# charles-cooper/Smoothed-Particle-Hydrodynamics

Hardware: AMD Instinct MI355X
Metric: particle-steps/sec (whole node) (higher is better)
Workload: dtype f32; 1 GPU; config4_16M_box; particles=16507704, particles_per_gpu=16507704, cell_ids=wide, parallelism=1 GPU

## Files before the change

include/sphmi.h:

```cpp
#ifndef SPHMI_H
#define SPHMI_H

#include <stddef.h>
#include <stdint.h>

#ifdef __cplusplus
extern "C" {
#endif

#define SPHMI_ABI_VERSION 2
#define SPH_MAX_PARTICLES ((1 << 27) - 1)
#define SPH_MAX_NEIGHBOR_COUNT 32
#define SPH_MAX_MEMBRANES_INCLUDING_SAME_PARTICLE 7
#define SPH_LIQUID_PARTICLE 1
#define SPH_ELASTIC_PARTICLE 2
#define SPH_BOUNDARY_PARTICLE 3

typedef enum sph_status {
  SPH_OK = 0,
  SPH_ERR_INVALID = -1,
  SPH_ERR_HIP = -2,
  SPH_ERR_ORDER = -3,
  SPH_ERR_UNKNOWN_BUFFER = -4,
  SPH_ERR_SIZE = -5
// ... 69 lines not shown

#define SPH_SURFACE_FIELDS 6
int sph_extract_surface(sph_solver* s, const float origin[3], const float spacing[3], const int32_t dims[3], uint32_t typeMask,
                        int32_t field, float iso, int64_t counts[2] );
int sph_read_surface(sph_solver* s, float* vertices , int32_t* triangles );

#define SPH_GRADIENT_WORDS 32
int sph_sample_gradient_points(sph_solver* s, const float* points4 , int32_t count,
                               uint32_t typeMask, float* out );
int sph_sample_gradient_grid(sph_solver* s, const float origin[3], const float spacing[3], const int32_t dims[3],
                             uint32_t typeMask, float* out );
int sph_surface_normals(sph_solver* s, float* normals );

#define SPH_DIAG_WORDS 32
#define SPH_DIAG_MAX_REGIONS 16
int sph_diagnostics(sph_solver* s, const float* regions6 , int32_t count,
                    uint32_t typeMask, double* out );
#define SPH_HIST_MAX_BINS 4096
int sph_histogram(sph_solver* s, int32_t field, float lo, float hi, int32_t bins, const float* region6 ,
                  uint32_t typeMask, uint32_t* out );

int sph_label_components(sph_solver* s, float linkRadius, uint32_t typeMask, int64_t counts[2] );
int sph_read_components(sph_solver* s, int32_t* labels , int32_t* rootCount ,
                        float* bbox );
int sph_component_diagnostics(sph_solver* s, const int32_t* components , int32_t count,
                              double* out );

#define SPH_SELECT_WORDS 12
#define SPH_SELECT_MAX_TERMS 4
#define SPH_SELECT_FIELD_SURFACE 7
typedef struct sph_select_term { int32_t field; float lo, hi; } sph_select_term;
int sph_particle_measure(sph_solver* s, float* out );
int sph_select_particles(sph_solver* s, const float* region6 , uint32_t typeMask,
                         const sph_select_term* terms , int32_t termCount, int32_t component ,
                         int64_t* count);
int sph_read_selection(sph_solver* s, int32_t* sortedIndex , uint32_t* origId ,
                       float* records );

#define SPH_ELASTIC_WORDS 12
#define SPH_MUSCLE_WORDS 16
#define SPH_MEMBRANE_WORDS 8
int sph_elastic_measure(sph_solver* s, int32_t* sortedIndex , uint32_t* origId ,
                        float* records , float* connections );
int sph_muscle_diagnostics(sph_solver* s, double* out );
int sph_membrane_measure(sph_solver* s, float* out , double totals[4]);

#define SPH_FORCE_WORDS 40
#define SPH_FORCE_DIAG_WORDS 64
int sph_force_measure(sph_solver* s, int32_t fromSelection, float* out );
int sph_force_diagnostics(sph_solver* s, const float* regions6 , int32_t count,
                          uint32_t typeMask, double* out );

typedef struct sph_render_view {
  int32_t width, height;
  int32_t projection;
  float eye[3], right[3], up[3], forward[3];
  float scale;
  float centre[2];
  float nearPlane;
  float radius;
  float maxRadiusPx;
  int32_t colourMode;
  int32_t field; float lo, hi;
  float typeColour[3][3];
  float ambient;
  uint8_t background[4];
} sph_render_view;
#define SPH_RENDER_FIELD_RAMP { {0.f, 0.f, 1.f}, {0.f, 1.f, 1.f}, {0.f, 1.f, 0.f}, {1.f, 1.f, 0.f}, {1.f, 0.f, 0.f} }
#define SPH_RENDER_LABEL_COLOURS 12
#define SPH_RENDER_LABEL_PALETTE { {0.90f, 0.10f, 0.10f}, {0.10f, 0.50f, 0.90f}, {0.20f, 0.70f, 0.20f}, {0.95f, 0.60f, 0.10f}, \
                                   {0.60f, 0.30f, 0.80f}, {0.10f, 0.75f, 0.75f}, {0.95f, 0.90f, 0.20f}, {0.85f, 0.35f, 0.65f}, \
                                   {0.55f, 0.35f, 0.15f}, {0.40f, 0.85f, 0.55f}, {0.30f, 0.30f, 0.65f}, {0.75f, 0.75f, 0.75f} }
int sph_render_particles(sph_solver* s, const sph_render_view* view, const float* region6 , uint32_t typeMask,
                         int32_t wantThickness, int64_t counts[2] );
int sph_read_render(sph_solver* s, float* depth, int32_t* sortedIndex, uint32_t* origId, uint8_t* rgba ,
                    uint32_t* thickness);

typedef struct sph_render_mesh_style {
  int32_t source;
  int32_t shading;
  int32_t colourMode;
  int32_t field;
  float lo, hi;
  float colour[3];
  int32_t compose;
} sph_render_mesh_style;
int sph_render_mesh(sph_solver* s, const sph_render_view* view, const sph_render_mesh_style* style,
                    int64_t counts[4] );
int sph_read_render_triangles(sph_solver* s, int32_t* triangle );

int sph_remove_region(sph_solver* s, const float* region6 , uint32_t typeMask, int32_t countOnly,
                      int64_t* removed);
int sph_remove_selection(sph_solver* s, int64_t* removed);
int sph_remove_ids(sph_solver* s, const uint32_t* origIds , int64_t count, int64_t* removed);
int sph_add_particles(sph_solver* s, const float* position4, const float* velocity4 , int32_t count);
int sph_emit_lattice(sph_solver* s, const float origin[3], const float spacing[3], const int32_t dims[3], const float velocity[3],
                     float typeValue , int64_t* added);
int sph_read_edit_map(sph_solver* s, int32_t* newIdOfOld );

#define SPH_FIELD_SLOTS 4
#define SPH_FIELD_DIAG_WORDS 8
int sph_field_create(sph_solver* s, int32_t slot, const float* valuesN , float inflow);
int sph_field_release(sph_solver* s, int32_t slot);
int sph_field_write(sph_solver* s, int32_t slot, const float* valuesN );
int sph_field_read(sph_solver* s, int32_t slot, float* outN );
int sph_field_set_region(sph_solver* s, int32_t slot, const float* region6 , uint32_t typeMask, float value,
                         int64_t* painted);
int sph_field_set_selection(sph_solver* s, int32_t slot, float value, int64_t* painted);
int sph_field_diffuse(sph_solver* s, int32_t slot, float coefficient, int32_t substeps, uint32_t typeMask, float* stability);
int sph_field_diagnostics(sph_solver* s, int32_t slot, const float* regions6 , int32_t count,
                          uint32_t typeMask, double* out );

#define SPH_TRACE_TIME 0
#define SPH_TRACE_ARC 1
#define SPH_TRACE_EULER 0
#define SPH_TRACE_MIDPOINT 1
#define SPH_TRACE_MOVING 0
#define SPH_TRACE_MAX_STEPS 1
#define SPH_TRACE_LEFT_MATTER 2
#define SPH_TRACE_LEFT_REGION 3
#define SPH_TRACE_STAGNANT 4
#define SPH_TRACE_NONFINITE 5
#define SPH_TRACE_MAX_STEPS_LIMIT 65535
typedef struct sph_trace_params {
  float step;
  float minSpeed;
  int32_t maxSteps;
  int32_t mode;
  int32_t integrator;
} sph_trace_params;
int sph_trace_streamlines(sph_solver* s, const float* seeds4 , int32_t count, uint32_t typeMask,
                          const sph_trace_params* params, const float* region6 ,
                          float* vertices , int32_t* lengths ,
                          int32_t* status );
int sph_tracers_set(sph_solver* s, const float* points4 , int32_t count);
int sph_tracers_advect(sph_solver* s, uint32_t typeMask, const sph_trace_params* params, const float* region6 ,
                       int64_t counts[2] );
int sph_tracers_read(sph_solver* s, float* pos4 , int32_t* status, int32_t* steps);

int sph_synchronize(sph_solver* s);

typedef enum sph_stage {
  SPH_ST_HASH = 0, SPH_ST_SORT, SPH_ST_SORT_POST, SPH_ST_INDEX, SPH_ST_FIND_NEIGHBORS, SPH_ST_DENSITY,
  SPH_ST_FORCES, SPH_ST_ELASTIC, SPH_ST_PREDICT_DENSITY, SPH_ST_PRESSURE_FORCE, SPH_ST_INTEGRATE, SPH_ST_MEMBRANES,
  SPH_ST_COUNT
} sph_stage;
int sph_set_stage_timing(sph_solver* s, int enable);
int sph_get_stage_times(sph_solver* s, double* ms_total, int64_t* launches, int n);
int sph_reset_stage_times(sph_solver* s);
int sph_step_sort_passes(sph_solver* s);
int sph_set_step_chunks(sph_solver* s, int32_t chunks);
int sph_set_step_pipeline(sph_solver* s, int32_t depth);

typedef struct sph_slab {
  int32_t layerLo, layerHi;
  int32_t ghostLayers;
  int32_t hasLower, hasUpper;
  int32_t globalIdBits;
} sph_slab;
#define SPH_SLAB_RECORD_WORDS 9
#define SPH_SLAB_COMPACT_WORDS 7
int sph_slab_init(sph_solver* s, const sph_slab* slab, const uint32_t* globalIds );
int sph_slab_pack(sph_solver* s, void* msgDown, void* msgUp, int32_t capRecords, int32_t counts[3]);
int sph_slab_pack_framed(sph_solver* s, void* frameDown, void* frameUp, int32_t capRecords, int32_t counts[3]);
int sph_slab_rebuild(sph_solver* s, const void* recvDown, int32_t nDown, const void* recvUp, int32_t nUp);
int sph_slab_step_begin(sph_solver* s, int iterationCount, void* frameDown, void* frameUp, int32_t capRecords);
int sph_slab_step_messages(sph_solver* s, int32_t counts[2]);
int sph_slab_rebuild_framed(sph_solver* s, const void* frameDown, int32_t capDownRecords, const void* frameUp, int32_t capUpRecords);
int sph_slab_rebuild_finish(sph_solver* s, int32_t counts[4]);
int sph_slab_liquid_signature(sph_solver* s, uint32_t* typeBits);
int sph_slab_set_record_format(sph_solver* s, int32_t recordWords, uint32_t typeBits);
int sph_stream_wait_event(sph_solver* s, void* hipEvent);
int sph_particle_count(sph_solver* s);
int sph_slab_read(sph_solver* s, float* position4, float* velocity4, uint32_t* globalIds, uint32_t* owned);

const char* sph_last_error(void);
int sph_abi_version(void);
const char* sph_build_info(void);

#ifdef __cplusplus
}
#endif
#endif
```

smoothed-particle-hydrodynamics_amd/csrc/sph_api.hip:

```cpp
#include <stdarg.h>
#include <string.h>

#include <cmath>
#include <memory>

#include "sph_api_internal.h"
#include "sph_fastmath.h"

#define SPH_STR_(x) #x
#define SPH_STR(x) SPH_STR_(x)
static thread_local char g_err[512] = "";
void sph_set_error(const char* fmt, ...) {
  va_list ap;
  va_start(ap, fmt);
  vsnprintf(g_err, sizeof(g_err), fmt, ap);
  va_end(ap);
}

extern "C" const char* sph_last_error(void) { return g_err; }
extern "C" int sph_abi_version(void) { return SPHMI_ABI_VERSION; }

extern "C" const char* sph_build_info(void) {
  return "libsphmi gfx950 abi " SPH_STR(SPHMI_ABI_VERSION)
#ifdef FN_STAMPS
// ... 196 lines not shown
      if (ended) continue;
      if (x <= -2.f || (double)x >= (double)N) {
        sph_set_error("elastic connection %d of particle %d: partner %g is neither -1 nor in [0, %d)", k, i, x, N);
        return SPH_ERR_INVALID;
      }
      if ((int)x == -1) { ended = true; continue; }
      if (!std::isfinite(w[1])) { sph_set_error("elastic connection %d of particle %d: rest length %g is not finite", k, i, w[1]); return SPH_ERR_INVALID; }
      if (!(w[2] >= -2147483648.f && w[2] < 2147483648.f)) {
        sph_set_error("elastic connection %d of particle %d: muscle word %g does not convert to int", k, i, w[2]);
        return SPH_ERR_INVALID;
      }
    }
  }
  if (!(membraneData && pml && M > 0)) return SPH_OK;
  for (size_t k = 0; k < (size_t)3 * M; k++)
    if (membraneData[k] < 0 || membraneData[k] >= N) {
      sph_set_error("membraneData[%zu] (corner %zu of membrane %zu) = %d is not in [0, %d)", k, k % 3, k / 3, membraneData[k], N);
      return SPH_ERR_INVALID;
    }
  for (int i = 0; i < E; i++)
    for (int k = 0; k < SPH_MAX_MEMBRANES_INCLUDING_SAME_PARTICLE; k++) {
      const int32_t m = pml[(size_t)i * SPH_MAX_MEMBRANES_INCLUDING_SAME_PARTICLE + k];
      if (m < 0) break;
      if (m >= M) {
        sph_set_error("particleMembranesList[%d][%d] = %d is not below numOfMembranes %d", i, k, m, M);
        return SPH_ERR_INVALID;
      }
    }
  if (c.elasticOffset != 0) { sph_set_error("membrane lists need elasticOffset 0 (got %d): they are indexed by original particle id", c.elasticOffset); return SPH_ERR_INVALID; }
  for (int i = E; i < N; i++)
    if (position[4 * (size_t)i + 3] >= 2.f && position[4 * (size_t)i + 3] < 3.f) {
      sph_set_error("particle %d has elastic type %g but lies outside the elastic block [0, %d) that the membrane lists cover", i,
                    position[4 * (size_t)i + 3], E);
      return SPH_ERR_INVALID;
    }
  return SPH_OK;
}

extern "C" int sph_create(const sph_config* cfg, const float* position, const float* velocity, const float* elastic,
                          const int32_t* membraneData, const int32_t* pml, sph_solver** out) {
  if (!cfg || !position || !velocity || !out) { sph_set_error("sph_create: null argument"); return SPH_ERR_INVALID; }
  *out = nullptr;
  if (cfg->abi_version != SPHMI_ABI_VERSION) { sph_set_error("sph_config.abi_version %d != %d", cfg->abi_version, SPHMI_ABI_VERSION); return SPH_ERR_INVALID; }
  const int N = cfg->particleCount;
  const int cap = cfg->capacity > 0 ? cfg->capacity : N;
  static_assert((long long)SPH_MAX_PARTICLES * SPH_MAXN < 0x100000000LL, "uint32 mapBase in k_find_neighbors");
  if (N <= 0 || cap < N || cap > SPH_MAX_PARTICLES) {
    sph_set_error("particleCount %d / capacity %d out of range: one solver holds at most %d particles (2^27 - 1; 32-bit neighbour-map "
                  "indices)", N, cap, SPH_MAX_PARTICLES);
    return SPH_ERR_INVALID;
  }
  if (cfg->gridCellsX <= 0 || cfg->gridCellsY <= 0 || cfg->gridCellsZ <= 0 ||
      (long long)cfg->gridCellsX * cfg->gridCellsY * cfg->gridCellsZ != (long long)cfg->gridCellCount) {
    sph_set_error("gridCellCount does not equal gridCellsX*gridCellsY*gridCellsZ");
    return SPH_ERR_INVALID;
  }
  if (cfg->cellIdMask != 0xffffu && cfg->cellIdMask != 0xffffffffu) { sph_set_error("cellIdMask must be 0xffff (reference) or 0xffffffff (wide)"); return SPH_ERR_INVALID; }
  if (cfg->numOfElasticP < 0 || (cfg->numOfElasticP > 0 && cfg->elasticOffset < 0) || (long long)cfg->numOfElasticP + cfg->elasticOffset > N ||
      (cfg->numOfElasticP > 0 && !elastic)) {
    sph_set_error("elastic configuration inconsistent");
    return SPH_ERR_INVALID;
  }
  if (cfg->numOfElasticP > 0 && (cfg->muscleCount <= 0 || cfg->muscleCount > 4096)) { sph_set_error("muscleCount out of range"); return SPH_ERR_INVALID; }
  if (cfg->maxIteration < 1) { sph_set_error("maxIteration must be >= 1"); return SPH_ERR_INVALID; }
  if (!(cfg->h > 0.f) || !(cfg->hashGridCellSize > 0.f)) { sph_set_error("h / hashGridCellSize must be positive"); return SPH_ERR_INVALID; }

  uint32_t liquidSig = 0u;
  for (int i = 0; i < N; i++) {
    const float* p4 = position + 4 * (size_t)i;
    sph_fold_liquid_signature(liquidSig, p4, velocity + 4 * (size_t)i);
    if (const char* fault = sph_position_fault(*cfg, p4)) {
      sph_set_error("particle %d at (%g, %g, %g) is %s", i, p4[0], p4[1], p4[2], fault);
      return SPH_ERR_INVALID;
    }
  }
  { const int rc = check_elastic_input(*cfg, position, elastic, membraneData, pml); if (rc != SPH_OK) return rc; }
  int ndev = 0;
  const hipError_t devErr = hipGetDeviceCount(&ndev);
  if (devErr != hipSuccess || ndev <= 0 || cfg->device < 0 || cfg->device >= ndev) {
    char two[300];
    if (two_hip_runtimes(two, sizeof(two)))
      sph_set_error("no HIP device %d (found %d): two HIP runtimes are mapped into this process (%s); load the one the rest of the "
                    "process uses BEFORE libsphmi.so so that both bind to it", cfg->device, ndev, two);
    else
      sph_set_error("no HIP device %d (found %d%s%s): libsphmi has no CPU fallback", cfg->device, ndev,
                    devErr != hipSuccess ? ", " : "", devErr != hipSuccess ? hipGetErrorString(devErr) : "");
    return SPH_ERR_HIP;
  }
  SPH_HIP(hipSetDevice(cfg->device));

  std::unique_ptr<sph_solver> owner(new sph_solver());
  sph_solver* const s = owner.get();
  s->cfg = *cfg;
  s->liquidSig = liquidSig;
  if (cfg->stream) { s->stream = (hipStream_t)cfg->stream; s->ownStream = false; }
  else {
    hipError_t e = hipStreamCreateWithFlags(&s->stream, hipStreamNonBlocking);
    if (e != hipSuccess) { sph_set_error("hipStreamCreate failed: %s", hipGetErrorString(e)); return SPH_ERR_HIP; }
    s->ownStream = true;
  }
  SPH_HIP(hipStreamCreateWithFlags(&s->chunkStream, hipStreamNonBlocking));
  SPH_HIP(hipStreamCreateWithFlags(&s->searchStream, hipStreamNonBlocking));
  SPH_HIP(hipEventCreateWithFlags(&s->evSearchFork, hipEventDisableTiming));
  for (hipEvent_t& e : s->evChunk) SPH_HIP(hipEventCreateWithFlags(&e, hipEventDisableTiming));
  SPH_HIP(hipEventCreateWithFlags(&s->evChunkJoin, hipEventDisableTiming));
  SphDev& d = s->d;
  d.N = N; d.G = cfg->gridCellCount; d.gx = cfg->gridCellsX; d.gy = cfg->gridCellsY; d.gz = cfg->gridCellsZ;
  d.cellMask = cfg->cellIdMask;
  d.h = cfg->h; d.cellSize = cfg->hashGridCellSize; d.cellSizeInv = cfg->hashGridCellSizeInv;
  d.simScale = cfg->simulationScale; d.simScaleInv = cfg->simulationScaleInv;
  d.xmin = cfg->xmin; d.xmax = cfg->xmax; d.ymin = cfg->ymin; d.ymax = cfg->ymax; d.zmin = cfg->zmin; d.zmax = cfg->zmax;
  d.r0 = cfg->r0; d.mass = cfg->mass; d.rho0 = cfg->rho0; d.dt = cfg->timeStep; d.delta = cfg->delta;
  d.gravx = cfg->gravity_x; d.gravy = cfg->gravity_y; d.gravz = cfg->gravity_z;
  d.surfTens = cfg->surfTensCoeff;
  {
    volatile float massMu = cfg->mass * cfg->viscosity;
    volatile float hs = cfg->h * cfg->simulationScale;
    volatile float hs2 = hs * hs;
    volatile float hs4 = hs2 * hs2;
    volatile float hs6 = hs4 * hs2;
    volatile float pts = cfg->timeStep * cfg->simulationScaleInv;
    volatile float r0d = cfg->rho0 * cfg->delta;
    volatile float halfHs = hs / 2;
    d.massMu = massMu; d.hs = hs; d.hs2 = hs2; d.hs6 = hs6; d.posTimeStep = pts; d.rho0delta = r0d;
    d.closeR = 0.5 * (double)halfHs;
    float f = (float)d.closeR;
    while ((double)f < d.closeR) f = nextafterf(f, INFINITY);
    while ((double)nextafterf(f, -INFINITY) >= d.closeR) f = nextafterf(f, -INFINITY);
    d.closeRf = f;
  }
  d.massWpoly6 = ((double)cfg->mass) * cfg->Wpoly6Coefficient;
  sph_fast_bounds(cfg->simulationScale, d.hs, (float)((double)d.hs6 * d.massWpoly6), &d.fastD2Min, &d.fastD2Max, &d.fastValueMin);
  d.massGradW = ((double)cfg->mass) * cfg->gradWspikyCoefficient;
  d.del2W = cfg->del2WviscosityCoefficient;
  d.numElastic = cfg->numOfElasticP; d.elasticOffset = cfg->elasticOffset; d.muscleCount = cfg->muscleCount;
  d.numMembranes = cfg->numOfMembranes; d.hasElastic = cfg->numOfElasticP > 0;
  d.rangeLo = 0; d.rangeHi = d.G;

  s->capacity = cap;
  s->capTiles = (cap + SPH_TILE - 1) / SPH_TILE;
  s->sortBits = (cfg->cellIdMask == 0xffffu) ? 16 : bit_length((uint32_t)(d.G > 0 ? d.G - 1 : 0));
  if (s->sortBits < 1) s->sortBits = 1;
  s->maxSortBlocks = (cap + (SPH_BLOCK * 16) - 1) / (SPH_BLOCK * 16);

  int rc = SPH_OK;
  const size_t n = (size_t)cap, nUp = (size_t)N, G1 = (size_t)d.G + 1, mapN = (size_t)s->capTiles * 64 * 32;
#define A(ptr, count) if (rc == SPH_OK) rc = dev_alloc(s, &(ptr), (count))
  A(d.posOrig, n); A(d.velOrig, n); A(d.sortedPos, n); A(d.sortedVel, n); A(d.predPos, 3 * n); A(d.acc, n); A(d.accP, n); A(d.rp, n); A(d.bndMask, n); A(d.gatherRec, 2 * ((n + 3) / 4 * 4));
  A(d.keys, n); A(d.vals, n); A(d.keysAlt, n); A(d.valsAlt, n); A(d.backIndex, n);
  A(d.cellStart, G1); A(d.cellStartRaw, G1);
  A(d.nbrId, mapN); A(d.nbrDist, mapN); A(d.nbr16, mapN); A(d.nbrBase, (size_t)s->capTiles * 64);
  A(d.rho, n);
  const size_t waves = (size_t)s->capTiles;
  A(d.pBlk, waves); A(d.cBlk, waves); A(d.xBlk, waves); A(d.k12Skip, waves); A(d.k10Skip, waves); A(d.skipGate, SPH_GATE_SLOTS);
  A(s->blockHist, (size_t)SPH_SORT_MAX_DIGITS * s->maxSortBlocks + SPH_SORT_MAX_DIGITS);
  A(d.gid, n); A(d.owned, n); A(s->slabCounts, SPH_SLAB_COUNT_WORDS);
  A(d.dbg, SPH_DBG_WORDS); A(s->chunkEdges, SPH_STEP_CHUNKS_MAX + 1); A(s->pipeTable, SPH_STEP_CHUNKS_MAX + 3);
  float* binU = nullptr;
  A(binU, 64);
  d.binU = binU;
  if (d.hasElastic) {
    A(d.elasticMask, n); A(d.membDelta, n); A(d.elastic, (size_t)32 * d.numElastic); A(d.muscle, (size_t)d.muscleCount);
    if (membraneData && pml && cfg->numOfMembranes > 0) { A(d.membraneData, (size_t)3 * cfg->numOfMembranes); A(d.pml, (size_t)7 * d.numElastic); }
  }
#undef A
  if (rc != SPH_OK) return rc;

#define UP(dst, src, bytes) do { hipError_t e_ = hipMemcpyAsync((dst), (src), (bytes), hipMemcpyHostToDevice, s->stream); \
    if (e_ != hipSuccess) { sph_set_error("upload failed: %s", hipGetErrorString(e_)); return SPH_ERR_HIP; } } while (0)
  UP(d.posOrig, position, sizeof(float4) * nUp);
  UP(d.velOrig, velocity, sizeof(float4) * nUp);
  if (d.hasElastic) {
    UP(d.elastic, elastic, sizeof(float4) * 32 * (size_t)d.numElastic);
    hipMemsetAsync(d.muscle, 0, sizeof(float) * (size_t)d.muscleCount, s->stream);
    hipMemsetAsync(d.membDelta, 0, sizeof(float4) * n, s->stream);
    if (d.membraneData) {
      UP(d.membraneData, membraneData, sizeof(int32_t) * 3 * (size_t)cfg->numOfMembranes);
      UP(d.pml, pml, sizeof(int32_t) * 7 * (size_t)d.numElastic);
    }
  }
  {
    float U[64];
    compute_bin_thresholds(cfg->h, U);
    UP(binU, U, sizeof(U));
  }
#undef UP
  hipMemsetAsync(d.predPos, 0, sizeof(float) * 3 * n, s->stream);
  hipMemsetAsync(d.acc, 0, sizeof(float4) * n, s->stream);
  hipMemsetAsync(d.accP, 0, sizeof(float4) * n, s->stream);
  hipMemsetAsync(d.rho, 0, sizeof(float) * n, s->stream);
  hipMemsetAsync(d.rp, 0, sizeof(float2) * n, s->stream);
  for (uint8_t* f : {d.pBlk, d.cBlk, d.xBlk, d.k12Skip, d.k10Skip}) hipMemsetAsync(f, 0, waves, s->stream);
  hipMemsetAsync(d.nbrId, 0xff, sizeof(int32_t) * mapN, s->stream);
  hipMemsetAsync(d.nbrDist, 0, sizeof(float) * mapN, s->stream);
  hipMemsetAsync(d.nbr16, 0xff, sizeof(uint16_t) * mapN, s->stream);
  hipMemsetAsync(d.nbrBase, 0, sizeof(int32_t) * (size_t)s->capTiles * 64, s->stream);
  hipMemsetAsync(d.dbg, 0, sizeof(uint32_t) * SPH_DBG_WORDS, s->stream);
  hipMemsetAsync(d.skipGate, 0, sizeof(uint32_t) * SPH_GATE_SLOTS, s->stream);
  hipMemsetAsync(d.cellStartRaw, 0, sizeof(uint32_t) * G1, s->stream);
  hipMemsetAsync(d.cellStart, 0, sizeof(uint32_t) * G1, s->stream);
  hipMemsetAsync(d.sortedPos, 0, sizeof(float4) * n, s->stream);
  hipMemsetAsync(d.sortedVel, 0, sizeof(float4) * n, s->stream);
  hipMemsetAsync(d.keys, 0, sizeof(uint32_t) * n, s->stream);
  hipMemsetAsync(d.vals, 0, sizeof(uint32_t) * n, s->stream);
  hipMemsetAsync(d.backIndex, 0, sizeof(uint32_t) * n, s->stream);
  hipError_t e = hipStreamSynchronize(s->stream);
  if (e != hipSuccess) { sph_set_error("sph_create: %s", hipGetErrorString(e)); return SPH_ERR_HIP; }
  *out = owner.release();
  return SPH_OK;
}

struct Stage {
  const char* name;
  int need, timer;
  int (*launch)(sph_solver*);
  int gain;
};
#define LAUNCH(call) [](sph_solver* s) { return call; }
static const Stage kClearBuffers = {"sph_run_clear_buffers", 0, SPH_ST_FIND_NEIGHBORS, LAUNCH(sphk_clear_neighbors(s)), 0};
static const Stage kHashParticles = {"sph_run_hash_particles", 0, SPH_ST_HASH, LAUNCH(sphk_hash(s)), P_HASH};
static const Stage kSort = {"sph_run_sort", P_HASH, SPH_ST_SORT, LAUNCH(sphk_sort(s)), P_SORT};
static const Stage kSortPostPass = {"sph_run_sort_post_pass", P_SORT, SPH_ST_SORT_POST, LAUNCH(sphk_sort_post(s)), P_SORTPOST};
static const Stage kIndexx = {"sph_run_indexx", P_SORT, SPH_ST_INDEX, LAUNCH(sphk_index_raw(s)), P_INDEXX};
static const Stage kIndexPostPass = {"sph_run_index_post_pass", P_INDEXX, SPH_ST_INDEX, LAUNCH(sphk_index_fixed(s)), P_INDEXPOST};
static const Stage kFindNeighbors = {"sph_run_find_neighbors", P_SORTPOST | P_INDEXPOST, SPH_ST_FIND_NEIGHBORS, LAUNCH(sphk_find_neighbors(s)), P_FIND};
static const Stage kComputeDensity = {"sph_run_pcisph_compute_density", P_FIND, SPH_ST_DENSITY, LAUNCH(sphk_density(s)), P_DENSITY};
static const Stage kComputeForces = {"sph_run_pcisph_compute_forces_and_init_pressure", P_DENSITY, SPH_ST_FORCES, LAUNCH(sphk_forces(s, false)), P_FORCES};
static const Stage kElasticForces = {"sph_run_pcisph_compute_elastic_forces", P_FORCES, SPH_ST_ELASTIC, LAUNCH(sphk_elastic(s)), 0};
static const Stage kPredictPositions = {"sph_run_pcisph_predict_positions", P_FORCES, SPH_ST_PRESSURE_FORCE, LAUNCH(sphk_predict_positions(s)), P_PREDICTPOS};
static const Stage kPredictDensity = {"sph_run_pcisph_predict_density", P_PREDICTPOS, SPH_ST_PREDICT_DENSITY, LAUNCH(sphk_predict_density(s, false)), P_PREDICTDENS};
static const Stage kCorrectPressure = {"sph_run_pcisph_correct_pressure", P_PREDICTDENS, SPH_ST_PREDICT_DENSITY, LAUNCH(sphk_correct_pressure(s)), 0};
static const Stage kPressureForce = {"sph_run_pcisph_compute_pressure_force_acceleration", P_PREDICTDENS, SPH_ST_PRESSURE_FORCE, LAUNCH(sphk_pressure_force(s, 0)), P_PRESSUREFORCE};
static const Stage kIntegrate = {"sph_run_pcisph_integrate", P_FORCES, SPH_ST_INTEGRATE, LAUNCH(sphk_integrate(s)), 0};
static const Stage kClearMembraneBuffers = {"sph_run_clear_membrane_buffers", 0, SPH_ST_MEMBRANES, LAUNCH(sphk_clear_membranes(s)), 0};
static const Stage kMembranes = {"sph_run_compute_interaction_with_membranes", P_FIND, SPH_ST_MEMBRANES, LAUNCH(sphk_membranes(s)), 0};
static const Stage kMembranesFinalize = {"sph_run_compute_interaction_with_membranes_finalize", 0, SPH_ST_MEMBRANES, LAUNCH(sphk_membranes_finalize(s)), 0};
#undef LAUNCH

static int run_stage(sph_solver* s, const Stage& st) {
  ENTER(s); NEED(s, st.need, st.name);
  sph_state_changes(s);
  StageTimer t(s, st.timer);
  const int rc = st.launch(s);
  if (rc == SPH_OK) s->progress = st.gain == P_HASH ? P_HASH : s->progress | st.gain;
  return rc;
}

extern "C" int sph_run_clear_buffers(sph_solver* s) { return run_stage(s, kClearBuffers); }
extern "C" int sph_run_hash_particles(sph_solver* s) { return run_stage(s, kHashParticles); }
extern "C" int sph_run_sort(sph_solver* s) { return run_stage(s, kSort); }
extern "C" int sph_run_sort_post_pass(sph_solver* s) { return run_stage(s, kSortPostPass); }
extern "C" int sph_run_indexx(sph_solver* s) { return run_stage(s, kIndexx); }
extern "C" int sph_run_index_post_pass(sph_solver* s) { return run_stage(s, kIndexPostPass); }
extern "C" int sph_run_find_neighbors(sph_solver* s) { return run_stage(s, kFindNeighbors); }
extern "C" int sph_run_pcisph_compute_density(sph_solver* s) { return run_stage(s, kComputeDensity); }
extern "C" int sph_run_pcisph_compute_forces_and_init_pressure(sph_solver* s) { return run_stage(s, kComputeForces); }
extern "C" int sph_run_pcisph_compute_elastic_forces(sph_solver* s) { return run_stage(s, kElasticForces); }
extern "C" int sph_run_pcisph_predict_positions(sph_solver* s) { return run_stage(s, kPredictPositions); }
extern "C" int sph_run_pcisph_predict_density(sph_solver* s) { return run_stage(s, kPredictDensity); }
extern "C" int sph_run_pcisph_correct_pressure(sph_solver* s) { return run_stage(s, kCorrectPressure); }
extern "C" int sph_run_pcisph_compute_pressure_force_acceleration(sph_solver* s) { return run_stage(s, kPressureForce); }
extern "C" int sph_run_pcisph_integrate(sph_solver* s, int ) { return run_stage(s, kIntegrate); }
extern "C" int sph_run_clear_membrane_buffers(sph_solver* s) { return run_stage(s, kClearMembraneBuffers); }
extern "C" int sph_run_compute_interaction_with_membranes(sph_solver* s) {
  ENTER(s); NEED(s, kMembranes.need, kMembranes.name);
  if (!s->d.pml) return SPH_OK;
  return run_stage(s, kMembranes);
}
extern "C" int sph_run_compute_interaction_with_membranes_finalize(sph_solver* s) { return run_stage(s, kMembranesFinalize); }

#ifndef SPH_OVERLAP_CHUNKS
#define SPH_OVERLAP_CHUNKS 16
#endif
#ifndef SPH_OVERLAP_MIN_PARTICLES
#define SPH_OVERLAP_MIN_PARTICLES (4 << 20)
#endif
static_assert(SPH_OVERLAP_CHUNKS >= 1 && SPH_OVERLAP_CHUNKS <= SPH_STEP_CHUNKS_MAX, "chunk count");
#ifndef SPH_PIPELINE_DEPTH
#define SPH_PIPELINE_DEPTH 1
#endif
static_assert(SPH_PIPELINE_DEPTH >= 0 && SPH_PIPELINE_DEPTH <= SPH_PIPELINE_STAGES_MAX, "pipeline depth");

extern "C" int sph_set_step_chunks(sph_solver* s, int32_t chunks) {
  ENTER(s);
  if (chunks < 0 || chunks > SPH_STEP_CHUNKS_MAX) { sph_set_error("sph_set_step_chunks: %d is not in [0, %d]", chunks, SPH_STEP_CHUNKS_MAX); return SPH_ERR_INVALID; }
  s->stepChunks = chunks;
  return SPH_OK;
}

extern "C" int sph_set_step_pipeline(sph_solver* s, int32_t depth) {
  ENTER(s);
  if (depth < -1 || depth > SPH_PIPELINE_STAGES_MAX) { sph_set_error("sph_set_step_pipeline: %d is not in [-1, %d]", depth, SPH_PIPELINE_STAGES_MAX); return SPH_ERR_INVALID; }
  s->stepPipeline = depth;
  return SPH_OK;
}

static int step_chunks(const sph_solver* s) {
  if (s->hasSlab || s->timing) return 1;
  if (s->stepChunks > 0) return s->stepChunks;
  return s->d.N >= SPH_OVERLAP_MIN_PARTICLES ? SPH_OVERLAP_CHUNKS : 1;
}

struct ChunkEdges { uint32_t e[SPH_STEP_CHUNKS_MAX + 1]; };
__global__ void k_chunk_edges(uint32_t* edges, ChunkEdges v) {
  if (threadIdx.x <= SPH_STEP_CHUNKS_MAX) edges[threadIdx.x] = v.e[threadIdx.x];
}

static int step_pipeline(const sph_solver* s) {
  return sphPipelineDepth(s->stepPipeline >= 0 ? s->stepPipeline : SPH_PIPELINE_DEPTH, s->cfg.maxIteration, s->d.hasElastic ? 1 : 0);
}

__global__ void k_halo_check(const uint32_t* keys, const uint32_t* cellStart, int G, int gx, int gy, int N, int chunks, ChunkEdges v,
                             uint32_t* table, uint32_t* dbg) {
  const int c = threadIdx.x;
  int ok = 1;
  if (c < chunks) {
    const int64_t reach = (int64_t)gx * gy + gx + 1;
    ok = sphChunkHaloOk(keys, cellStart, G, reach, N, v.e[c], v.e[c + 1], v.e[max(c - 1, 0)], v.e[min(c + 2, chunks)]);
  }
  const bool passed = __all(ok);
  if (c <= SPH_STEP_CHUNKS_MAX) table[c] = passed ? v.e[c] : 0u;
  if (c == 0) {
    table[SPH_STEP_CHUNKS_MAX + 1] = 0u;
    table[SPH_STEP_CHUNKS_MAX + 2] = passed ? 0u : (uint32_t)N;
    atomicAdd(&dbg[passed ? 10 : 9], 1u);
  }
}

static int enqueue_search_overlapped(sph_solver* s, int chunks, int depth) {
  const int N = s->d.N;
  ChunkEdges v;
  for (int i = 0; i <= SPH_STEP_CHUNKS_MAX; i++) v.e[i] = (uint32_t)sphChunkEdge(N, chunks, i);
  if (s->chunkEdgesN != N || s->chunkEdgesC != chunks) {
    hipLaunchKernelGGL(k_chunk_edges, dim3(1), dim3(64), 0, s->stream, s->chunkEdges, v);
    SPH_HIP(hipGetLastError());
    s->chunkEdgesN = N; s->chunkEdgesC = chunks;
  }
  if (depth > 0) {
    hipLaunchKernelGGL(k_halo_check, dim3(1), dim3(64), 0, s->stream, s->d.keys, s->d.cellStart, s->d.G, s->d.gx, s->d.gy, N, chunks, v,
                       s->pipeTable, s->d.dbg);
    SPH_HIP(hipGetLastError());
  }
  SPH_HIP(hipEventRecord(s->evSearchFork, s->stream));
  SPH_HIP(hipStreamWaitEvent(s->searchStream, s->evSearchFork, 0));
  auto launch = [s, N, chunks](int stage, int c) -> int {
    const int lo = (int)sphChunkEdge(N, chunks, c), hi = (int)sphChunkEdge(N, chunks, c + 1);
    if (hi <= lo) return SPH_OK;
    if (stage > 0) return sphk_pipeline_stage(s, stage, c, lo, hi, s->chunkStream);
    hipStream_t fnStream = (c & 1) ? s->searchStream : s->stream;
    int rc = sphk_find_neighbors(s, -1, lo, hi, fnStream);
    if (rc != SPH_OK) return rc;
    SPH_HIP(hipEventRecord(s->evChunk[c], fnStream));
    SPH_HIP(hipStreamWaitEvent(s->chunkStream, s->evChunk[c], 0));
    rc = sphk_density_chunk(s, c, lo, hi, s->chunkStream);
    return rc != SPH_OK ? rc : sphk_pack_gather_records(s, lo, hi, s->chunkStream);
  };
  int32_t stage[SPH_PIPELINE_ITEMS_MAX(SPH_STEP_CHUNKS_MAX)], chunk[SPH_PIPELINE_ITEMS_MAX(SPH_STEP_CHUNKS_MAX)];
  const int items = sphPipelineSchedule(chunks, depth, s->cfg.maxIteration, s->d.hasElastic ? 1 : 0, stage, chunk);
  int rc = SPH_OK;
  for (int i = 0; i < items && rc == SPH_OK; i++) rc = launch(stage[i], chunk[i]);
  SPH_HIP(hipEventRecord(s->evChunkJoin, s->chunkStream));
  SPH_HIP(hipStreamWaitEvent(s->stream, s->evChunkJoin, 0));
  for (int k = 1; k <= depth && rc == SPH_OK; k++) rc = sphk_pipeline_stage(s, k, -1, 0, N, s->stream);
  return rc;
}

int enqueue_step(sph_solver* s, const StepTail* tail) {
  int rc;
  sph_state_changes(s);
#define RUN(stage, call) do { StageTimer t_(s, stage); rc = (call); if (rc != SPH_OK) return rc; } while (0)
  if (s->hasSlab) {
    RUN(SPH_ST_SORT, sphk_hash_sort_post_slab(s));
    RUN(SPH_ST_SORT_POST, sphk_index_fixed(s));
  } else {
    int bits = s->sortBits;
    bool compact = false;
    RUN(SPH_ST_HASH, sphk_hash_for_step(s, &bits, &compact));
    RUN(SPH_ST_SORT, sphk_sort_pairs(s, s->d.N, bits));
    if (compact) {
      StageTimer t_(s, SPH_ST_SORT_POST);
      rc = sphk_sort_post_rekey(s);
      if (rc == SPH_OK) rc = sphk_index_fixed(s);
      if (rc != SPH_OK) return rc;
    } else {
      RUN(SPH_ST_SORT_POST, sphk_sort_post_and_index(s));
    }
  }
  const bool slab = s->hasSlab;
  const int M = s->cfg.maxIteration;
  auto layersFor = [&](int hops) { return slab ? min((hops * 31 + 59) / 60, s->slab.ghostLayers) : -1; };
  const int chunks = step_chunks(s);
  const int piped = chunks > 1 ? step_pipeline(s) : 0;
  s->waveSkip = !slab && piped <= 1;
  if (chunks > 1) {
    rc = enqueue_search_overlapped(s, chunks, piped);
    if (rc != SPH_OK) return rc;
  } else {
    RUN(SPH_ST_FIND_NEIGHBORS, sphk_find_neighbors(s, layersFor(2 * (M - 1) + 1)));
    RUN(SPH_ST_DENSITY, sphk_density(s, layersFor(1)));
  }
  if (slab) RUN(SPH_ST_FORCES, sphk_ghost_init(s));
  const bool densityInForces = !slab && M >= 1;
  if (piped < 1) RUN(SPH_ST_FORCES, sphk_forces(s, true, layersFor(0), densityInForces, chunks <= 1));
  if (s->d.hasElastic) RUN(SPH_ST_ELASTIC, sphk_elastic(s));
  for (int iter = 0; iter < M; iter++) {
    const int left = M - 1 - iter;
    if (piped >= 2 * iter + 2) continue;
    if (piped < 2 * iter + 1) {
      if (iter > 0 || !densityInForces) RUN(SPH_ST_PREDICT_DENSITY, sphk_predict_density(s, true, layersFor(2 * left + 1), iter == 0, iter));
      else RUN(SPH_ST_PREDICT_DENSITY, SPH_OK);
    }
    if (left > 0 || !tail) { RUN(SPH_ST_PRESSURE_FORCE, sphk_pressure_force(s, left == 0 ? 2 : 1, layersFor(2 * left), iter)); continue; }
    const long long lo = max((long long)s->slab.layerLo, 0LL), hi = min((long long)s->slab.layerHi, (long long)s->d.gz);
    const long long W1 = (long long)s->slab.ghostLayers + 1;
    const long long dEnd = s->slab.hasLower ? min(lo + W1, hi) : lo;
    const long long uBeg = s->slab.hasUpper ? max(hi - W1, dEnd) : hi;
    if (dEnd > lo) RUN(SPH_ST_PRESSURE_FORCE, sphk_pressure_force_layers(s, 2, lo, dEnd));
    if (hi > uBeg) RUN(SPH_ST_PRESSURE_FORCE, sphk_pressure_force_layers(s, 2, uBeg, hi));
    const SphDev dA = sph_ranged_layers(s, lo, dEnd), dB = sph_ranged_layers(s, uBeg, hi);
    SlabPart part{SLAB_PART_MESSAGES, dA.rangeLo, dA.rangeHi, dB.rangeLo, dB.rangeHi};
    rc = sphk_slab_pack(s, tail->frameDown ? tail->frameDown + 1 : nullptr, tail->frameUp ? tail->frameUp + 1 : nullptr, tail->capRecords,
                        tail->frameDown, tail->frameUp, part, s->slabCounts + 4);
    if (rc != SPH_OK) return rc;
    SPH_HIP(hipMemcpyAsync(s->slabHost + 4, s->slabCounts + 4, sizeof(uint32_t) * 3, hipMemcpyDeviceToHost, s->stream));
    SPH_HIP(hipEventRecord(s->slabMsgEvent, s->stream));
    if (uBeg > dEnd) RUN(SPH_ST_PRESSURE_FORCE, sphk_pressure_force_layers(s, 2, dEnd, uBeg));
    rc = sphk_slab_pack(s, nullptr, nullptr, 0, nullptr, nullptr, SlabPart{SLAB_PART_KEPT, 0, 0, 0, 0}, s->slabCounts + 8);
    if (rc != SPH_OK) return rc;
    SPH_HIP(hipMemcpyAsync(s->slabHost + 8, s->slabCounts + 8, sizeof(uint32_t) * 3, hipMemcpyDeviceToHost, s->stream));
    SPH_HIP(hipMemcpyAsync(s->slabHost + 3, s->slabCounts + 3, sizeof(uint32_t), hipMemcpyDeviceToHost, s->stream));
    SPH_HIP(hipMemcpyAsync(s->slabHost + 7, s->slabCounts + 7, sizeof(uint32_t), hipMemcpyDeviceToHost, s->stream));
  }
  if (s->d.hasElastic) {
    RUN(SPH_ST_MEMBRANES, sphk_clear_membranes(s));
    if (s->d.pml) RUN(SPH_ST_MEMBRANES, sphk_membranes(s));
    RUN(SPH_ST_MEMBRANES, sphk_membranes_finalize(s));
  }
#undef RUN
  s->progress = P_HASH | P_SORT | P_SORTPOST | P_INDEXPOST | P_FIND | P_DENSITY | P_FORCES | P_PREDICTPOS | P_PREDICTDENS |
                P_PRESSUREFORCE;
  return SPH_OK;
}

extern "C" int sph_step(sph_solver* s, int iterationCount) {
  (void)iterationCount;
  ENTER(s);
  return enqueue_step(s, nullptr);
}

extern "C" int sph_update_muscles(sph_solver* s, const float* signal, int n) {
  ENTER(s);
  if (!signal || n != s->cfg.muscleCount) { sph_set_error("sph_update_muscles: n must equal muscleCount"); return SPH_ERR_SIZE; }
  if (!s->d.muscle) return SPH_OK;
  SPH_HIP(hipMemcpyAsync(s->d.muscle, signal, sizeof(float) * (size_t)n, hipMemcpyHostToDevice, s->stream));
  SPH_HIP(hipStreamSynchronize(s->stream));
  return SPH_OK;
}

extern "C" int sph_step_sort_passes(sph_solver* s) {
  ENTER(s);
  bool compact;
  return sph_sort_passes(sphk_step_sort_bits(s, &compact));
}

extern "C" int sph_synchronize(sph_solver* s) {
  ENTER(s);
  return sph_check_finite_state(s);
}
```

smoothed-particle-hydrodynamics_amd/csrc/sph_api_read.hip:

```cpp
#include <string.h>

#include <vector>

#include "sph_api_internal.h"

int sph_d2h(sph_solver* s, void* dst, const void* src, size_t bytes) {
  SPH_HIP(hipMemcpyAsync(dst, src, bytes, hipMemcpyDeviceToHost, s->stream));
  SPH_HIP(hipStreamSynchronize(s->stream));
  return SPH_OK;
}

static int report_blown_up(sph_solver* s) {
  sph_set_error("%llu particle coordinate(s) were not finite: the simulation state has blown up", (unsigned long long)s->blownUp);
  return SPH_ERR_INVALID;
}
int sph_check_finite_state(sph_solver* s) {
  uint32_t bad = 0;
  SPH_HIP(hipMemcpyAsync(&bad, s->d.dbg + 6, sizeof(bad), hipMemcpyDeviceToHost, s->stream));
  SPH_HIP(hipStreamSynchronize(s->stream));
  if (bad) {
    s->blownUp += bad;
    SPH_HIP(hipMemsetAsync(s->d.dbg + 6, 0, sizeof(uint32_t), s->stream));
  }
  return s->blownUp ? report_blown_up(s) : SPH_OK;
}

extern "C" int sph_read_position(sph_solver* s, float* out) {
  ENTER(s); if (!out) return SPH_ERR_INVALID;
  const int rc = sph_d2h(s, out, s->d.posOrig, sizeof(float4) * (size_t)s->d.N);
  return rc != SPH_OK ? rc : sph_check_finite_state(s);
}
static int copy_setup(sph_solver* s) {
  if (s->copyStream) return SPH_OK;
  SPH_HIP(hipStreamCreateWithFlags(&s->copyStream, hipStreamNonBlocking));
  SPH_HIP(hipEventCreateWithFlags(&s->evReadReady, hipEventDisableTiming));
  SPH_HIP(hipEventCreateWithFlags(&s->evCopyDone, hipEventDisableTiming));
  SPH_HIP(hipHostMalloc((void**)&s->pinnedFlags, sizeof(uint32_t) * 4, hipHostMallocDefault));
  s->pinnedFlags[0] = 0u;
  return SPH_OK;
}

static bool host_pinned(sph_solver* s, void* p, size_t bytes) {
  for (int i = 0; i < s->numHostRegs; i++)
    if ((char*)p >= (char*)s->hostRegs[i].p && (char*)p + bytes <= (char*)s->hostRegs[i].p + s->hostRegs[i].bytes) return true;
  unsigned int flags = 0;
  if (hipHostGetFlags(&flags, p) == hipSuccess) return true;
  (void)hipGetLastError();
  if (s->numHostRegs >= 8) return false;
  const hipError_t e = hipHostRegister(p, bytes, hipHostRegisterDefault);
  if (e != hipSuccess) { (void)hipGetLastError(); return false; }
  s->hostRegs[s->numHostRegs].p = p; s->hostRegs[s->numHostRegs].bytes = bytes; s->numHostRegs++;
  return true;
}

extern "C" int sph_read_position_wait(sph_solver* s) {
  ENTER(s);
  if (!s->copyPending) return s->blownUp ? report_blown_up(s) : SPH_OK;
  SPH_HIP(hipEventSynchronize(s->evCopyDone));
  s->copyPending = false;
  if (s->copyViaStage) memcpy(s->copyUserDst, s->copyStage, s->copyBytes);
  if (s->pinnedFlags[0]) {
    if (!s->blownUp) s->blownUp = s->pinnedFlags[0];
    return report_blown_up(s);
  }
  return s->blownUp ? report_blown_up(s) : SPH_OK;
}

extern "C" int sph_read_position_async(sph_solver* s, float* out) {
  ENTER(s); if (!out) return SPH_ERR_INVALID;
  int rc = copy_setup(s);
  if (rc != SPH_OK) return rc;
  if (s->copyPending) {
    rc = sph_read_position_wait(s);
    if (rc != SPH_OK) return rc;
  }
  const size_t bytes = sizeof(float4) * (size_t)s->d.N;
  void* dst = out;
  s->copyViaStage = false;
  if (!host_pinned(s, out, bytes)) {
    if (s->copyStageBytes < bytes) {
      if (s->copyStage) hipHostFree(s->copyStage);
      s->copyStage = nullptr; s->copyStageBytes = 0;
      SPH_HIP(hipHostMalloc(&s->copyStage, bytes, hipHostMallocDefault));
      s->copyStageBytes = bytes;
    }
    dst = s->copyStage;
    s->copyViaStage = true;
  }
  s->copyUserDst = out;
  s->copyBytes = bytes;
  SPH_HIP(hipEventRecord(s->evReadReady, s->stream));
  SPH_HIP(hipStreamWaitEvent(s->copyStream, s->evReadReady, 0));
  SPH_HIP(hipMemcpyAsync(dst, s->d.posOrig, bytes, hipMemcpyDeviceToHost, s->copyStream));
  SPH_HIP(hipMemcpyAsync(s->pinnedFlags, s->d.dbg + 6, sizeof(uint32_t), hipMemcpyDeviceToHost, s->copyStream));
  SPH_HIP(hipEventRecord(s->evCopyDone, s->copyStream));
  s->copyPending = true;
  return SPH_OK;
}

extern "C" int sph_host_unregister(sph_solver* s, void* p) {
  ENTER(s);
  if (s->copyPending) { const int rc = sph_read_position_wait(s); if (rc != SPH_OK && rc != SPH_ERR_INVALID) return rc; }
  for (int i = 0; i < s->numHostRegs; i++)
    if (s->hostRegs[i].p == p) {
      hipHostUnregister(p);
      s->hostRegs[i] = s->hostRegs[--s->numHostRegs];
      return SPH_OK;
    }
  return SPH_OK;
}

int sph_guard_position_write(sph_solver* s, hipStream_t stream) {
  if (s->copyPending) SPH_HIP(hipStreamWaitEvent(stream ? stream : s->stream, s->evCopyDone, 0));
  return SPH_OK;
}

extern "C" int sph_read_velocity(sph_solver* s, float* out) {
  ENTER(s); if (!out) return SPH_ERR_INVALID;
  return sph_d2h(s, out, s->d.velOrig, sizeof(float4) * (size_t)s->d.N);
}
extern "C" int sph_read_density(sph_solver* s, float* out) {
  ENTER(s); if (!out) return SPH_ERR_INVALID;
  return sph_d2h(s, out, s->d.rho, sizeof(float) * (size_t)s->d.N);
}
extern "C" int sph_read_particle_index(sph_solver* s, uint32_t* out) {
  ENTER(s); if (!out) return SPH_ERR_INVALID;
  const size_t n = (size_t)s->d.N;
  std::vector<uint32_t> k(n), v(n);
  int rc = sph_d2h(s, k.data(), s->d.keys, sizeof(uint32_t) * n);
  if (rc == SPH_OK) rc = sph_d2h(s, v.data(), s->d.vals, sizeof(uint32_t) * n);
  if (rc != SPH_OK) return rc;
  for (size_t i = 0; i < n; i++) { out[2 * i] = k[i]; out[2 * i + 1] = v[i]; }
  return SPH_OK;
}

extern "C" int sph_read_buffer(sph_solver* s, const char* name, void* out, size_t bytes, size_t* needed) {
  ENTER(s);
  if (!name) return SPH_ERR_INVALID;
  const SphDev& d = s->d;
  const size_t n = (size_t)d.N, G1 = (size_t)d.G + 1;
  size_t need = 0;
  enum { B_POS, B_VEL, B_SPOS, B_SVEL, B_ACC, B_NMAP, B_NIDS, B_PI, B_PIB, B_GCI, B_GCIF, B_P, B_RHO, B_DBG, B_TRACE, B_K12SKIP, B_K10SKIP } which;
  if (!strcmp(name, "position")) { which = B_POS; need = sizeof(float4) * 2 * n; }
  else if (!strcmp(name, "velocity")) { which = B_VEL; need = sizeof(float4) * 2 * n; }
  else if (!strcmp(name, "sortedPosition")) { which = B_SPOS; need = sizeof(float4) * 2 * n; }
  else if (!strcmp(name, "sortedVelocity")) { which = B_SVEL; need = sizeof(float4) * n; }
  else if (!strcmp(name, "acceleration")) { which = B_ACC; need = sizeof(float4) * 2 * n; }
  else if (!strcmp(name, "neighborMap")) { which = B_NMAP; need = sizeof(float) * 2 * 32 * n; }
  else if (!strcmp(name, "neighborIds")) { which = B_NIDS; need = sizeof(int32_t) * 32 * n; }
  else if (!strcmp(name, "particleIndex")) { which = B_PI; need = sizeof(uint32_t) * 2 * n; }
  else if (!strcmp(name, "particleIndexBack")) { which = B_PIB; need = sizeof(uint32_t) * n; }
  else if (!strcmp(name, "gridCellIndex")) { which = B_GCI; need = sizeof(uint32_t) * G1; }
  else if (!strcmp(name, "gridCellIndexFixedUp")) { which = B_GCIF; need = sizeof(uint32_t) * G1; }
  else if (!strcmp(name, "pressure")) { which = B_P; need = sizeof(float) * n; }
  else if (!strcmp(name, "rho")) { which = B_RHO; need = sizeof(float) * 2 * n; }
  else if (!strcmp(name, "diagnosticTrace")) { which = B_TRACE; need = sizeof(uint32_t) * n; }
  else if (!strcmp(name, "debugCounters")) { which = B_DBG; need = sizeof(uint32_t) * SPH_DBG_WORDS; }
  else if (!strcmp(name, "pressureForceSkipped")) { which = B_K12SKIP; need = (n + SPH_TILE - 1) / SPH_TILE; }
  else if (!strcmp(name, "predictDensitySkipped")) { which = B_K10SKIP; need = (n + SPH_TILE - 1) / SPH_TILE; }
  else { sph_set_error("unknown buffer '%s'", name); return SPH_ERR_UNKNOWN_BUFFER; }
  if (needed) *needed = need;
  if (!out) return SPH_OK;
  if (bytes != need) { sph_set_error("buffer '%s' is %zu bytes, caller gave %zu", name, need, bytes); return SPH_ERR_SIZE; }
  int rc = SPH_OK;
  char* o = (char*)out;
  switch (which) {
    case B_POS:
      rc = sph_d2h(s, o, d.posOrig, sizeof(float4) * n);
      if (rc == SPH_OK) { if (d.membDelta) rc = sph_d2h(s, o + sizeof(float4) * n, d.membDelta, sizeof(float4) * n); else memset(o + sizeof(float4) * n, 0, sizeof(float4) * n); }
      break;
    case B_VEL:
      rc = sph_d2h(s, o, d.velOrig, sizeof(float4) * n);
      memset(o + sizeof(float4) * n, 0, sizeof(float4) * n);
      break;
    case B_SPOS: {
      std::vector<uint32_t> k(n);
      std::vector<float4> sv(n);
      rc = sph_d2h(s, o, d.sortedPos, sizeof(float4) * n);
      if (rc == SPH_OK) {
        std::vector<float> p3(3 * n);
        rc = sph_d2h(s, p3.data(), d.predPos, sizeof(float) * 3 * n);
        float4* half = (float4*)(o + sizeof(float4) * n);
        if (rc == SPH_OK) for (size_t i = 0; i < n; i++) half[i] = make_float4(p3[3 * i], p3[3 * i + 1], p3[3 * i + 2], 0.f);
      }
      if (rc == SPH_OK) rc = sph_d2h(s, k.data(), d.keys, sizeof(uint32_t) * n);
      if (rc == SPH_OK) rc = sph_d2h(s, sv.data(), d.sortedVel, sizeof(float4) * n);
      if (rc != SPH_OK) break;
      float4* a = (float4*)o;
      for (size_t i = 0; i < n; i++) {
        const int type = (int)a[i].w;
        const float cellf = (float)(int)k[i];
        a[i].w = cellf;
        a[n + i].w = (type == SPH_BOUNDARY_PARTICLE) ? cellf : cellf + d.posTimeStep * (sv[i].w + d.dt * 0.f);
      }
    } break;
    case B_SVEL: rc = sph_d2h(s, o, d.sortedVel, sizeof(float4) * n); break;
    case B_ACC:
      rc = sph_d2h(s, o, d.acc, sizeof(float4) * n);
      if (rc == SPH_OK) rc = sph_d2h(s, o + sizeof(float4) * n, d.accP, sizeof(float4) * n);
      break;
    case B_NIDS: rc = sph_read_neighbor_rows(s, 0, d.N, (int32_t*)o, nullptr); break;
    case B_NMAP: {
      std::vector<int32_t> ids(32 * n);
      std::vector<float> dist(32 * n);
      rc = sph_read_neighbor_rows(s, 0, d.N, ids.data(), dist.data());
      if (rc == SPH_OK) for (size_t e = 0; e < 32 * n; e++) { ((float*)o)[2 * e] = (float)ids[e]; ((float*)o)[2 * e + 1] = dist[e]; }
    } break;
    case B_PI: rc = sph_read_particle_index(s, (uint32_t*)o); break;
    case B_PIB: rc = sph_d2h(s, o, d.backIndex, sizeof(uint32_t) * n); break;
    case B_GCI: rc = sph_d2h(s, o, d.cellStartRaw, sizeof(uint32_t) * G1); break;
    case B_GCIF: rc = sph_d2h(s, o, d.cellStart, sizeof(uint32_t) * G1); break;
    case B_P: {
      std::vector<float2> rp(n);
      rc = sph_d2h(s, rp.data(), d.rp, sizeof(float2) * n);
      if (rc == SPH_OK) for (size_t i = 0; i < n; i++) ((float*)o)[i] = rp[i].y;
    } break;
    case B_TRACE: rc = sph_d2h(s, o, d.valsAlt, sizeof(uint32_t) * n); break;
    case B_DBG: rc = sph_d2h(s, o, d.dbg, sizeof(uint32_t) * SPH_DBG_WORDS); break;
    case B_K12SKIP: rc = sph_d2h(s, o, d.k12Skip, need); break;
    case B_K10SKIP: rc = sph_d2h(s, o, d.k10Skip, need); break;
    case B_RHO:
      rc = sph_d2h(s, o, d.rho, sizeof(float) * n);
      if (rc == SPH_OK) {
        std::vector<float2> rp(n);
        rc = sph_d2h(s, rp.data(), d.rp, sizeof(float2) * n);
        if (rc == SPH_OK) for (size_t i = 0; i < n; i++) ((float*)o)[n + i] = rp[i].x;
      }
      break;
  }
  return rc;
}

extern "C" int sph_read_neighbor_rows(sph_solver* s, int32_t first, int32_t count, int32_t* ids, float* dist) {
  ENTER(s);
  if (first < 0 || count < 0 || (long long)first + count > s->d.N) { sph_set_error("sph_read_neighbor_rows: range outside [0, N)"); return SPH_ERR_INVALID; }
  if (count == 0) return SPH_OK;
  const size_t t0 = (size_t)first / SPH_TILE, t1 = ((size_t)first + count + SPH_TILE - 1) / SPH_TILE;
  const size_t words = (t1 - t0) * 64 * 32, base = t0 * 64 * 32;
  std::vector<int32_t> ti;
  std::vector<float> td;
  int rc = SPH_OK;
  std::vector<uint16_t> t16;
  std::vector<int32_t> tb;
  if (ids) {
    ti.resize(words); t16.resize(words); tb.resize((t1 - t0) * 64);
    rc = sph_d2h(s, ti.data(), s->d.nbrId + base, sizeof(int32_t) * words);
    if (rc == SPH_OK) rc = sph_d2h(s, t16.data(), s->d.nbr16 + base, sizeof(uint16_t) * words);
    if (rc == SPH_OK) rc = sph_d2h(s, tb.data(), s->d.nbrBase + t0 * 64, sizeof(int32_t) * tb.size());
  }
  if (rc == SPH_OK && dist) { td.resize(words); rc = sph_d2h(s, td.data(), s->d.nbrDist + base, sizeof(float) * words); }
  if (rc != SPH_OK) return rc;
  const int shift = (int)(t0 * 64);
  for (int32_t i = 0; i < count; i++)
    for (int k = 0; k < 32; k++) {
      const size_t src = nbr_index(first + i, k) - base;
      if (ids) {
        int j = nbr_decode(t16.data(), tb.data(), ti.data(), first + i - shift, k);
        const uint32_t e = t16[src];
        if (t16[nbr_index(first + i - shift, 0)] != SPH_N16_WIDE && e != SPH_N16_EMPTY && !(e & 0x8000u)) j += shift;
        ids[(size_t)i * 32 + k] = j;
      }
      if (dist) dist[(size_t)i * 32 + k] = td[src];
    }
  return SPH_OK;
}
```

smoothed-particle-hydrodynamics_amd/csrc/sph_common.h:

```cpp
#pragma once
#include <hip/hip_runtime.h>
#include <stdint.h>
#include <stdio.h>

#include <vector>

#include "sphmi.h"
#include "sphmi_chunks.h"

#define SPH_BLOCK 256
#define SPH_TILE 64
#define SPH_MAXN 32
#define SPH_RSEG 30
#define SPH_DBG_WORDS 32
#define SPH_SLAB_COUNT_WORDS 24
#define SPH_SORT_MAX_DIGITS 512
#define SPH_GATE_SLOTS 16
#define SPH_STEP_CHUNKS_MAX 16
static_assert(SPH_CHUNK_ALIGN == SPH_BLOCK, "chunk edges are launch-block edges of the density and pack passes");

struct SphDev {
  int N, G;
  int gx, gy, gz;
  uint32_t cellMask;
  float h, cellSize, cellSizeInv, simScale, simScaleInv;
  float xmin, xmax, ymin, ymax, zmin, zmax;
  float r0, mass, rho0, dt, delta;
  float gravx, gravy, gravz;
  float surfTens;
  float massMu;
  float hs, hs2, hs6;
  float posTimeStep;
  float rho0delta;
  double massWpoly6;
  double massGradW;
  double del2W;
  double closeR;
  float fastValueMin, fastD2Min, fastD2Max;
  float closeRf;
  int rangeLo, rangeHi;
  int numElastic, elasticOffset, muscleCount, numMembranes;
  int hasElastic;
  float4 *posOrig, *velOrig, *membDelta;
  float4 *sortedPos, *sortedVel, *acc, *accP;
  float* predPos;
  uint32_t* elasticMask;
  uint32_t* bndMask;
  float4* gatherRec;
  float2* rp;
  uint8_t* pBlk;
  uint8_t* cBlk;
  uint8_t* xBlk;
  uint32_t* skipGate;
  int gateIn, gateOut;
  uint8_t *k12Skip, *k10Skip;
  uint32_t *keys, *vals, *keysAlt, *valsAlt, *backIndex;
  uint32_t *cellStart, *cellStartRaw;
  uint32_t *gid, *owned;
  int32_t* nbrId;
  float* nbrDist;
  uint16_t* nbr16;
  int32_t* nbrBase;
  float* rho;
  float4* elastic;
  int32_t *membraneData, *pml;
  float* muscle;
  const float* binU;
  uint32_t* dbg;
};

struct SphScratch {
  void* p = nullptr;
  size_t bytes = 0;
  SphScratch() = default;
  SphScratch(const SphScratch&) = delete;
  SphScratch& operator=(const SphScratch&) = delete;
  ~SphScratch() { if (p) hipFree(p); }
};

struct SphDerived {
  bool valid = false;
  int N = 0;
  uint64_t epoch = 0;
};

struct sph_solver {
  sph_config cfg = {};
  SphDev d = {};
  std::vector<void*> allocs;
  hipStream_t stream = nullptr;
  bool ownStream = false;
  int sortBits = 0;
  int capacity = 0;
  int capTiles = 0;
  sph_slab slab = {}; bool hasSlab = false;
  uint32_t* slabCounts = nullptr;
  uint32_t* slabHost = nullptr;
  hipEvent_t slabMsgEvent = nullptr;
  bool slabStepPending = false;
  int slabCapRecords = 0;
  int slabKept = 0;
  int slabRecWords = 0;
  uint32_t slabTypeBits = 0;
  uint32_t liquidSig = 0;
  bool slabRebuildPending = false;
  hipEvent_t slabRebuildEvent = nullptr;
  int slabCapDown = 0, slabCapUp = 0;
  uint32_t* blockHist = nullptr;
  int maxSortBlocks = 0;
  int progress = 0;
  bool timing = false;
  struct Pending { int stage; hipEvent_t a, b; };
  std::vector<Pending> pending;
  double stageMs[SPH_ST_COUNT] = {};
  int64_t stageLaunches[SPH_ST_COUNT] = {};
  hipStream_t copyStream = nullptr;
  hipEvent_t evReadReady = nullptr, evCopyDone = nullptr;
  hipStream_t chunkStream = nullptr, searchStream = nullptr;
  hipEvent_t evChunk[SPH_STEP_CHUNKS_MAX] = {}, evChunkJoin = nullptr, evSearchFork = nullptr;
  int stepChunks = 0;
  uint32_t* chunkEdges = nullptr;
  int chunkEdgesN = -1, chunkEdgesC = -1;
  int stepPipeline = -1;
  bool waveSkip = false;
  uint32_t* pipeTable = nullptr;
  bool copyPending = false;
  float* copyUserDst = nullptr;
  void* copyStage = nullptr; size_t copyStageBytes = 0;
  bool copyViaStage = false;
  size_t copyBytes = 0;
  struct HostReg { void* p; size_t bytes; };
  HostReg hostRegs[8] = {}; int numHostRegs = 0;
  uint32_t* pinnedFlags = nullptr;
  uint64_t blownUp = 0;
  uint64_t stateEpoch = 0;
  SphScratch sampleBuf, diagBuf, surfBuf, meshBuf;
  SphDerived mesh;
  int64_t meshCounts[2] = {};
  uint32_t meshTypeMask = 0; int meshField = 0;
  SphScratch ccBuf, ccTable;
  SphDerived cc;
  int64_t ccCounts[2] = {};
  SphScratch selBuf, selList;
  SphDerived sel;
  int64_t selCount = 0;
  SphScratch elasticBuf;
  SphScratch renderBuf;
  SphDerived render;
  bool renderThickness = false;
  int renderW = 0, renderH = 0;
  SphScratch renderMeshBuf, renderTriBuf;
  bool renderHasMesh = false;
  sph_render_view renderView = {};
  SphScratch editBuf;
  SphDerived map;
  bool mapIdentity = false;
  int mapLength = 0;
  SphScratch fieldSlot[SPH_FIELD_SLOTS], fieldBuf, fieldStage;
  bool fieldLive[SPH_FIELD_SLOTS] = {};
  float fieldInflow[SPH_FIELD_SLOTS] = {};
  SphScratch tracerBuf;
  int tracerCount = 0;

  sph_solver() = default;
  ~sph_solver();
};

int sph_guard_position_write(sph_solver* s, hipStream_t stream = nullptr);

void sph_set_error(const char* fmt, ...);

#define SPH_HIP(call)                                                                   \
  do {                                                                                  \
    hipError_t _e = (call);                                                             \
    if (_e != hipSuccess) {                                                             \
      sph_set_error("%s failed: %s (%s:%d)", #call, hipGetErrorString(_e), __FILE__, __LINE__); \
      return SPH_ERR_HIP;                                                               \
    }                                                                                   \
  } while (0)

static inline int sph_blocks(int n, int per = SPH_BLOCK) { return (n + per - 1) / per; }

SphDev sph_ranged(const sph_solver* s, int ghostDepth);

#ifdef __HIPCC__
__device__ __forceinline__ bool sph_range_id(const SphDev& d, int linear, int& id) {
  const int begin = (int)d.cellStart[d.rangeLo], end = (int)d.cellStart[d.rangeHi];
  id = begin + linear;
  return id < end;
}

__device__ __forceinline__ int xcd_block(int nblocks) {
  const int b = blockIdx.x;
  const int per = nblocks >> 3;
  const int even = per << 3;
  if (b >= even) return b;
  return (b & 7) * per + (b >> 3);
}
#endif


__host__ __device__ static inline size_t nbr_index(int id, int slot) {
  return ((((size_t)(id >> 6) * 8 + (size_t)(slot >> 2)) * 64 + (size_t)(id & 63)) << 2) + (size_t)(slot & 3);
}

#define SPH_N16_BIAS 16384
#define SPH_N16_MAX 0x7FFD
#define SPH_N16_EMPTY 0xFFFFu
#define SPH_N16_WIDE 0xFFFEu
__host__ __device__ static inline int nbr_decode(const uint16_t* n16, const int32_t* nbase, const int32_t* n32, int id, int slot) {
  const size_t row0 = nbr_index(id, 0), at = nbr_index(id, slot);
  if (n16[row0] == SPH_N16_WIDE) return n32[at];
  const uint32_t e = n16[at];
  if (e == SPH_N16_EMPTY) return -1;
  return ((e & 0x8000u) ? nbase[id] : id) + (int)(e & 0x7fffu) - SPH_N16_BIAS;
}

int sphk_hash(sph_solver* s);
int sphk_sort(sph_solver* s);
int sphk_sort_pairs(sph_solver* s, int n, int bits);
int sph_sort_passes(int bits);
int sphk_step_sort_bits(const sph_solver* s, bool* compact);
int sphk_hash_for_step(sph_solver* s, int* sortBits, bool* compact);
int sphk_sort_post_rekey(sph_solver* s);
int sphk_sort_post(sph_solver* s);
int sphk_index_raw(sph_solver* s);
int sphk_index_fixed(sph_solver* s);
int sphk_sort_post_and_index(sph_solver* s);
int sphk_hash_sort_post_slab(sph_solver* s);
int sphk_clear_neighbors(sph_solver* s);
int sphk_find_neighbors(sph_solver* s, int ghostDepth = -1, int idxLo = 0, int idxHi = INT32_MAX, hipStream_t stream = nullptr);
int sphk_density(sph_solver* s, int ghostDepth = -1);
int sphk_density_chunk(sph_solver* s, int c, int idxLo, int idxHi, hipStream_t stream);
int sphk_pack_gather_records(sph_solver* s, int idxLo, int idxHi, hipStream_t stream);
int sphk_forces(sph_solver* s, bool fusePredict, int ghostDepth = -1, bool fuseDensity = false, bool packRecords = true);
int sphk_ghost_init(sph_solver* s);
int sphk_predict_positions(sph_solver* s);
int sphk_predict_density(sph_solver* s, bool fuseCorrect, int ghostDepth = -1, bool first = false, int iteration = 0);
int sphk_correct_pressure(sph_solver* s);
int sphk_pressure_force(sph_solver* s, int fuse, int ghostDepth = -1, int iteration = 0);
int sphk_integrate(sph_solver* s);
int sphk_pipeline_stage(sph_solver* s, int stage, int c, int idxLo, int idxHi, hipStream_t stream);
enum { SLAB_PART_ALL = 0, SLAB_PART_MESSAGES = 1, SLAB_PART_KEPT = 2 };
struct SlabPart { int mode, a0, a1, b0, b1; };
int sphk_slab_pack(sph_solver* s, uint32_t* msgDown, uint32_t* msgUp, int capRecords, uint32_t* headDown = nullptr,
                   uint32_t* headUp = nullptr,
                   SlabPart part = SlabPart{SLAB_PART_ALL, 0, 0, 0, 0}, uint32_t* counts = nullptr);
SphDev sph_ranged_layers(const sph_solver* s, long long loLayer, long long hiLayer);
int sphk_pressure_force_layers(sph_solver* s, int fuse, long long loLayer, long long hiLayer);
int sphk_slab_rebuild(sph_solver* s, const uint32_t* recvDown, int nDown, const uint32_t* recvUp, int nUp, int kept);
int sphk_slab_rebuild_framed(sph_solver* s, const uint32_t* frameDown, int capDown, const uint32_t* frameUp, int capUp,
                             const uint32_t* keptPtr, uint32_t* totals);
int sphk_slab_sort_rebuild(sph_solver* s, int total);
struct SampleArgs {
  uint32_t typeMask;
  float hh;
  float ss2;
  float mwp;
  float ox, oy, oz, sx, sy, sz;
  int nx, ny, nz, kBase;
};
int sphk_sample_points(sph_solver* s, const SampleArgs& a, const float* pts4, int count, float* out);
int sphk_sample_grid(sph_solver* s, const SampleArgs& a, const float origin[3], const float spacing[3], int nx, int ny,
                     int kBase, int nz, float* out);
int sphk_gradient_points(sph_solver* s, const SampleArgs& a, float K, const float* pts4, int count, float* out);
int sphk_gradient_grid(sph_solver* s, const SampleArgs& a, float K, const float origin[3], const float spacing[3], int nx, int ny,
                       int kBase, int nz, float* out);
int sphk_surface_normals(sph_solver* s, const SampleArgs& a, float K, int field, const float* verts, int count, float* normals);
struct TraceArgs {
  float step, minSpeed;
  int maxSteps, mode, integrator;
  int hasRegion;
  float box[6];
};
int sphk_trace_streamlines(sph_solver* s, const SampleArgs& a, const TraceArgs& t, const float* seeds4, int count, float* verts,
                           int32_t* lengths, int32_t* status);
int sphk_tracers_advect(sph_solver* s, const SampleArgs& a, const TraceArgs& t, float* pos4, int32_t* status, int32_t* steps,
// ... 108 lines not shown
```

smoothed-particle-hydrodynamics_amd/csrc/sph_pcisph.hip:

```cpp
#include "sph_common.h"
#include "sph_fastmath.h"

#define TYPE_OF(p4) ((int)(p4).w)
typedef float f32x3 __attribute__((ext_vector_type(3)));
typedef f32x3 f32x3a __attribute__((aligned(4)));
__device__ __forceinline__ float4 load_pred(const SphDev& d, int id) {
  const f32x3a v = *reinterpret_cast<const f32x3a*>(d.predPos + 3 * (size_t)id);
  return make_float4(v.x, v.y, v.z, 0.f);
}
__device__ __forceinline__ void store_pred(const SphDev& d, int id, const float4 p) {
  const f32x3a v = {p.x, p.y, p.z};
  *reinterpret_cast<f32x3a*>(d.predPos + 3 * (size_t)id) = v;
}
#define NBR_INDEX(j) (max((j), 0))

#define FC_BATCH 8
#define PF_BATCH 8
#define PD_BATCH 16
#define SPH_SERIAL_GRID 2048

__device__ __forceinline__ size_t rec_index(int j, int part) { return ((size_t)(j >> 2) << 3) + (size_t)(part << 2) + (size_t)(j & 3); }

struct NbrTile {
  const int4* ids;
  const float4* dist;
  const uint2* v16;
  int self, zOff;
  __device__ __forceinline__ NbrTile(const SphDev& d, int id) {
    const size_t base = ((size_t)(id >> 6) * 8) * 64 + (size_t)(id & 63);
    ids = reinterpret_cast<const int4*>(d.nbrId) + base;
    dist = reinterpret_cast<const float4*>(d.nbrDist) + base;
    v16 = reinterpret_cast<const uint2*>(d.nbr16) + base;
    self = id;
    zOff = d.nbrBase[id] - id;
  }
  __device__ __forceinline__ int4 id4(int g) const { return ids[(size_t)g * 64]; }
  __device__ __forceinline__ float4 dist4(int g) const {
    typedef float nt4 __attribute__((ext_vector_type(4)));
    const nt4 q = __builtin_nontemporal_load(reinterpret_cast<const nt4*>(&dist[(size_t)g * 64]));
    return make_float4(q.x, q.y, q.z, q.w);
  }
  __device__ __forceinline__ uint2 vec16(int g) const {
    typedef unsigned int nt2 __attribute__((ext_vector_type(2)));
    const nt2 q = __builtin_nontemporal_load(reinterpret_cast<const nt2*>(&v16[(size_t)g * 64]));
    return make_uint2(q.x, q.y);
  }
  __device__ __forceinline__ static bool wide(const uint2& group0) { return (group0.x & 0xffffu) == SPH_N16_WIDE; }
  __device__ __forceinline__ int id_wide(int slot) const {
    return reinterpret_cast<const int32_t*>(ids)[((size_t)(slot >> 2) * 64) * 4 + (size_t)(slot & 3)];
  }
  __device__ __forceinline__ int decode(const uint2& v, int k) const {
    const uint32_t w = (k >> 1) == 0 ? v.x : v.y;
    const uint32_t e = (k & 1) ? (w >> 16) : (w & 0xffffu);
    const int j = self - SPH_N16_BIAS + (int)(e & 0x7fffu) + ((e & 0x8000u) ? zOff : 0);
    return e == SPH_N16_EMPTY ? -1 : j;
  }
};

__device__ __forceinline__ bool xcd_range_id(const SphDev& d, int b, int& id) {
  const int begin = (int)d.cellStart[d.rangeLo], end = (int)d.cellStart[d.rangeHi];
  const int active = (end - begin + SPH_BLOCK - 1) / SPH_BLOCK;
  if (b >= active) return false;
  const int per = active >> 3, even = per << 3;
  if (b < even) {
    const int x = b & 7;
    int k = b >> 3;
    b = x * per + k;
  }
  id = begin + b * SPH_BLOCK + threadIdx.x;
  return id < end;
}
__device__ __forceinline__ bool xcd_range_id(const SphDev& d, int& id) { return xcd_range_id(d, (int)blockIdx.x, id); }
__device__ __forceinline__ int range_blocks(const SphDev& d) {
  return ((int)d.cellStart[d.rangeHi] - (int)d.cellStart[d.rangeLo] + SPH_BLOCK - 1) / SPH_BLOCK;
}

__device__ __forceinline__ bool wave_leader() { return (int)__lane_id() == __ffsll((unsigned long long)__ballot(1)) - 1; }
__device__ __forceinline__ bool wave_flag_store(uint8_t* flags, int id, bool set) {
  const bool any = __any(set);
  if (wave_leader()) flags[id >> 6] = any ? 1 : 0;
  return any;
}
__device__ __forceinline__ bool gate_open(const SphDev& d) { return d.skipGate[d.gateIn] == 0u; }
__device__ __forceinline__ void gate_count(const SphDev& d, int id, bool waveFlagged) {
  if (waveFlagged && ((id >> 8) & 63) == 0 && wave_leader() && *(volatile uint32_t*)&d.skipGate[d.gateOut] == 0u)
    atomicAdd(&d.skipGate[d.gateOut], 1u);
}
__device__ __forceinline__ bool nbr_wave_flags(const NbrTile& t, const uint2 (&v16)[8], const bool wideRow, const uint8_t* flags) {
  uint32_t seen = 0u;
#pragma unroll
  for (int g = 0; g < 8; g++) {
    int jj[4];
#pragma unroll
    for (int k = 0; k < 4; k++) jj[k] = t.decode(v16[g], k);
    if (wideRow) {
#pragma unroll
      for (int k = 0; k < 4; k++) jj[k] = t.id_wide(g * 4 + k);
    }
#pragma unroll
    for (int k = 0; k < 4; k++) {
      const uint32_t f = flags[NBR_INDEX(jj[k]) >> 6];
      seen |= jj[k] != -1 ? f : 0u;
    }
  }
  return seen != 0u;
}

constexpr int DENSITY_ITEMS = 1;
__global__ __launch_bounds__(SPH_BLOCK) void k_density(SphDev d, int nblocks) {
  typedef float nt4 __attribute__((ext_vector_type(4)));
  const int begin = (int)d.cellStart[d.rangeLo], end = (int)d.cellStart[d.rangeHi];
  const int first = begin + blockIdx.x * (SPH_BLOCK * DENSITY_ITEMS) + threadIdx.x;
  float4 r[DENSITY_ITEMS][8];
#pragma unroll
  for (int it = 0; it < DENSITY_ITEMS; it++) {
    const int id = first + it * SPH_BLOCK;
    if (id < end) {
      const NbrTile t(d, id);
#pragma unroll
      for (int g = 0; g < 8; g++) {
        const nt4 q = __builtin_nontemporal_load(reinterpret_cast<const nt4*>(&t.dist[(size_t)g * 64]));
        r[it][g] = make_float4(q.x, q.y, q.z, q.w);
      }
    }
  }
#pragma unroll
  for (int it = 0; it < DENSITY_ITEMS; it++) {
    const int id = first + it * SPH_BLOCK;
    if (id >= end) continue;
    double density = 0.0;
#pragma unroll
    for (int g = 0; g < 8; g++) {
      const float rr[4] = {r[it][g].x, r[it][g].y, r[it][g].z, r[it][g].w};
#pragma unroll
      for (int k = 0; k < 4; k++) {
        if (rr[k] != -1.f) {
          const float r2 = rr[k] * rr[k];
          const float a = d.hs2 - r2;
          density += (double)(a * a * a);
        }
      }
    }
    if (density < (double)d.hs6) density = (double)d.hs6;
    density *= d.massWpoly6;
    d.rho[id] = (float)density;
  }
}

int sphk_density(sph_solver* s, int ghostDepth) {
  const int nb = sph_blocks(s->d.N, SPH_BLOCK * DENSITY_ITEMS);
  hipLaunchKernelGGL(k_density, dim3(nb), dim3(SPH_BLOCK), 0, s->stream, sph_ranged(s, ghostDepth), nb);
  SPH_HIP(hipGetLastError());
  return SPH_OK;
}

__device__ __forceinline__ float4 predict_position(const SphDev& d, const float4 x, const float4 v, const float4 ap) {
  if (TYPE_OF(x) == SPH_BOUNDARY_PARTICLE) return x;
  float4 o;
  o.x = x.x + d.posTimeStep * (v.x + d.dt * ap.x);
  o.y = x.y + d.posTimeStep * (v.y + d.dt * ap.y);
  o.z = x.z + d.posTimeStep * (v.z + d.dt * ap.z);
  o.w = x.w;
  return o;
}

__global__ __launch_bounds__(SPH_BLOCK) void k_predict_positions(SphDev d) {
  const int id = blockIdx.x * SPH_BLOCK + threadIdx.x;
  if (id >= d.N) return;
  store_pred(d, id, predict_position(d, d.sortedPos[id], d.sortedVel[id], d.accP[id]));
}

int sphk_predict_positions(sph_solver* s) {
  hipLaunchKernelGGL(k_predict_positions, dim3(sph_blocks(s->d.N)), dim3(SPH_BLOCK), 0, s->stream, s->d);
  SPH_HIP(hipGetLastError());
  return SPH_OK;
}

__device__ __forceinline__ float corrected_pressure(const SphDev& d, float p, float rhoPred);

template <bool FUSE_PREDICT, bool FUSE_DENSITY>
__device__ __forceinline__ void forces_particle(const SphDev& d, const int id) {
  static_assert(FUSE_PREDICT || !FUSE_DENSITY, "the density half reads what the predict half forms");
  const float4 xi = d.sortedPos[id];
  const float4 zero = make_float4(0.f, 0.f, 0.f, 0.f);
  const bool boundary = TYPE_OF(xi) == SPH_BOUNDARY_PARTICLE;
  if (!FUSE_DENSITY && boundary) {
    d.acc[id] = zero;
    if (FUSE_PREDICT) store_pred(d, id, xi);
    else { d.accP[id] = zero; d.rp[id].y = 0.f; }
    return;
  }
  const float4 vi = d.sortedVel[id];
  const NbrTile t(d, id);
  float4 xpi = xi;
  if (FUSE_DENSITY) xpi = predict_position(d, xi, vi, zero);
  double density = 0.0;
  float sx = 0.f, sy = 0.f, sz = 0.f, tx = 0.f, ty = 0.f, tz = 0.f;
  uint32_t bnd = 0u, ela = 0u;
  bool wideRow = false;
  bool closePair = false;
#pragma unroll 1
  for (int b = 0; b < 32 / FC_BATCH; b++) {
    int jj[FC_BATCH];
    float rr[FC_BATCH];
#pragma unroll
    for (int q = 0; q < FC_BATCH / 4; q++) {
      const float4 rq = t.dist4(b * (FC_BATCH / 4) + q);
      rr[4 * q] = rq.x; rr[4 * q + 1] = rq.y; rr[4 * q + 2] = rq.z; rr[4 * q + 3] = rq.w;
    }
#pragma unroll
    for (int q = 0; q < FC_BATCH / 4; q++) {
      const uint2 v = t.vec16(b * (FC_BATCH / 4) + q);
      if (b == 0 && q == 0) wideRow = NbrTile::wide(v);
#pragma unroll
      for (int k = 0; k < 4; k++) jj[4 * q + k] = t.decode(v, k);
    }
    if (wideRow) {
#pragma unroll
      for (int k = 0; k < FC_BATCH; k++) jj[k] = t.id_wide(b * FC_BATCH + k);
    }
    float4 xj[FC_BATCH], vr[FC_BATCH];
#pragma unroll
    for (int k = 0; k < FC_BATCH; k++) {
      const int jc = NBR_INDEX(jj[k]);
      xj[k] = d.gatherRec[rec_index(jc, 0)];
      vr[k] = d.gatherRec[rec_index(jc, 1)];
    }
#pragma unroll
    for (int k = 0; k < FC_BATCH; k++) {
      const int slot = b * FC_BATCH + k;
      const bool valid = jj[k] != -1;
      if (valid && TYPE_OF(xj[k]) == SPH_BOUNDARY_PARTICLE) bnd |= 1u << slot;
      if (valid && TYPE_OF(xj[k]) == SPH_ELASTIC_PARTICLE) ela |= 1u << slot;
      const bool use = valid && rr[k] < d.hs;
      if (FUSE_DENSITY) closePair |= valid && rr[k] < d.closeRf;
      const float rj = vr[k].w;
      const float w = d.hs - rr[k];
      sx = use ? sx + (vr[k].x - vi.x) * w / rj : sx;
      sy = use ? sy + (vr[k].y - vi.y) * w / rj : sy;
      sz = use ? sz + (vr[k].z - vi.z) * w / rj : sz;
      tx = use ? tx + d.surfTens * (xi.x - xj[k].x) : tx;
      ty = use ? ty + d.surfTens * (xi.y - xj[k].y) : ty;
      tz = use ? tz + d.surfTens * (xi.z - xj[k].z) : tz;
      if (FUSE_DENSITY) {
        const float4 xpj = predict_position(d, xj[k], vr[k], zero);
        const float rx = xpi.x - xpj.x, ry = xpi.y - xpj.y, rz = xpi.z - xpj.z;
        const float r2 = (rx * rx + ry * ry + rz * rz) * d.simScale * d.simScale;
        const float a = d.hs2 - r2;
        const float term = (valid && r2 < d.hs2) ? a * a * a : 0.f;
        density += (double)term;
      }
    }
  }
  if (FUSE_DENSITY) {
    if (density < (double)d.hs6) density = (double)d.hs6;
    density *= d.massWpoly6;
    const float rhoP = (float)density;
    const float p = corrected_pressure(d, 0.f, rhoP);
    d.rp[id] = make_float2(rhoP, p);
    store_pred(d, id, xpi);
    if (d.pBlk) {
      const bool anyP = wave_flag_store(d.pBlk, id, p != 0.f);
      const bool anyC = wave_flag_store(d.cBlk, id, closePair && !boundary);
      gate_count(d, id, anyP || anyC);
    }
    if (boundary) { d.acc[id] = zero; return; }
  }
  d.bndMask[id] = bnd;
  if (d.hasElastic) d.elasticMask[id] = ela;
  const float scale = d.massMu * (float)(d.del2W / (double)d.rho[id]);
  float4 a;
  a.x = sx * scale + d.gravx + tx;
  a.y = sy * scale + d.gravy + ty;
  a.z = sz * scale + d.gravz + tz;
  a.w = 0.f;
  d.acc[id] = a;
  if (FUSE_DENSITY) return;
  if (FUSE_PREDICT) store_pred(d, id, predict_position(d, xi, vi, zero));
  else { d.accP[id] = zero; d.rp[id].y = 0.f; }
}

template <bool FUSE_PREDICT, bool FUSE_DENSITY>
__global__ __launch_bounds__(SPH_BLOCK, 4) void k_forces(SphDev d, int nblocks) {
  int id;
  if (!xcd_range_id(d, id)) return;
  forces_particle<FUSE_PREDICT, FUSE_DENSITY>(d, id);
}
template <bool FUSE_PREDICT, bool FUSE_DENSITY>
__global__ __launch_bounds__(SPH_BLOCK, 4) void k_forces_strided(SphDev d) {
  const int active = range_blocks(d);
  for (int b = blockIdx.x; b < active; b += gridDim.x) {
    int id;
    if (xcd_range_id(d, b, id)) forces_particle<FUSE_PREDICT, FUSE_DENSITY>(d, id);
  }
}


__global__ __launch_bounds__(SPH_BLOCK) void k_pack_gather_records(SphDev d, int lo, int hi) {
  const int id = lo + blockIdx.x * SPH_BLOCK + threadIdx.x;
  if (id >= hi) return;
  const float4 v = d.sortedVel[id];
  d.gatherRec[rec_index(id, 0)] = d.sortedPos[id];
  d.gatherRec[rec_index(id, 1)] = make_float4(v.x, v.y, v.z, d.rho[id]);
}

__global__ __launch_bounds__(SPH_BLOCK) void k_ghost_init(SphDev d) {
  const int id = blockIdx.x * SPH_BLOCK + threadIdx.x;
  if (id >= d.N) return;
  const float4 zero = make_float4(0.f, 0.f, 0.f, 0.f);
  store_pred(d, id, predict_position(d, d.sortedPos[id], d.sortedVel[id], zero));
}

int sphk_ghost_init(sph_solver* s) {
  hipLaunchKernelGGL(k_ghost_init, dim3(sph_blocks(s->d.N)), dim3(SPH_BLOCK), 0, s->stream, s->d);
  SPH_HIP(hipGetLastError());
  return SPH_OK;
}

int sphk_pack_gather_records(sph_solver* s, int idxLo, int idxHi, hipStream_t stream) {
  if (idxLo < 0 || idxLo % 4 != 0) { sph_set_error("sphk_pack_gather_records: idxLo %d is not a multiple of 4", idxLo); return SPH_ERR_INVALID; }
  idxHi = min(idxHi, s->d.N);
  if (idxHi <= idxLo) return SPH_OK;
  hipLaunchKernelGGL(k_pack_gather_records, dim3(sph_blocks(idxHi - idxLo)), dim3(SPH_BLOCK), 0, stream, s->d, idxLo, idxHi);
  SPH_HIP(hipGetLastError());
  return SPH_OK;
}

int sphk_density_chunk(sph_solver* s, int c, int idxLo, int idxHi, hipStream_t stream) {
  if (c < 0 || c >= SPH_STEP_CHUNKS_MAX || idxLo < 0 || idxHi > s->d.N) { sph_set_error("sphk_density_chunk: chunk %d [%d, %d) of %d particles", c, idxLo, idxHi, s->d.N); return SPH_ERR_INVALID; }
  if (idxHi <= idxLo) return SPH_OK;
  SphDev d = s->d;
  d.cellStart = s->chunkEdges; d.rangeLo = c; d.rangeHi = c + 1;
  const int nb = sph_blocks(idxHi - idxLo, SPH_BLOCK * DENSITY_ITEMS);
  hipLaunchKernelGGL(k_density, dim3(nb), dim3(SPH_BLOCK), 0, stream, d, nb);
  SPH_HIP(hipGetLastError());
  return SPH_OK;
}

static SphDev wave_skip_view(const sph_solver* s, SphDev d, bool fused, int stage) {
  if (!(fused && s->waveSkip)) d.pBlk = d.cBlk = d.xBlk = d.k12Skip = d.k10Skip = nullptr;
  d.gateIn = (stage - 1) & (SPH_GATE_SLOTS - 1); d.gateOut = stage & (SPH_GATE_SLOTS - 1);
  return d;
}

int sphk_forces(sph_solver* s, bool fusePredict, int ghostDepth, bool fuseDensity, bool packRecords) {
  if (fuseDensity && (!fusePredict || s->hasSlab)) { sph_set_error("sphk_forces: the density half needs the fused step outside slab mode"); return SPH_ERR_INVALID; }
  const int nb = sph_blocks(s->d.N);
  const SphDev d = wave_skip_view(s, sph_ranged(s, ghostDepth), fuseDensity, 1);
  if (packRecords) { const int rc = sphk_pack_gather_records(s, 0, s->d.N, s->stream); if (rc != SPH_OK) return rc; }
  if (fuseDensity) hipLaunchKernelGGL((k_forces<true, true>), dim3(nb), dim3(SPH_BLOCK), 0, s->stream, d, nb);
  else if (fusePredict) hipLaunchKernelGGL((k_forces<true, false>), dim3(nb), dim3(SPH_BLOCK), 0, s->stream, d, nb);
  else hipLaunchKernelGGL((k_forces<false, false>), dim3(nb), dim3(SPH_BLOCK), 0, s->stream, d, nb);
  SPH_HIP(hipGetLastError());
  return SPH_OK;
}

__device__ __forceinline__ float corrected_pressure(const SphDev& d, float p, float rhoPred) {
  const float rho_err = rhoPred - d.rho0;
  float p_corr = rho_err * d.delta;
  if (p_corr < 0.f) p_corr = 0.f;
  return p + p_corr;
}

template <bool FUSE_CORRECT, bool FIRST>
__device__ __forceinline__ void predict_density_particle(const SphDev& d, const int id) {
  const float4 xi = load_pred(d, id);
  const NbrTile t(d, id);
  uint2 v16[8];
#pragma unroll
  for (int g = 0; g < 8; g++) v16[g] = t.vec16(g);
  const bool wideRow = NbrTile::wide(v16[0]);
  if (FUSE_CORRECT && !FIRST && d.xBlk) {
    bool skip = false;
    const float2 old = d.rp[id];
    if (gate_open(d)) {
      const bool moved = d.xBlk[id >> 6] != 0 || nbr_wave_flags(t, v16, wideRow, d.xBlk);
      skip = !__any(moved);
    }
    if (wave_leader()) d.k10Skip[id >> 6] = skip ? 1 : 0;
    if (skip) {
      const float p = corrected_pressure(d, old.y, old.x);
      d.rp[id] = make_float2(old.x, p);
      gate_count(d, id, wave_flag_store(d.pBlk, id, p != 0.f) || d.cBlk[id >> 6] != 0);
      return;
    }
  }
  double density = 0.0;
#pragma unroll
  for (int b = 0; b < 32 / PD_BATCH; b++) {
    int jj[PD_BATCH];
#pragma unroll
    for (int k = 0; k < PD_BATCH; k++) {
      const int slot = b * PD_BATCH + k;
      jj[k] = t.decode(v16[slot >> 2], slot & 3);
    }
    if (wideRow) {
#pragma unroll
      for (int k = 0; k < PD_BATCH; k++) jj[k] = t.id_wide(b * PD_BATCH + k);
    }
    float4 xj[PD_BATCH];
#pragma unroll
    for (int k = 0; k < PD_BATCH; k++) xj[k] = load_pred(d, NBR_INDEX(jj[k]));
#pragma unroll
    for (int k = 0; k < PD_BATCH; k++) {
      const float rx = xi.x - xj[k].x, ry = xi.y - xj[k].y, rz = xi.z - xj[k].z;
      const float r2 = (rx * rx + ry * ry + rz * rz) * d.simScale * d.simScale;
      const float a = d.hs2 - r2;
      const float term = (jj[k] != -1 && r2 < d.hs2) ? a * a * a : 0.f;
      density += (double)term;
    }
  }
  if (density < (double)d.hs6) density = (double)d.hs6;
  density *= d.massWpoly6;
  const float rhoP = (float)density;
  if (FUSE_CORRECT) {
    const float pOld = FIRST ? 0.f : d.rp[id].y;
    const float p = corrected_pressure(d, pOld, rhoP);
    d.rp[id] = make_float2(rhoP, p);
    if (d.pBlk) gate_count(d, id, wave_flag_store(d.pBlk, id, p != 0.f) || d.cBlk[id >> 6] != 0);
  } else {
    d.rp[id].x = rhoP;
  }
}

template <bool FUSE_CORRECT, bool FIRST>
__global__ __launch_bounds__(SPH_BLOCK) void k_predict_density(SphDev d, int nblocks) {
  int id;
  if (!xcd_range_id(d, id)) return;
  predict_density_particle<FUSE_CORRECT, FIRST>(d, id);
}
template <bool FUSE_CORRECT, bool FIRST>
__global__ __launch_bounds__(SPH_BLOCK) void k_predict_density_strided(SphDev d) {
  const int active = range_blocks(d);
  for (int b = blockIdx.x; b < active; b += gridDim.x) {
    int id;
    if (xcd_range_id(d, b, id)) predict_density_particle<FUSE_CORRECT, FIRST>(d, id);
  }
}

int sphk_predict_density(sph_solver* s, bool fuseCorrect, int ghostDepth, bool first, int iteration) {
  const int nb = sph_blocks(s->d.N);
  const SphDev d = wave_skip_view(s, sph_ranged(s, ghostDepth), fuseCorrect, 2 * iteration + 1);
  if (fuseCorrect && first) hipLaunchKernelGGL((k_predict_density<true, true>), dim3(nb), dim3(SPH_BLOCK), 0, s->stream, d, nb);
  else if (fuseCorrect) hipLaunchKernelGGL((k_predict_density<true, false>), dim3(nb), dim3(SPH_BLOCK), 0, s->stream, d, nb);
  else hipLaunchKernelGGL((k_predict_density<false, false>), dim3(nb), dim3(SPH_BLOCK), 0, s->stream, d, nb);
  SPH_HIP(hipGetLastError());
  return SPH_OK;
}

__global__ __launch_bounds__(SPH_BLOCK) void k_correct_pressure(SphDev d) {
  const int id = blockIdx.x * SPH_BLOCK + threadIdx.x;
  if (id >= d.N) return;
  const float2 v = d.rp[id];
  d.rp[id].y = corrected_pressure(d, v.y, v.x);
}

int sphk_correct_pressure(sph_solver* s) {
  hipLaunchKernelGGL(k_correct_pressure, dim3(sph_blocks(s->d.N)), dim3(SPH_BLOCK), 0, s->stream, s->d);
  SPH_HIP(hipGetLastError());
  return SPH_OK;
}

__device__ __forceinline__ void integrate_particle(const SphDev& d, int id, const float4 x, const float4 v, const float4 a0,
                                                   const float4 a1) {
  const float ax = a0.x + a1.x, ay = a0.y + a1.y, az = a0.z + a1.z;
  float nvx = v.x + d.dt * ax, nvy = v.y + d.dt * ay, nvz = v.z + d.dt * az, nvw = v.w + d.dt * 0.f;
  float nx = x.x + d.posTimeStep * nvx, ny = x.y + d.posTimeStep * nvy, nz = x.z + d.posTimeStep * nvz;
  if (nx < d.xmin) nx = d.xmin;
  if (ny < d.ymin) ny = d.ymin;
  if (nz < d.zmin) nz = d.zmin;
  if (nx > d.xmax - 0.000001f) nx = d.xmax - 0.000001f;
  if (ny > d.ymax - 0.000001f) ny = d.ymax - 0.000001f;
  if (nz > d.zmax - 0.000001f) nz = d.zmax - 0.000001f;
  nvx = (v.x + nvx) * 0.5f; nvy = (v.y + nvy) * 0.5f; nvz = (v.z + nvz) * 0.5f; nvw = (v.w + nvw) * 0.5f;

  const NbrTile t(d, id);
  float ncx = 0.f, ncy = 0.f, ncz = 0.f, ncw = 0.f, wsum = 0.f, wsum2 = 0.f;
  const uint32_t bnd = d.bndMask[id];
  if (__any(bnd != 0u)) {
    const bool wideRow = NbrTile::wide(t.vec16(0));
#pragma unroll 2
    for (int g = 0; g < 8; g++) {
      const uint2 v = t.vec16(g);
#pragma unroll
      for (int k = 0; k < 4; k++) {
        if (!((bnd >> (g * 4 + k)) & 1u)) continue;
        const int jb = wideRow ? t.id_wide(g * 4 + k) : t.decode(v, k);
        const float4 pb = d.sortedPos[jb];
        float dist = (nx - pb.x) * (nx - pb.x);
        dist += (ny - pb.y) * (ny - pb.y);
        dist += (nz - pb.z) * (nz - pb.z);
        dist = sqrtf(dist);
        const float w = fmaxf(0.f, (d.r0 - dist) / d.r0);
        const float4 nb = d.sortedVel[jb];
        ncx += nb.x * w; ncy += nb.y * w; ncz += nb.z * w; ncw += nb.w * w;
        wsum += w;
        wsum2 += w * (d.r0 - dist);
      }
    }
  }
  float len = ((ncx * ncx + ncy * ncy) + ncz * ncz) + ncw * ncw;
  if (len != 0.f) {
    len = sqrtf(len);
    nx += ((ncx / len) * wsum2) / wsum;
    ny += ((ncy / len) * wsum2) / wsum;
    nz += ((ncz / len) * wsum2) / wsum;
    const float vn = ncx * nvx + ncy * nvy + ncz * nvz;
    if (vn < 0.f) {
      nvx -= ncx * vn; nvy -= ncy * vn; nvz -= ncz * vn;
      nvx *= 0.99f; nvy *= 0.99f; nvz *= 0.99f; nvw *= 0.99f;
    }
  }
  if (!d.hasElastic) {
    nx += 0.f; ny += 0.f; nz += 0.f;
  }
  const uint32_t src = d.vals[id];
  d.velOrig[src] = make_float4(nvx, nvy, nvz, nvw);
  d.posOrig[src] = make_float4(nx, ny, nz, x.w);
}

__global__ __launch_bounds__(SPH_BLOCK) void k_integrate(SphDev d, int nblocks) {
  const int id = xcd_block(nblocks) * SPH_BLOCK + threadIdx.x;
  if (id >= d.N) return;
  const float4 x = d.sortedPos[id];
  if (TYPE_OF(x) == SPH_BOUNDARY_PARTICLE) return;
  integrate_particle(d, id, x, d.sortedVel[id], d.acc[id], d.accP[id]);
}

int sphk_integrate(sph_solver* s) {
  const int nb = sph_blocks(s->d.N);
  { const int g = sph_guard_position_write(s); if (g != SPH_OK) return g; }
  hipLaunchKernelGGL(k_integrate, dim3(nb), dim3(SPH_BLOCK), 0, s->stream, s->d, nb);
  SPH_HIP(hipGetLastError());
  return SPH_OK;
}

template <bool FAST>
__device__ __forceinline__ bool pf_batch(const SphDev& d, const float4 xi, const float pi_, const float hq, const float4 (&xj)[PF_BATCH],
                                         const float2 (&rpj)[PF_BATCH], const int (&jj)[PF_BATCH], float& rx, float& ry, float& rz,
                                         const bool ownOk) {
  bool ok = ownOk;
  const float half = FAST ? SPH_FAST_HALF_SCALED : 0.5f;
#pragma unroll
  for (int k = 0; k < PF_BATCH; k++) {
    const float ex_ = xi.x - xj[k].x, ey_ = xi.y - xj[k].y, ez_ = xi.z - xj[k].z;
    const float d2_ = ex_ * ex_ + ey_ * ey_ + ez_ * ez_;
    float sq_;
    if (FAST) ok = sph_sqrt_fast(d2_, d.fastD2Min, d.fastD2Max, &sq_) && ok;
    else sq_ = sqrtf(d2_);
    const float r = sq_ * d.simScale;
    float num = -(d.hs - r) * (d.hs - r) * half * (pi_ + rpj[k].y);
    if (__any(r < d.closeRf)) num = (r < d.closeRf) ? -(hq - r) * (hq - r) * half * d.rho0delta : num;
    const float value = FAST ? sph_div1_by(num, rpj[k].x) : num / rpj[k].x;
    const float vx = (xi.x - xj[k].x) * d.simScale, vy = (xi.y - xj[k].y) * d.simScale, vz = (xi.z - xj[k].z) * d.simScale;
    const bool use = jj[k] != -1 && r < d.hs;
    const float ax_ = value * vx, ay_ = value * vy, az_ = value * vz;
    float q_[3];
    if (FAST) ok = (sph_div3_by<false>(ax_, ay_, az_, value, d.fastValueMin, r, q_) || !use) && ok;
    else { q_[0] = ax_ / r; q_[1] = ay_ / r; q_[2] = az_ / r; }
    if (FAST) {
      rx = use ? __builtin_fmaf(q_[0], SPH_FAST_UNSCALE, rx) : rx;
      ry = use ? __builtin_fmaf(q_[1], SPH_FAST_UNSCALE, ry) : ry;
      rz = use ? __builtin_fmaf(q_[2], SPH_FAST_UNSCALE, rz) : rz;
    } else {
      rx = use ? rx + q_[0] : rx;
      ry = use ? ry + q_[1] : ry;
      rz = use ? rz + q_[2] : rz;
    }
  }
  return !FAST || !__any(!ok);
}

template <int FUSE>
__device__ __forceinline__ void pressure_force_particle(const SphDev& d, const int id) {
  const float4 xi = d.sortedPos[id];
  const float4 zero = make_float4(0.f, 0.f, 0.f, 0.f);
  const bool boundary = TYPE_OF(xi) == SPH_BOUNDARY_PARTICLE;
  if (FUSE != 0 && d.pBlk && !__any(!boundary) && wave_leader()) {
    d.k12Skip[id >> 6] = 1;
    if (FUSE == 1) d.xBlk[id >> 6] = 0;
  }
  if (boundary) {
    if (FUSE == 1) store_pred(d, id, xi);
    else d.accP[id] = zero;
    return;
  }
  const float2 rpi = d.rp[id];
  const bool consult = FUSE != 0 && d.pBlk && gate_open(d);
  float4 vi = zero;
  if (FUSE != 0) vi = d.sortedVel[id];
  const float pi_ = rpi.y;
  const bool ownOk = sph_exp_in(xi.x, SPH_FAST_COORD_EXP_LO, 100) && sph_exp_in(xi.y, SPH_FAST_COORD_EXP_LO, 100) &&
                     sph_exp_in(xi.z, SPH_FAST_COORD_EXP_LO, 100);
  const NbrTile t(d, id);
  float rx = 0.f, ry = 0.f, rz = 0.f;
  const float hq = d.hs * 0.25f;
  uint2 v16[8];
#pragma unroll
  for (int g = 0; g < 8; g++) v16[g] = t.vec16(g);
  const bool wideRow = NbrTile::wide(v16[0]);
  bool skip = false;
  if (consult) {
    const bool live = pi_ != 0.f || nbr_wave_flags(t, v16, wideRow, d.pBlk);
    skip = d.cBlk[id >> 6] == 0 && !__any(live);
  }
  if (FUSE != 0 && d.pBlk && wave_leader()) d.k12Skip[id >> 6] = skip ? 1 : 0;
  if (!skip) {
#pragma unroll
    for (int b = 0; b < 32 / PF_BATCH; b++) {
      int jj[PF_BATCH];
#pragma unroll
      for (int k = 0; k < PF_BATCH; k++) {
        const int slot = b * PF_BATCH + k;
        jj[k] = t.decode(v16[slot >> 2], slot & 3);
      }
      if (wideRow) {
#pragma unroll
        for (int k = 0; k < PF_BATCH; k++) jj[k] = t.id_wide(b * PF_BATCH + k);
      }
      float4 xj[PF_BATCH];
      float2 rpj[PF_BATCH];
#pragma unroll
      for (int k = 0; k < PF_BATCH; k++) {
        const int jc = NBR_INDEX(jj[k]);
        xj[k] = d.sortedPos[jc];
        rpj[k] = d.rp[jc];
      }
      const float bx = rx, by = ry, bz = rz;
      if (!pf_batch<true>(d, xi, pi_, hq, xj, rpj, jj, rx, ry, rz, ownOk)) {
        if ((threadIdx.x & 63) == 0) atomicAdd(&d.dbg[8], 1u);
        rx = bx; ry = by; rz = bz;
        pf_batch<false>(d, xi, pi_, hq, xj, rpj, jj, rx, ry, rz, true);
      }
    }
  }
  const float scale = (float)(d.massGradW / (double)rpi.x);
  const float4 ap = make_float4(rx * scale, ry * scale, rz * scale, 0.f);
  if (FUSE != 1) d.accP[id] = ap;
  if (FUSE == 1) {
    const float4 xp = predict_position(d, xi, vi, ap);
    if (d.xBlk) {
      bool changed = true;
      if (consult) {
        const float4 was = load_pred(d, id);
        changed = __float_as_uint(was.x) != __float_as_uint(xp.x) || __float_as_uint(was.y) != __float_as_uint(xp.y) ||
                  __float_as_uint(was.z) != __float_as_uint(xp.z);
      }
      gate_count(d, id, wave_flag_store(d.xBlk, id, changed));
    }
    store_pred(d, id, xp);
  }
  if (FUSE == 2) integrate_particle(d, id, xi, vi, d.acc[id], ap);
}

template <int FUSE>
__global__ __launch_bounds__(SPH_BLOCK) void k_pressure_force(SphDev d, int nblocks) {
  int id;
  if (!xcd_range_id(d, id)) return;
  pressure_force_particle<FUSE>(d, id);
}
template <int FUSE>
__global__ __launch_bounds__(SPH_BLOCK) void k_pressure_force_strided(SphDev d) {
  const int active = range_blocks(d);
  for (int b = blockIdx.x; b < active; b += gridDim.x) {
    int id;
    if (xcd_range_id(d, b, id)) pressure_force_particle<FUSE>(d, id);
  }
}

static int launch_pressure_force(sph_solver* s, int fuse, const SphDev& ranged, int nb, hipStream_t stream, int stage) {
  const SphDev d = wave_skip_view(s, ranged, fuse != 0, stage);
  if (fuse == 2) { const int g = sph_guard_position_write(s, stream); if (g != SPH_OK) return g; }
  if (fuse == 0) hipLaunchKernelGGL((k_pressure_force<0>), dim3(nb), dim3(SPH_BLOCK), 0, stream, d, nb);
  else if (fuse == 1) hipLaunchKernelGGL((k_pressure_force<1>), dim3(nb), dim3(SPH_BLOCK), 0, stream, d, nb);
  else hipLaunchKernelGGL((k_pressure_force<2>), dim3(nb), dim3(SPH_BLOCK), 0, stream, d, nb);
  SPH_HIP(hipGetLastError());
  return SPH_OK;
}

int sphk_pressure_force(sph_solver* s, int fuse, int ghostDepth, int iteration) {
  return launch_pressure_force(s, fuse, sph_ranged(s, ghostDepth), sph_blocks(s->d.N), s->stream, 2 * iteration + 2);
}

int sphk_pressure_force_layers(sph_solver* s, int fuse, long long loLayer, long long hiLayer) {
  return launch_pressure_force(s, fuse, sph_ranged_layers(s, loLayer, hiLayer), sph_blocks(s->d.N), s->stream, 0);
}

int sphk_pipeline_stage(sph_solver* s, int stage, int c, int idxLo, int idxHi, hipStream_t stream) {
  const int M = s->cfg.maxIteration;
  if (s->hasSlab || !s->pipeTable || stage < 1 || stage > 2 * M || c >= SPH_STEP_CHUNKS_MAX || idxLo < 0 || idxHi > s->d.N) {
    sph_set_error("sphk_pipeline_stage: stage %d of %d, chunk %d [%d, %d) of %d particles", stage, 2 * M, c, idxLo, idxHi, s->d.N);
    return SPH_ERR_INVALID;
  }
  if (idxHi <= idxLo) return SPH_OK;
  SphDev d = wave_skip_view(s, s->d, true, stage);
  d.cellStart = c >= 0 ? s->pipeTable : s->pipeTable + SPH_STEP_CHUNKS_MAX + 1;
  d.rangeLo = c >= 0 ? c : 0; d.rangeHi = d.rangeLo + 1;
  const int nb = sph_blocks(idxHi - idxLo);
  const bool last = stage == 2 * M;
  if (c < 0) {
    const int grid = min(nb, SPH_SERIAL_GRID);
    if (last) { const int g = sph_guard_position_write(s, stream); if (g != SPH_OK) return g; }
    if (stage == 1) hipLaunchKernelGGL((k_forces_strided<true, true>), dim3(grid), dim3(SPH_BLOCK), 0, stream, d);
    else if (stage & 1) hipLaunchKernelGGL((k_predict_density_strided<true, false>), dim3(grid), dim3(SPH_BLOCK), 0, stream, d);
    else if (last) hipLaunchKernelGGL((k_pressure_force_strided<2>), dim3(grid), dim3(SPH_BLOCK), 0, stream, d);
    else hipLaunchKernelGGL((k_pressure_force_strided<1>), dim3(grid), dim3(SPH_BLOCK), 0, stream, d);
  } else if (stage == 1) {
    hipLaunchKernelGGL((k_forces<true, true>), dim3(nb), dim3(SPH_BLOCK), 0, stream, d, nb);
  } else if (stage & 1) {
    hipLaunchKernelGGL((k_predict_density<true, false>), dim3(nb), dim3(SPH_BLOCK), 0, stream, d, nb);
  } else {
    return launch_pressure_force(s, last ? 2 : 1, d, nb, stream, stage);
  }
  SPH_HIP(hipGetLastError());
  return SPH_OK;
}
```

smoothed-particle-hydrodynamics_amd/csrc/sph_sort.hip:

```cpp
#include "sph_common.h"

__global__ __launch_bounds__(SPH_BLOCK) void k_hash(SphDev d) {
  const int id = blockIdx.x * SPH_BLOCK + threadIdx.x;
  if (id < SPH_GATE_SLOTS) d.skipGate[id] = 0u;
  if (id >= d.N) return;
  const float4 p = d.posOrig[id];
  if (!(fabsf(p.x) <= 3.0e38f && fabsf(p.y) <= 3.0e38f && fabsf(p.z) <= 3.0e38f)) atomicAdd(&d.dbg[6], 1u);
  const int cx = (int)(p.x * d.cellSizeInv), cy = (int)(p.y * d.cellSizeInv), cz = (int)(p.z * d.cellSizeInv);
  const int cell = cx + cy * d.gx + cz * d.gx * d.gy;
  d.keys[id] = (uint32_t)cell & d.cellMask;
  d.vals[id] = (uint32_t)id;
}

struct CompactKey { int usedX, usedY, czBase, layers; };

__global__ __launch_bounds__(SPH_BLOCK) void k_hash_compact(SphDev d, CompactKey c) {
  const int id = blockIdx.x * SPH_BLOCK + threadIdx.x;
  if (id < SPH_GATE_SLOTS) d.skipGate[id] = 0u;
  if (id >= d.N) return;
  const float4 p = d.posOrig[id];
  if (!(fabsf(p.x) <= 3.0e38f && fabsf(p.y) <= 3.0e38f && fabsf(p.z) <= 3.0e38f)) atomicAdd(&d.dbg[6], 1u);
  const int cx = min(max((int)(p.x * d.cellSizeInv), 0), c.usedX - 1), cy = min(max((int)(p.y * d.cellSizeInv), 0), c.usedY - 1);
  const int cz = min(max((int)(p.z * d.cellSizeInv) - c.czBase, 0), c.layers - 1);
  d.keys[id] = (uint32_t)(cx + c.usedX * (cy + c.usedY * cz));
  d.vals[id] = (uint32_t)id;
}

__global__ __launch_bounds__(SPH_BLOCK) void k_sort_post_rekey(SphDev d) {
  const int i = blockIdx.x * SPH_BLOCK + threadIdx.x;
  if (i >= d.N) return;
  const uint32_t src = d.vals[i];
  const float4 p = d.posOrig[src];
  d.sortedPos[i] = p;
  d.sortedVel[i] = d.velOrig[src];
  d.backIndex[src] = (uint32_t)i;
  const int cx = (int)(p.x * d.cellSizeInv), cy = (int)(p.y * d.cellSizeInv), cz = (int)(p.z * d.cellSizeInv);
  d.keys[i] = (uint32_t)(cx + cy * d.gx + cz * d.gx * d.gy) & d.cellMask;
}

static int bits_for(long long n) { int b = 1; while ((1LL << b) < n) b++; return b; }

static CompactKey compact_plan(const sph_solver* s, int* bits) {
  const SphDev& d = s->d;
  CompactKey c;
  c.usedX = min((int)(d.xmax * d.cellSizeInv) + 1, d.gx);
  c.usedY = min((int)(d.ymax * d.cellSizeInv) + 1, d.gy);
  long long lo = 0, hi = min((long long)(d.zmax * d.cellSizeInv) + 1, (long long)d.gz);
  if (s->hasSlab) {
    lo = max((long long)s->slab.layerLo - s->slab.ghostLayers - 2, 0LL);
    hi = min((long long)s->slab.layerHi + s->slab.ghostLayers + 2, (long long)d.gz);
  }
  c.czBase = (int)lo; c.layers = (int)max(hi - lo, 1LL);
  *bits = bits_for((long long)c.usedX * c.usedY * c.layers);
  return c;
}

int sphk_step_sort_bits(const sph_solver* s, bool* compact) {
  int bits = s->sortBits;
  const CompactKey c = compact_plan(s, &bits);
  const SphDev& d = s->d;
  const bool clampFree = d.xmin >= 0.f && d.ymin >= 0.f && d.zmin >= 0.f && (int)(d.xmax * d.cellSizeInv) < c.usedX &&
                         (int)(d.ymax * d.cellSizeInv) < c.usedY && (s->hasSlab || (int)(d.zmax * d.cellSizeInv) < c.czBase + c.layers);
  *compact = clampFree && s->d.cellMask == 0xffffffffu && sph_sort_passes(bits) < sph_sort_passes(s->sortBits);
  return *compact ? bits : s->sortBits;
}

int sphk_hash_for_step(sph_solver* s, int* sortBits, bool* compact) {
  *sortBits = sphk_step_sort_bits(s, compact);
  if (!*compact) return sphk_hash(s);
  int bits;
  const CompactKey c = compact_plan(s, &bits);
  hipLaunchKernelGGL(k_hash_compact, dim3(sph_blocks(s->d.N)), dim3(SPH_BLOCK), 0, s->stream, s->d, c);
  SPH_HIP(hipGetLastError());
  return SPH_OK;
}

int sphk_sort_post_rekey(sph_solver* s) {
  hipLaunchKernelGGL(k_sort_post_rekey, dim3(sph_blocks(s->d.N)), dim3(SPH_BLOCK), 0, s->stream, s->d);
  SPH_HIP(hipGetLastError());
  return SPH_OK;
}

int sphk_hash_sort_post_slab(sph_solver* s) {
  int bits;
  bool compact;
  int rc = sphk_hash_for_step(s, &bits, &compact);
  if (rc == SPH_OK) rc = sphk_sort_pairs(s, s->d.N, bits);
  if (rc != SPH_OK) return rc;
  return compact ? sphk_sort_post_rekey(s) : sphk_sort_post(s);
}

int sphk_hash(sph_solver* s) {
  hipLaunchKernelGGL(k_hash, dim3(sph_blocks(s->d.N)), dim3(SPH_BLOCK), 0, s->stream, s->d);
  SPH_HIP(hipGetLastError());
  return SPH_OK;
}

#define RS_ITEMS 16
#define RS_TILE (SPH_BLOCK * RS_ITEMS)

template <int BITS>
__global__ __launch_bounds__(SPH_BLOCK) void k_radix_hist(const uint32_t* __restrict__ keys, int N, int shift,
                                                           uint32_t* __restrict__ blockHist, int numBlocks) {
  constexpr int D = 1 << BITS;
  __shared__ uint32_t hist[D];
  for (int i = threadIdx.x; i < D; i += SPH_BLOCK) hist[i] = 0;
  __syncthreads();
  const int base = blockIdx.x * RS_TILE;
#pragma unroll
  for (int r = 0; r < RS_ITEMS; r++) {
    const int i = base + r * SPH_BLOCK + threadIdx.x;
    if (i < N) atomicAdd(&hist[(keys[i] >> shift) & (uint32_t)(D - 1)], 1u);
  }
  __syncthreads();
  for (int i = threadIdx.x; i < D; i += SPH_BLOCK) blockHist[(size_t)i * numBlocks + blockIdx.x] = hist[i];
}

__global__ __launch_bounds__(SPH_BLOCK) void k_radix_scan_rows(uint32_t* __restrict__ blockHist, int numBlocks,
                                                                uint32_t* __restrict__ digitTotal) {
  __shared__ uint32_t part[SPH_BLOCK];
  uint32_t* row = blockHist + (size_t)blockIdx.x * numBlocks;
  const int per = (numBlocks + SPH_BLOCK - 1) / SPH_BLOCK;
  const int lo = min((int)threadIdx.x * per, numBlocks), hi = min(lo + per, numBlocks);
  uint32_t sum = 0;
  for (int i = lo; i < hi; i++) sum += row[i];
  part[threadIdx.x] = sum;
  __syncthreads();
  for (int off = 1; off < SPH_BLOCK; off <<= 1) {
    const uint32_t v = (threadIdx.x >= (unsigned)off) ? part[threadIdx.x - off] : 0u;
    __syncthreads();
    part[threadIdx.x] += v;
    __syncthreads();
  }
  uint32_t run = part[threadIdx.x] - sum;
  for (int i = lo; i < hi; i++) { const uint32_t v = row[i]; row[i] = run; run += v; }
  if (threadIdx.x == SPH_BLOCK - 1) digitTotal[blockIdx.x] = part[SPH_BLOCK - 1];
}

template <int BITS>
__global__ __launch_bounds__(SPH_BLOCK) void k_radix_scatter(const uint32_t* __restrict__ keysIn,
                                                              const uint32_t* __restrict__ valsIn,
                                                              uint32_t* __restrict__ keysOut,
                                                              uint32_t* __restrict__ valsOut, int N, int shift,
                                                              const uint32_t* __restrict__ blockHist, int numBlocks,
                                                              const uint32_t* __restrict__ digitTotal) {
  constexpr int D = 1 << BITS, PER = D / SPH_BLOCK;
  __shared__ volatile uint32_t waveCount[4][D];
  __shared__ uint32_t digitBase[4][D];
  __shared__ uint32_t scan[SPH_BLOCK];
  const int wave = threadIdx.x >> 6, lane = threadIdx.x & 63;
  for (int i = threadIdx.x; i < 4 * D; i += SPH_BLOCK) waveCount[i / D][i % D] = 0;
  uint32_t tot[PER], mySum = 0;
#pragma unroll
  for (int p = 0; p < PER; p++) { tot[p] = digitTotal[threadIdx.x * PER + p]; mySum += tot[p]; }
  scan[threadIdx.x] = mySum;
  __syncthreads();
  for (int off = 1; off < SPH_BLOCK; off <<= 1) {
    const uint32_t v = (threadIdx.x >= (unsigned)off) ? scan[threadIdx.x - off] : 0u;
    __syncthreads();
    scan[threadIdx.x] += v;
    __syncthreads();
  }
  uint32_t digitStart[PER];
  {
    uint32_t run = scan[threadIdx.x] - mySum;
#pragma unroll
    for (int p = 0; p < PER; p++) { digitStart[p] = run; run += tot[p]; }
  }
  const int base = blockIdx.x * RS_TILE + wave * (64 * RS_ITEMS);
  const unsigned long long ltMask = (lane == 0) ? 0ull : (~0ull >> (64 - lane));
  uint32_t key[RS_ITEMS], val[RS_ITEMS], rank[RS_ITEMS];
#pragma unroll
  for (int r = 0; r < RS_ITEMS; r++) {
    const int i = base + r * 64 + lane;
    const bool valid = i < N;
    key[r] = valid ? keysIn[i] : 0u;
    val[r] = valid ? valsIn[i] : 0u;
    const uint32_t dgt = (key[r] >> shift) & (uint32_t)(D - 1);
    unsigned long long peers = __ballot(valid);
#pragma unroll
    for (int b = 0; b < BITS; b++) {
      const bool bit = (dgt >> b) & 1u;
      const unsigned long long m = __ballot(valid && bit);
      peers &= bit ? m : ~m;
    }
    const uint32_t before = valid ? waveCount[wave][dgt] : 0u;
    rank[r] = before + (uint32_t)__popcll(peers & ltMask);
    if (valid && (peers & ltMask) == 0ull) waveCount[wave][dgt] = before + (uint32_t)__popcll(peers);
  }
  __syncthreads();
#pragma unroll
  for (int p = 0; p < PER; p++) {
    const int dgt = threadIdx.x * PER + p;
    uint32_t run = digitStart[p] + blockHist[(size_t)dgt * numBlocks + blockIdx.x];
#pragma unroll
    for (int w = 0; w < 4; w++) { digitBase[w][dgt] = run; run += waveCount[w][dgt]; }
  }
  __syncthreads();
#pragma unroll
  for (int r = 0; r < RS_ITEMS; r++) {
    const int i = base + r * 64 + lane;
    if (i < N) {
      const uint32_t dst = digitBase[wave][(key[r] >> shift) & (uint32_t)(D - 1)] + rank[r];
      keysOut[dst] = key[r];
      valsOut[dst] = val[r];
    }
  }
}

int sphk_sort(sph_solver* s) { return sphk_sort_pairs(s, s->d.N, s->sortBits); }

int sph_sort_digit_bits(int bits) { return ((bits + 8) / 9 < (bits + 7) / 8) ? 9 : 8; }
int sph_sort_passes(int bits) { const int w = sph_sort_digit_bits(bits); return (bits + w - 1) / w; }

template <int BITS>
static void radix_pass(sph_solver* s, int n, int nb, int shift) {
  SphDev& d = s->d;
  constexpr int D = 1 << BITS;
  uint32_t* digitTotal = s->blockHist + (size_t)SPH_SORT_MAX_DIGITS * s->maxSortBlocks;
  hipLaunchKernelGGL((k_radix_hist<BITS>), dim3(nb), dim3(SPH_BLOCK), 0, s->stream, d.keys, n, shift, s->blockHist, nb);
  hipLaunchKernelGGL(k_radix_scan_rows, dim3(D), dim3(SPH_BLOCK), 0, s->stream, s->blockHist, nb, digitTotal);
  hipLaunchKernelGGL((k_radix_scatter<BITS>), dim3(nb), dim3(SPH_BLOCK), 0, s->stream, d.keys, d.vals, d.keysAlt, d.valsAlt,
                     n, shift, s->blockHist, nb, digitTotal);
  uint32_t* t = d.keys; d.keys = d.keysAlt; d.keysAlt = t;
  t = d.vals; d.vals = d.valsAlt; d.valsAlt = t;
}

int sphk_sort_pairs(sph_solver* s, int n, int bits) {
  const int nb = (n + RS_TILE - 1) / RS_TILE;
  if (nb > s->maxSortBlocks) { sph_set_error("sort of %d keys exceeds the solver's capacity", n); return SPH_ERR_SIZE; }
  const int w = sph_sort_digit_bits(bits);
  for (int shift = 0; shift < bits; shift += w) {
    if (w == 9) radix_pass<9>(s, n, nb, shift);
    else radix_pass<8>(s, n, nb, shift);
  }
  SPH_HIP(hipGetLastError());
  return SPH_OK;
}

__global__ __launch_bounds__(SPH_BLOCK) void k_sort_post(SphDev d) {
  const int i = blockIdx.x * SPH_BLOCK + threadIdx.x;
  if (i >= d.N) return;
  const uint32_t src = d.vals[i];
  d.sortedPos[i] = d.posOrig[src];
  d.sortedVel[i] = d.velOrig[src];
  d.backIndex[src] = (uint32_t)i;
}

__global__ __launch_bounds__(SPH_BLOCK) void k_cell_start(SphDev d, int first, int last, int first2, int last2) {
  int c = first + blockIdx.x * SPH_BLOCK + threadIdx.x;
  if (c >= last) {
    const int spare = c - last;
    if (spare == 0) c = 0; else if (spare == 1) c = d.G; else c = first2 + (spare - 2);
    if (spare >= 2 && c >= last2) return;
  }
  if (c > d.G) return;
  int lo = 0, hi = d.N;
  while (lo < hi) {
    const int mid = (lo + hi) >> 1;
    if (d.keys[mid] < (uint32_t)c) lo = mid + 1; else hi = mid;
  }
  d.cellStart[c] = (c == d.G) ? (uint32_t)d.N : (uint32_t)lo;
}

int sphk_sort_post(sph_solver* s) {
  hipLaunchKernelGGL(k_sort_post, dim3(sph_blocks(s->d.N)), dim3(SPH_BLOCK), 0, s->stream, s->d);
  SPH_HIP(hipGetLastError());
  return SPH_OK;
}
int sphk_index_fixed(sph_solver* s) {
  int first = 0, last = s->d.G + 1, first2 = 0, last2 = 0;
  if (s->hasSlab) {
    const long long layerCells = (long long)s->d.gx * s->d.gy, W = s->slab.ghostLayers, G = s->d.G;
    const long long lo = max((long long)s->slab.layerLo - W - 2, 0LL) * layerCells;
    const long long hi = min(((long long)s->slab.layerHi + W + 3) * layerCells, G + 1);
    first = (int)min(lo, G + 1); last = (int)max(hi, (long long)first);
    const long long reach = layerCells + s->d.gx + 2;
    if (first == 0 && last < G + 1) { first2 = (int)max(G - reach, (long long)last); last2 = (int)G; }
    else if (last == G + 1 && first > 0) { first2 = 1; last2 = (int)min(reach + 1, (long long)first); }
  }
  const int lanes = (last - first) + 2 + max(last2 - first2, 0);
  hipLaunchKernelGGL(k_cell_start, dim3(sph_blocks(lanes)), dim3(SPH_BLOCK), 0, s->stream, s->d, first, last, first2, last2);
  SPH_HIP(hipGetLastError());
  return SPH_OK;
}
int sphk_sort_post_and_index(sph_solver* s) {
  int rc = sphk_sort_post(s);
  return rc == SPH_OK ? sphk_index_fixed(s) : rc;
}

__global__ __launch_bounds__(SPH_BLOCK) void k_index_raw(SphDev d) {
  const int i = blockIdx.x * SPH_BLOCK + threadIdx.x;
  if (i >= d.N) return;
  const uint32_t key = d.keys[i];
  if (key < (uint32_t)d.G && key > 0u && (i == 0 || d.keys[i - 1] != key)) d.cellStartRaw[key] = (uint32_t)i;
}
__global__ void k_index_raw_ends(SphDev d) {
  d.cellStartRaw[0] = 0u;
  d.cellStartRaw[d.G] = (uint32_t)d.N;
}

int sphk_index_raw(sph_solver* s) {
  SPH_HIP(hipMemsetAsync(s->d.cellStartRaw, 0xff, sizeof(uint32_t) * ((size_t)s->d.G + 1), s->stream));
  hipLaunchKernelGGL(k_index_raw, dim3(sph_blocks(s->d.N)), dim3(SPH_BLOCK), 0, s->stream, s->d);
  hipLaunchKernelGGL(k_index_raw_ends, dim3(1), dim3(1), 0, s->stream, s->d);
  SPH_HIP(hipGetLastError());
  return SPH_OK;
}
```

smoothed-particle-hydrodynamics_amd/sphmi/__init__.py:

```python
import ctypes as C
import os

import numpy as np

_PKG = os.path.dirname(os.path.dirname(os.path.abspath(__file__)))
LIB_PATH = os.environ.get("SPHMI_LIB", os.path.join(_PKG, "libsphmi.so"))
HOST_LIB_PATH = os.path.join(_PKG, "libsphmi_host.so")

ABI_VERSION = 2
SAMPLE_WORDS = 8
SURFACE_FIELDS = 6
DIAG_WORDS = 32
DIAG_MAX_REGIONS = 16
HIST_MAX_BINS = 4096
HIST_FIELDS = ("density", "speed", "pressure", "neighbors", "x", "y", "z")
SELECT_WORDS = 12
SELECT_MAX_TERMS = 4
SELECT_FIELDS = HIST_FIELDS + ("surface",)
GRADIENT_WORDS = 32
ELASTIC_WORDS = 12
MUSCLE_WORDS = 16
MEMBRANE_WORDS = 8
FORCE_WORDS = 40
FORCE_DIAG_WORDS = 64
FIELD_SLOTS = 4
FIELD_DIAG_WORDS = 8
TRACE_TIME, TRACE_ARC = 0, 1
TRACE_EULER, TRACE_MIDPOINT = 0, 1
TRACE_MOVING, TRACE_MAX_STEPS, TRACE_LEFT_MATTER, TRACE_LEFT_REGION, TRACE_STAGNANT, TRACE_NONFINITE = 0, 1, 2, 3, 4, 5
TRACE_MAX_STEPS_LIMIT = 65535
TRACE_MODES = ("time", "arc")
TRACE_INTEGRATORS = ("euler", "midpoint")
MAX_NEIGHBOR_COUNT = 32
LIQUID_PARTICLE, ELASTIC_PARTICLE, BOUNDARY_PARTICLE = 1, 2, 3

STAGE_NAMES = ["hash", "sort", "sort_post", "index", "find_neighbors", "density", "forces", "elastic",
               "predict_density", "pressure_force", "integrate", "membranes"]


class SphConfig(C.Structure):
    _fields_ = [("abi_version", C.c_int32), ("particleCount", C.c_int32), ("capacity", C.c_int32),
                ("gridCellsX", C.c_int32), ("gridCellsY", C.c_int32), ("gridCellsZ", C.c_int32),
                ("gridCellCount", C.c_int32), ("cellIdMask", C.c_uint32)] + \
               [(n, C.c_float) for n in
                ["h", "hashGridCellSize", "hashGridCellSizeInv", "simulationScale", "simulationScaleInv",
                 "xmin", "xmax", "ymin", "ymax", "zmin", "zmax", "r0", "mass", "rho0", "timeStep", "viscosity",
                 "delta", "gravity_x", "gravity_y", "gravity_z", "surfTensCoeff"]] + \
               [(n, C.c_double) for n in ["Wpoly6Coefficient", "gradWspikyCoefficient", "del2WviscosityCoefficient"]] + \
               [(n, C.c_int32) for n in ["numOfElasticP", "elasticOffset", "muscleCount", "numOfMembranes",
                                         "maxIteration", "device"]] + \
               [("stream", C.c_void_p)]


class SphSlab(C.Structure):
    _fields_ = [(n, C.c_int32) for n in ["layerLo", "layerHi", "ghostLayers", "hasLower", "hasUpper", "globalIdBits"]]


SLAB_RECORD_WORDS = 9
SLAB_COMPACT_WORDS = 7


class SphSelectTerm(C.Structure):
    _fields_ = [("field", C.c_int32), ("lo", C.c_float), ("hi", C.c_float)]


class SphRenderView(C.Structure):
    _fields_ = [("width", C.c_int32), ("height", C.c_int32), ("projection", C.c_int32),
                ("eye", C.c_float * 3), ("right", C.c_float * 3), ("up", C.c_float * 3), ("forward", C.c_float * 3),
                ("scale", C.c_float), ("centre", C.c_float * 2), ("nearPlane", C.c_float), ("radius", C.c_float),
                ("maxRadiusPx", C.c_float), ("colourMode", C.c_int32), ("field", C.c_int32), ("lo", C.c_float), ("hi", C.c_float),
                ("typeColour", (C.c_float * 3) * 3), ("ambient", C.c_float), ("background", C.c_uint8 * 4)]


RENDER_COLOUR_MODES = ("type", "density", "field", "label")


class SphRenderMeshStyle(C.Structure):
    _fields_ = [("source", C.c_int32), ("shading", C.c_int32), ("colourMode", C.c_int32), ("field", C.c_int32),
                ("lo", C.c_float), ("hi", C.c_float), ("colour", C.c_float * 3), ("compose", C.c_int32)]


RENDER_MESH_SOURCES = ("surface", "membranes")
RENDER_MESH_SHADINGS = ("flat", "smooth")
RENDER_MESH_SURFACE_FIELDS = ("density", "shepard", "vx", "vy", "vz", "pressure", "speed")


class SphTraceParams(C.Structure):
    _fields_ = [("step", C.c_float), ("minSpeed", C.c_float), ("maxSteps", C.c_int32), ("mode", C.c_int32), ("integrator", C.c_int32)]


class SphError(RuntimeError):
    pass


_host = None
_dev = None


def host_lib():
    global _host
    if _host is None:
        if not os.path.exists(HOST_LIB_PATH):
            raise SphError("libsphmi_host.so not built (run `python -c 'import __graft_entry__ as g; g.build()'`)")
        L = C.CDLL(HOST_LIB_PATH)
        L.sphmi_default_config.argtypes = [C.POINTER(SphConfig)]
        L.sphmi_config_set_box.argtypes = [C.POINTER(SphConfig), C.c_double, C.c_double, C.c_double, C.c_uint32]
        L.sphmi_count_particles.argtypes = [C.c_char_p]
        L.sphmi_load_configuration.argtypes = [C.c_char_p, C.c_char_p, C.c_int, C.c_void_p, C.c_void_p,
                                               C.POINTER(C.c_int), C.POINTER(C.c_int), C.POINTER(C.c_int)]
        L.sphmi_load_elastic_connections.argtypes = [C.c_char_p, C.c_int, C.c_void_p]
        L.sphmi_box_counts.argtypes = [C.POINTER(SphConfig), C.c_double, C.c_double, C.c_double, C.c_int, C.c_int, C.c_int, C.POINTER(C.c_int),
                                       C.POINTER(C.c_int)]
        L.sphmi_generate_box.argtypes = [C.POINTER(SphConfig), C.c_double, C.c_double, C.c_double, C.c_int, C.c_int, C.c_int, C.c_float, C.c_float,
                                         C.c_float, C.c_float, C.c_float, C.c_uint64, C.c_void_p, C.c_void_p]
        _box = [C.POINTER(SphConfig), C.c_double, C.c_double, C.c_double, C.c_int, C.c_int, C.c_int, C.c_float, C.c_float,
                C.c_float, C.c_float, C.c_float, C.c_uint64]
        L.sphmi_box_layer_histogram.argtypes = _box + [C.c_void_p, C.c_int]
        L.sphmi_generate_box_slice.argtypes = _box + [C.c_int, C.c_int, C.c_void_p, C.c_void_p, C.c_void_p, C.c_int, C.POINTER(C.c_int)]
        L.sphmi_muscle_signal.argtypes = [C.c_int, C.c_void_p, C.c_int]
        L.sphmi_step_chunk_edges.argtypes = [C.c_int64, C.c_int32, C.c_void_p]
        L.sphmi_step_pipeline_schedule.argtypes = [C.c_int32] * 4 + [C.c_void_p, C.c_void_p, C.c_int32, C.POINTER(C.c_int32)]
        L.sphmi_step_halo_check.argtypes = [C.c_void_p, C.c_int64, C.c_void_p, C.c_int64, C.c_void_p, C.c_int32, C.c_int32, C.c_int32]
        L.sphmi_trajectory_info.argtypes = [C.c_char_p] + [C.POINTER(C.c_int)] * 4
        L.sphmi_trajectory_frame.argtypes = [C.c_char_p, C.c_int, C.c_void_p]
        L.sphmi_trajectory_connections.argtypes = [C.c_char_p, C.c_int, C.c_void_p]
        L.sphmi_trajectory_membranes.argtypes = [C.c_char_p, C.c_int, C.c_void_p]
        L.sphmi_worm_counts.argtypes = [C.POINTER(SphConfig), C.c_double, C.c_double, C.c_double] + [C.POINTER(C.c_int)] * 4
        L.sphmi_generate_worm.argtypes = [C.POINTER(SphConfig), C.c_double, C.c_double, C.c_double] + [C.c_void_p] * 5
        L.sphmi_save_configuration.argtypes = [C.c_char_p, C.c_void_p, C.c_int, C.c_int, C.c_int, C.c_void_p, C.c_void_p,
                                               C.c_int, C.c_int]
        _host = L
    return _host


_STAGE_FUNCS = ["sph_run_clear_buffers", "sph_run_hash_particles", "sph_run_sort", "sph_run_sort_post_pass",
                "sph_run_indexx", "sph_run_index_post_pass", "sph_run_find_neighbors",
                "sph_run_pcisph_compute_density", "sph_run_pcisph_compute_forces_and_init_pressure",
                "sph_run_pcisph_compute_elastic_forces", "sph_run_pcisph_predict_positions",
                "sph_run_pcisph_predict_density", "sph_run_pcisph_correct_pressure",
                "sph_run_pcisph_compute_pressure_force_acceleration", "sph_run_clear_membrane_buffers",
                "sph_run_compute_interaction_with_membranes", "sph_run_compute_interaction_with_membranes_finalize"]
EXPORTED_SYMBOLS = ["sph_create", "sph_destroy", "sph_run_pcisph_integrate", "sph_step", "sph_update_muscles",
                    "sph_read_position", "sph_read_velocity", "sph_read_density", "sph_read_particle_index",
                    "sph_read_position_async", "sph_read_position_wait", "sph_host_unregister", "sph_build_info",
                    "sph_read_buffer", "sph_read_neighbor_rows", "sph_synchronize", "sph_set_stage_timing", "sph_get_stage_times",
                    "sph_reset_stage_times", "sph_step_sort_passes", "sph_set_step_chunks", "sph_set_step_pipeline", "sph_last_error", "sph_abi_version", "sph_slab_init", "sph_slab_pack", "sph_slab_pack_framed", "sph_slab_step_begin", "sph_slab_step_messages",
                    "sph_slab_rebuild", "sph_particle_count", "sph_slab_read", "sph_slab_rebuild_framed", "sph_slab_rebuild_finish",
                    "sph_slab_liquid_signature", "sph_slab_set_record_format", "sph_stream_wait_event", "sph_sample_points",
                    "sph_sample_grid", "sph_extract_surface", "sph_read_surface", "sph_sample_gradient_points",
                    "sph_sample_gradient_grid", "sph_surface_normals", "sph_diagnostics", "sph_histogram", "sph_label_components",
                    "sph_read_components", "sph_component_diagnostics", "sph_particle_measure", "sph_select_particles",
                    "sph_read_selection", "sph_elastic_measure", "sph_muscle_diagnostics", "sph_membrane_measure",
                    "sph_render_particles", "sph_read_render", "sph_render_mesh", "sph_read_render_triangles", "sph_force_measure", "sph_force_diagnostics", "sph_remove_region",
                    "sph_remove_selection", "sph_remove_ids", "sph_add_particles", "sph_emit_lattice", "sph_read_edit_map", "sph_field_create",
                    "sph_field_release", "sph_field_write", "sph_field_read", "sph_field_set_region", "sph_field_set_selection",
                    "sph_field_diffuse", "sph_field_diagnostics", "sph_trace_streamlines", "sph_tracers_set", "sph_tracers_advect",
                    "sph_tracers_read"] + _STAGE_FUNCS
HOST_EXPORTED_SYMBOLS = ["sphmi_default_config", "sphmi_config_set_box", "sphmi_count_particles",
                         "sphmi_load_configuration", "sphmi_load_elastic_connections", "sphmi_box_counts",
                         "sphmi_generate_box", "sphmi_box_layer_histogram", "sphmi_generate_box_slice", "sphmi_muscle_signal", "sphmi_step_chunk_edges", "sphmi_step_pipeline_schedule", "sphmi_step_halo_check", "sphmi_save_configuration", "sphmi_worm_counts",
                         "sphmi_generate_worm", "sphmi_trajectory_info", "sphmi_trajectory_frame", "sphmi_trajectory_connections",
                         "sphmi_trajectory_membranes"]


def hip_runtimes_loaded():
    paths = set()
    try:
        with open("/proc/self/maps") as f:
            for line in f:
                if "libamdhip64" in line:
                    paths.add(line.split()[-1])
    except OSError:
        pass
    return sorted(paths)


def _bind_one_hip_runtime():
    if hip_runtimes_loaded():
        return
    import importlib.util
    try:
        spec = importlib.util.find_spec("torch")
    except (ImportError, ValueError):
        spec = None
    if spec and spec.submodule_search_locations:
        cand = os.path.join(list(spec.submodule_search_locations)[0], "lib", "libamdhip64.so")
        if os.path.exists(cand):
            C.CDLL(cand, mode=C.RTLD_GLOBAL)


def device_lib():
    global _dev
    if _dev is None:
        if not os.path.exists(LIB_PATH):
            raise SphError("libsphmi.so not built: the HIP extension is required (no CPU fallback exists)")
        _bind_one_hip_runtime()
        L = C.CDLL(LIB_PATH)
        L.sph_create.argtypes = [C.POINTER(SphConfig), C.c_void_p, C.c_void_p, C.c_void_p, C.c_void_p, C.c_void_p,
                                 C.POINTER(C.c_void_p)]
        L.sph_destroy.argtypes = [C.c_void_p]
        for f in _STAGE_FUNCS + ["sph_synchronize", "sph_reset_stage_times", "sph_step_sort_passes"]:
            getattr(L, f).argtypes = [C.c_void_p]
        L.sph_run_pcisph_integrate.argtypes = [C.c_void_p, C.c_int]
        L.sph_step.argtypes = [C.c_void_p, C.c_int]
        L.sph_update_muscles.argtypes = [C.c_void_p, C.c_void_p, C.c_int]
        for f in ["sph_read_position", "sph_read_velocity", "sph_read_density", "sph_read_particle_index", "sph_read_position_async",
                  "sph_host_unregister"]:
            getattr(L, f).argtypes = [C.c_void_p, C.c_void_p]
        L.sph_read_position_wait.argtypes = [C.c_void_p]
        L.sph_build_info.restype = C.c_char_p
        L.sph_read_buffer.argtypes = [C.c_void_p, C.c_char_p, C.c_void_p, C.c_size_t, C.POINTER(C.c_size_t)]
        L.sph_read_neighbor_rows.argtypes = [C.c_void_p, C.c_int32, C.c_int32, C.c_void_p, C.c_void_p]
        L.sph_set_stage_timing.argtypes = [C.c_void_p, C.c_int]
        L.sph_set_step_chunks.argtypes = [C.c_void_p, C.c_int32]
        if hasattr(L, "sph_set_step_pipeline"):
            L.sph_set_step_pipeline.argtypes = [C.c_void_p, C.c_int32]
        L.sph_get_stage_times.argtypes = [C.c_void_p, C.POINTER(C.c_double), C.POINTER(C.c_int64), C.c_int]
        L.sph_last_error.restype = C.c_char_p
        L.sph_slab_init.argtypes = [C.c_void_p, C.POINTER(SphSlab), C.c_void_p]
        L.sph_slab_pack.argtypes = [C.c_void_p, C.c_void_p, C.c_void_p, C.c_int32, C.POINTER(C.c_int32)]
        L.sph_slab_pack_framed.argtypes = [C.c_void_p, C.c_void_p, C.c_void_p, C.c_int32, C.POINTER(C.c_int32)]
        L.sph_slab_step_begin.argtypes = [C.c_void_p, C.c_int, C.c_void_p, C.c_void_p, C.c_int32]
        L.sph_slab_step_messages.argtypes = [C.c_void_p, C.POINTER(C.c_int32)]
        L.sph_slab_rebuild.argtypes = [C.c_void_p, C.c_void_p, C.c_int32, C.c_void_p, C.c_int32]
        L.sph_slab_rebuild_framed.argtypes = [C.c_void_p, C.c_void_p, C.c_int32, C.c_void_p, C.c_int32]
        L.sph_slab_rebuild_finish.argtypes = [C.c_void_p, C.POINTER(C.c_int32)]
        L.sph_slab_liquid_signature.argtypes = [C.c_void_p, C.POINTER(C.c_uint32)]
        L.sph_slab_set_record_format.argtypes = [C.c_void_p, C.c_int32, C.c_uint32]
        L.sph_stream_wait_event.argtypes = [C.c_void_p, C.c_void_p]
        L.sph_particle_count.argtypes = [C.c_void_p]
        L.sph_slab_read.argtypes = [C.c_void_p, C.c_void_p, C.c_void_p, C.c_void_p, C.c_void_p]
        L.sph_sample_points.argtypes = [C.c_void_p, C.c_void_p, C.c_int32, C.c_uint32, C.c_void_p]
        L.sph_sample_grid.argtypes = [C.c_void_p, C.c_void_p, C.c_void_p, C.c_void_p, C.c_uint32, C.c_void_p]
        L.sph_extract_surface.argtypes = [C.c_void_p, C.c_void_p, C.c_void_p, C.c_void_p, C.c_uint32, C.c_int32, C.c_float,
                                          C.c_void_p]
        L.sph_read_surface.argtypes = [C.c_void_p, C.c_void_p, C.c_void_p]
        L.sph_sample_gradient_points.argtypes = [C.c_void_p, C.c_void_p, C.c_int32, C.c_uint32, C.c_void_p]
        L.sph_sample_gradient_grid.argtypes = [C.c_void_p, C.c_void_p, C.c_void_p, C.c_void_p, C.c_uint32, C.c_void_p]
        L.sph_surface_normals.argtypes = [C.c_void_p, C.c_void_p]
        L.sph_diagnostics.argtypes = [C.c_void_p, C.c_void_p, C.c_int32, C.c_uint32, C.c_void_p]
        L.sph_histogram.argtypes = [C.c_void_p, C.c_int32, C.c_float, C.c_float, C.c_int32, C.c_void_p, C.c_uint32, C.c_void_p]
        L.sph_label_components.argtypes = [C.c_void_p, C.c_float, C.c_uint32, C.c_void_p]
        L.sph_read_components.argtypes = [C.c_void_p, C.c_void_p, C.c_void_p, C.c_void_p]
        L.sph_component_diagnostics.argtypes = [C.c_void_p, C.c_void_p, C.c_int32, C.c_void_p]
        L.sph_particle_measure.argtypes = [C.c_void_p, C.c_void_p]
        L.sph_select_particles.argtypes = [C.c_void_p, C.c_void_p, C.c_uint32, C.c_void_p, C.c_int32, C.c_int32, C.c_void_p]
        L.sph_read_selection.argtypes = [C.c_void_p, C.c_void_p, C.c_void_p, C.c_void_p]
        L.sph_elastic_measure.argtypes = [C.c_void_p, C.c_void_p, C.c_void_p, C.c_void_p, C.c_void_p]
        L.sph_muscle_diagnostics.argtypes = [C.c_void_p, C.c_void_p]
        L.sph_membrane_measure.argtypes = [C.c_void_p, C.c_void_p, C.c_void_p]
        L.sph_force_measure.argtypes = [C.c_void_p, C.c_int32, C.c_void_p]
        L.sph_force_diagnostics.argtypes = [C.c_void_p, C.c_void_p, C.c_int32, C.c_uint32, C.c_void_p]
        L.sph_render_particles.argtypes = [C.c_void_p, C.POINTER(SphRenderView), C.c_void_p, C.c_uint32, C.c_int32, C.c_void_p]
        L.sph_read_render.argtypes = [C.c_void_p, C.c_void_p, C.c_void_p, C.c_void_p, C.c_void_p, C.c_void_p]
        L.sph_render_mesh.argtypes = [C.c_void_p, C.POINTER(SphRenderView), C.POINTER(SphRenderMeshStyle), C.c_void_p]
        L.sph_read_render_triangles.argtypes = [C.c_void_p, C.c_void_p]
        L.sph_remove_region.argtypes = [C.c_void_p, C.c_void_p, C.c_uint32, C.c_int32, C.c_void_p]
        L.sph_remove_selection.argtypes = [C.c_void_p, C.c_void_p]
        L.sph_remove_ids.argtypes = [C.c_void_p, C.c_void_p, C.c_int64, C.c_void_p]
        L.sph_add_particles.argtypes = [C.c_void_p, C.c_void_p, C.c_void_p, C.c_int32]
        L.sph_emit_lattice.argtypes = [C.c_void_p, C.c_void_p, C.c_void_p, C.c_void_p, C.c_void_p, C.c_float, C.c_void_p]
        L.sph_read_edit_map.argtypes = [C.c_void_p, C.c_void_p]
        L.sph_field_create.argtypes = [C.c_void_p, C.c_int32, C.c_void_p, C.c_float]
        L.sph_field_release.argtypes = [C.c_void_p, C.c_int32]
        L.sph_field_write.argtypes = [C.c_void_p, C.c_int32, C.c_void_p]
        L.sph_field_read.argtypes = [C.c_void_p, C.c_int32, C.c_void_p]
        L.sph_field_set_region.argtypes = [C.c_void_p, C.c_int32, C.c_void_p, C.c_uint32, C.c_float, C.c_void_p]
        L.sph_field_set_selection.argtypes = [C.c_void_p, C.c_int32, C.c_float, C.c_void_p]
        L.sph_field_diffuse.argtypes = [C.c_void_p, C.c_int32, C.c_float, C.c_int32, C.c_uint32, C.c_void_p]
        L.sph_field_diagnostics.argtypes = [C.c_void_p, C.c_int32, C.c_void_p, C.c_int32, C.c_uint32, C.c_void_p]
        L.sph_trace_streamlines.argtypes = [C.c_void_p, C.c_void_p, C.c_int32, C.c_uint32, C.POINTER(SphTraceParams), C.c_void_p,
                                            C.c_void_p, C.c_void_p, C.c_void_p]
        L.sph_tracers_set.argtypes = [C.c_void_p, C.c_void_p, C.c_int32]
        L.sph_tracers_advect.argtypes = [C.c_void_p, C.c_uint32, C.POINTER(SphTraceParams), C.c_void_p, C.c_void_p]
        L.sph_tracers_read.argtypes = [C.c_void_p, C.c_void_p, C.c_void_p, C.c_void_p]
        _dev = L
    return _dev


def default_config():
    cfg = SphConfig()
    rc = host_lib().sphmi_default_config(C.byref(cfg))
    if rc:
        raise SphError("sphmi_default_config failed: %d" % rc)
    cfg._box_in_h = (30.0, 20.0, 250.0)
    return cfg


def set_box(cfg, xmax_in_h, ymax_in_h, zmax_in_h, cell_id_mask=0xffff):
    rc = host_lib().sphmi_config_set_box(C.byref(cfg), xmax_in_h, ymax_in_h, zmax_in_h, cell_id_mask)
    if rc:
        raise SphError("sphmi_config_set_box failed: %d" % rc)
    cfg._box_in_h = (float(xmax_in_h), float(ymax_in_h), float(zmax_in_h))
    return cfg


def config_dict(cfg):
    d = {n: getattr(cfg, n) for n, _ in SphConfig._fields_ if n not in ("stream",)}
    d["N"] = d["particleCount"]
    return d


def load_configuration(position_file, velocity_file):
    n = host_lib().sphmi_count_particles(position_file.encode())
    if n <= 0:
        raise SphError("cannot read %s" % position_file)
    pos = np.empty((n, 4), np.float32)
    vel = np.empty((n, 4), np.float32)
    nl, ne, nb = C.c_int(), C.c_int(), C.c_int()
    rc = host_lib().sphmi_load_configuration(position_file.encode(), velocity_file.encode(), n, pos.ctypes.data,
                                             vel.ctypes.data, C.byref(nl), C.byref(ne), C.byref(nb))
    if rc:
        raise SphError("sphmi_load_configuration failed: %d" % rc)
    return pos, vel, dict(numOfLiquidP=nl.value, numOfElasticP=ne.value, numOfBoundaryP=nb.value)


def generate_box(cfg, lx, ly, lz, spacing=None, origin=None, jitter=0.0, seed=20261004):
    nl, nb = C.c_int(), C.c_int()
    bx = cfg._box_in_h
    rc = host_lib().sphmi_box_counts(C.byref(cfg), bx[0], bx[1], bx[2], lx, ly, lz, C.byref(nl), C.byref(nb))
    if rc:
        raise SphError("sphmi_box_counts failed: %d" % rc)
    n = nl.value + nb.value
    r0 = np.float32(cfg.r0)
    if spacing is None:
        spacing = np.float32(0.93) * r0
    if origin is None:
        origin = (np.float32(3) * r0,) * 3
    pos = np.empty((n, 4), np.float32)
    vel = np.empty((n, 4), np.float32)
    rc = host_lib().sphmi_generate_box(C.byref(cfg), bx[0], bx[1], bx[2], lx, ly, lz, spacing, origin[0], origin[1], origin[2], jitter,
                                       seed, pos.ctypes.data, vel.ctypes.data)
    if rc:
        raise SphError("sphmi_generate_box failed: %d" % rc)
    cfg.particleCount = n
    return pos, vel, dict(numOfLiquidP=nl.value, numOfElasticP=0, numOfBoundaryP=nb.value)


def _box_args(cfg, lx, ly, lz, spacing, origin, jitter, seed):
    bx = cfg._box_in_h
    r0 = np.float32(cfg.r0)
    if spacing is None:
        spacing = np.float32(0.93) * r0
    if origin is None:
        origin = (np.float32(3) * r0,) * 3
    return [C.byref(cfg), bx[0], bx[1], bx[2], lx, ly, lz, spacing, origin[0], origin[1], origin[2], jitter, seed]


def box_counts(cfg, lx, ly, lz):
    nl, nb = C.c_int(), C.c_int()
    bx = cfg._box_in_h
    rc = host_lib().sphmi_box_counts(C.byref(cfg), bx[0], bx[1], bx[2], lx, ly, lz, C.byref(nl), C.byref(nb))
    if rc:
        raise SphError("sphmi_box_counts failed: %d" % rc)
    return nl.value, nb.value


def box_layer_histogram(cfg, lx, ly, lz, spacing=None, origin=None, jitter=0.0, seed=20261004):
    hist = np.zeros(cfg.gridCellsZ, np.int64)
    rc = host_lib().sphmi_box_layer_histogram(*_box_args(cfg, lx, ly, lz, spacing, origin, jitter, seed), hist.ctypes.data, hist.size)
    if rc:
        raise SphError("sphmi_box_layer_histogram failed: %d" % rc)
    return hist


def generate_box_slice(cfg, lx, ly, lz, layer_lo, layer_hi, spacing=None, origin=None, jitter=0.0, seed=20261004):
    args = _box_args(cfg, lx, ly, lz, spacing, origin, jitter, seed) + [int(max(layer_lo, -(1 << 30))), int(min(layer_hi, 1 << 30))]
    n = C.c_int()
    rc = host_lib().sphmi_generate_box_slice(*args, None, None, None, 0, C.byref(n))
    if rc:
        raise SphError("sphmi_generate_box_slice failed: %d" % rc)
    pos, vel, gid = np.empty((n.value, 4), np.float32), np.empty((n.value, 4), np.float32), np.empty(n.value, np.uint32)
    rc = host_lib().sphmi_generate_box_slice(*args, pos.ctypes.data, vel.ctypes.data, gid.ctypes.data, n.value, C.byref(n))
    if rc:
        raise SphError("sphmi_generate_box_slice failed: %d" % rc)
    return pos, vel, gid


def generate_worm(cfg):
    bx = cfg._box_in_h
    ne, nl, nb, nm = C.c_int(), C.c_int(), C.c_int(), C.c_int()
    rc = host_lib().sphmi_worm_counts(C.byref(cfg), bx[0], bx[1], bx[2], C.byref(ne), C.byref(nl), C.byref(nb), C.byref(nm))
    if rc:
        raise SphError("sphmi_worm_counts failed: %d" % rc)
    n = ne.value + nl.value + nb.value
    pos = np.empty((n, 4), np.float32)
    vel = np.empty((n, 4), np.float32)
    elastic = np.empty((ne.value * 32, 4), np.float32)
    membranes = np.empty((nm.value, 3), np.int32)
    pml = np.empty((ne.value, 7), np.int32)
    rc = host_lib().sphmi_generate_worm(C.byref(cfg), bx[0], bx[1], bx[2], pos.ctypes.data, vel.ctypes.data, elastic.ctypes.data,
                                        membranes.ctypes.data, pml.ctypes.data)
    if rc:
        raise SphError("sphmi_generate_worm failed: %d" % rc)
    cfg.particleCount, cfg.numOfElasticP, cfg.numOfMembranes, cfg.elasticOffset = n, ne.value, nm.value, 0
    return dict(cfg=cfg, position=pos, velocity=vel, elastic=elastic, membranes=membranes, particle_membranes=pml,
                numOfLiquidP=nl.value, numOfElasticP=ne.value, numOfBoundaryP=nb.value)


def save_configuration(directory, position, num_elastic, num_liquid, connections=None, membranes=None, first=True):
    pos = np.ascontiguousarray(position, np.float32)
    con = None if connections is None else np.ascontiguousarray(connections, np.float32)
    mem = None if membranes is None else np.ascontiguousarray(membranes, np.int32)
    rc = host_lib().sphmi_save_configuration(directory.encode(), pos.ctypes.data, pos.shape[0], num_elastic, num_liquid,
                                             None if con is None else con.ctypes.data,
                                             None if mem is None else mem.ctypes.data,
                                             0 if mem is None else mem.shape[0], int(first))
    if rc:
        raise SphError("sphmi_save_configuration failed: %d" % rc)


def load_trajectory(directory):
    L = host_lib()
    ne, nl, nf, nm = C.c_int(), C.c_int(), C.c_int(), C.c_int()
    d = directory.encode()
    if L.sphmi_trajectory_info(d, C.byref(ne), C.byref(nl), C.byref(nf), C.byref(nm)):
        raise SphError("no trajectory in %s" % directory)
    P = ne.value + nl.value
    frames = np.empty((nf.value, P, 4), np.float32)
    for f in range(nf.value):
        if L.sphmi_trajectory_frame(d, f, frames[f].ctypes.data):
            raise SphError("trajectory frame %d unreadable" % f)
    out = dict(numOfElasticP=ne.value, numOfLiquidP=nl.value, frames=frames, connections=None, membranes=None)
    if ne.value:
        con = np.empty((32 * ne.value, 4), np.float32)
        if L.sphmi_trajectory_connections(d, ne.value, con.ctypes.data) == 0:
            out["connections"] = con
    if nm.value:
        mem = np.empty((nm.value, 4), np.int32)
        if L.sphmi_trajectory_membranes(d, nm.value, mem.ctypes.data) == 0:
            out["membranes"] = mem
    return out


def muscle_signal(step, muscle_count=100):
    out = np.zeros(muscle_count, np.float32)
    rc = host_lib().sphmi_muscle_signal(step, out.ctypes.data, muscle_count)
    if rc:
        raise SphError("sphmi_muscle_signal failed: %d" % rc)
    return out


def step_chunk_edges(n, chunks):
    if n < 0 or chunks < 1:
        raise SphError("step_chunk_edges: n >= 0 and chunks >= 1")
    out = np.zeros(chunks + 1, np.int64)
    rc = host_lib().sphmi_step_chunk_edges(n, chunks, out.ctypes.data)
    if rc:
        raise SphError("sphmi_step_chunk_edges failed: %d" % rc)
    return out


def step_pipeline_schedule(chunks, depth, max_iteration=3, has_elastic=False):
    if chunks < 1 or not 0 <= depth <= 6 or max_iteration < 0:
        raise SphError("step_pipeline_schedule: chunks >= 1, 0 <= depth <= 6, max_iteration >= 0")
    cap = 7 * chunks
    stage, chunk = np.zeros(cap, np.int32), np.zeros(cap, np.int32)
    clamped = C.c_int32(-1)
    n = host_lib().sphmi_step_pipeline_schedule(chunks, depth, max_iteration, int(bool(has_elastic)), stage.ctypes.data,
                                                chunk.ctypes.data, cap, C.byref(clamped))
    if n < 0:
        raise SphError("sphmi_step_pipeline_schedule failed: %d" % n)
    return clamped.value, [(int(a), int(b)) for a, b in zip(stage[:n], chunk[:n])]


def step_halo_check(keys, cell_start, edges, gx, gy):
    keys = np.ascontiguousarray(keys, np.uint32)
    cell_start = np.ascontiguousarray(cell_start, np.uint32)
    edges = np.ascontiguousarray(edges, np.int64)
    rc = host_lib().sphmi_step_halo_check(keys.ctypes.data, keys.size, cell_start.ctypes.data, cell_start.size - 1, edges.ctypes.data,
                                          edges.size - 1, int(gx), int(gy))
    if rc < 0:
        raise SphError("sphmi_step_halo_check failed: %d" % rc)
    return bool(rc)


_BUF_DTYPE = {"position": np.float32, "velocity": np.float32, "sortedPosition": np.float32,
              "sortedVelocity": np.float32, "acceleration": np.float32, "neighborMap": np.float32,
              "neighborIds": np.int32, "particleIndex": np.uint32, "particleIndexBack": np.uint32,
              "gridCellIndex": np.uint32, "gridCellIndexFixedUp": np.uint32, "pressure": np.float32,
              "rho": np.float32, "debugCounters": np.uint32, "diagnosticTrace": np.uint32,
              "pressureForceSkipped": np.uint8, "predictDensitySkipped": np.uint8}


def type_mask(types):
    m = 0
    for t in types:
        m |= 1 << int(t)
    return m & 0xffffffff


def _ptr(a):
    return None if a is None else a.ctypes.data_as(C.c_void_p)


def _points4(points, what):
    pts = np.asarray(points, np.float32)
    pts = pts.reshape(-1, pts.shape[-1]) if pts.ndim else pts.reshape(-1, 1)
    if pts.shape[1] not in (3, 4):
        raise SphError("%s: points must be [Q, 3] or [Q, 4]" % what)
    p4 = np.zeros((pts.shape[0], 4), np.float32)
    p4[:, :3] = pts[:, :3]
    return p4


def _lattice(origin, spacing, dims):
    return (np.ascontiguousarray(origin, np.float32).reshape(3), np.ascontiguousarray(spacing, np.float32).reshape(3),
            np.ascontiguousarray(dims, np.int32).reshape(3))


def _region(region, what):
    if region is None:
        return None
    rg = np.ascontiguousarray(region, np.float32)
    if rg.size != 6:
        raise SphError("%s: region must be (x0, y0, z0, x1, y1, z1)" % what)
    return rg


def _regions(regions, what):
    if regions is None:
        regions = [(-np.inf,) * 3 + (np.inf,) * 3]
    rg = np.ascontiguousarray(regions, np.float32)
    if rg.size % 6:
        raise SphError("%s: regions must be [R, 6]" % what)
    return rg.reshape(-1, 6)


def _field_index(field, names, what):
    if isinstance(field, str):
        if field not in names:
            raise SphError("%s: field must be one of %s" % (what, names))
        field = names.index(field)
    return int(field)


def build_info():
    return device_lib().sph_build_info().decode()


class owHIPSolver:

    def __init__(self, cfg, position_cpp, velocity_cpp, elasticConnectionsData_cpp=None, membraneData_cpp=None,
                 particleMembranesList_cpp=None):
        self._L = device_lib()
        self.cfg = cfg
        self.N = cfg.particleCount
        pos = np.ascontiguousarray(position_cpp, np.float32)
        vel = np.ascontiguousarray(velocity_cpp, np.float32)
        if pos.size != 4 * self.N or vel.size != 4 * self.N:
            raise SphError("position/velocity must hold 4*particleCount floats")
        el = None if elasticConnectionsData_cpp is None else np.ascontiguousarray(elasticConnectionsData_cpp, np.float32)
        mb = None if membraneData_cpp is None else np.ascontiguousarray(membraneData_cpp, np.int32)
        pm = None if particleMembranesList_cpp is None else np.ascontiguousarray(particleMembranesList_cpp, np.int32)
        for name, a, want, rule in (("elasticConnectionsData", el, 4 * 32 * cfg.numOfElasticP, "4*32*numOfElasticP"),
                                    ("membraneData", mb, 3 * cfg.numOfMembranes, "3*numOfMembranes"),
                                    ("particleMembranesList", pm, 7 * cfg.numOfElasticP, "7*numOfElasticP")):
            if a is not None and a.size != max(want, 0):
                raise SphError("%s holds %d words, the configuration asks for %s = %d" % (name, a.size, rule, want))
        h = C.c_void_p()
        self._chk(self._L.sph_create(C.byref(cfg), _ptr(pos), _ptr(vel), _ptr(el), _ptr(mb), _ptr(pm), C.byref(h)))
        self._h = h

    def _chk(self, rc):
        if rc != 0:
            raise SphError("libsphmi: %s (status %d)" % (self._L.sph_last_error().decode(), rc))
        return 0

    def close(self):
        if getattr(self, "_h", None):
            self._L.sph_destroy(self._h)
            self._h = None

    def __del__(self):
        try:
            self.close()
        except Exception:
            pass

    def _runClearBuffers(self): return self._chk(self._L.sph_run_clear_buffers(self._h))
    def _runHashParticles(self): return self._chk(self._L.sph_run_hash_particles(self._h))
    def _runSort(self): return self._chk(self._L.sph_run_sort(self._h))
    def _runSortPostPass(self): return self._chk(self._L.sph_run_sort_post_pass(self._h))
    def _runIndexx(self): return self._chk(self._L.sph_run_indexx(self._h))
    def _runIndexPostPass(self): return self._chk(self._L.sph_run_index_post_pass(self._h))
    def _runFindNeighbors(self): return self._chk(self._L.sph_run_find_neighbors(self._h))
    def _run_pcisph_computeDensity(self): return self._chk(self._L.sph_run_pcisph_compute_density(self._h))
    def _run_pcisph_computeForcesAndInitPressure(self): return self._chk(self._L.sph_run_pcisph_compute_forces_and_init_pressure(self._h))
    def _run_pcisph_computeElasticForces(self): return self._chk(self._L.sph_run_pcisph_compute_elastic_forces(self._h))
    def _run_pcisph_predictPositions(self): return self._chk(self._L.sph_run_pcisph_predict_positions(self._h))
    def _run_pcisph_predictDensity(self): return self._chk(self._L.sph_run_pcisph_predict_density(self._h))
    def _run_pcisph_correctPressure(self): return self._chk(self._L.sph_run_pcisph_correct_pressure(self._h))
    def _run_pcisph_computePressureForceAcceleration(self): return self._chk(self._L.sph_run_pcisph_compute_pressure_force_acceleration(self._h))
    def _run_pcisph_integrate(self, iterationCount): return self._chk(self._L.sph_run_pcisph_integrate(self._h, iterationCount))
    def _run_clearMembraneBuffers(self): return self._chk(self._L.sph_run_clear_membrane_buffers(self._h))
    def _run_computeInteractionWithMembranes(self): return self._chk(self._L.sph_run_compute_interaction_with_membranes(self._h))
    def _run_computeInteractionWithMembranes_finalize(self): return self._chk(self._L.sph_run_compute_interaction_with_membranes_finalize(self._h))

    def updateMuscleActivityData(self, signal):
        s = np.ascontiguousarray(signal, np.float32)
        return self._chk(self._L.sph_update_muscles(self._h, _ptr(s), s.size))

    def read_position_buffer(self, out=None):
        out = np.empty((self.N, 4), np.float32) if out is None else out
        self._chk(self._L.sph_read_position(self._h, _ptr(out)))
        return out

    def read_position_buffer_async(self, out):
        if not (isinstance(out, np.ndarray) and out.dtype == np.float32 and out.flags.c_contiguous and out.size == 4 * self.N):
            raise SphError("read_position_buffer_async needs a C-contiguous float32 array of 4*N elements")
        self._async_out = out
        self._chk(self._L.sph_read_position_async(self._h, _ptr(out)))
        return out

    def wait_position_buffer(self):
        return self._chk(self._L.sph_read_position_wait(self._h))

    def read_velocity_buffer(self, out=None):
        out = np.empty((self.N, 4), np.float32) if out is None else out
        self._chk(self._L.sph_read_velocity(self._h, _ptr(out)))
        return out

    def read_density_buffer(self, out=None):
        out = np.empty(self.N, np.float32) if out is None else out
        self._chk(self._L.sph_read_density(self._h, _ptr(out)))
        return out

    def read_particleIndex_buffer(self, out=None):
        out = np.empty((self.N, 2), np.uint32) if out is None else out
        self._chk(self._L.sph_read_particle_index(self._h, _ptr(out)))
        return out

    def sample_points(self, points, types=(1, 2, 3)):
        p4 = _points4(points, "sample_points")
        out = np.empty((p4.shape[0], SAMPLE_WORDS), np.float32)
# ... 272 lines not shown
    def field_write(self, slot, values):
        self._chk(self._L.sph_field_write(self._h, int(slot), _ptr(self._field_values(values, "field_write"))))

    def field_set_region(self, slot, value, region=None, types=(1,)):
        rg = _region(region, "field_set_region")
        painted = np.zeros(1, np.int64)
        self._chk(self._L.sph_field_set_region(self._h, int(slot), _ptr(rg), type_mask(types), float(np.float32(value)), _ptr(painted)))
        return int(painted[0])

    def field_set_selection(self, slot, value):
        painted = np.zeros(1, np.int64)
        self._chk(self._L.sph_field_set_selection(self._h, int(slot), float(np.float32(value)), _ptr(painted)))
        return int(painted[0])

    def field_diffuse(self, slot, coefficient, substeps=1, types=(1,)):
        sigma = np.zeros(1, np.float32)
        self._chk(self._L.sph_field_diffuse(self._h, int(slot), float(np.float32(coefficient)), int(substeps), type_mask(types), _ptr(sigma)))
        return float(sigma[0])

    def field_diagnostics(self, slot, regions=None, types=(1,)):
        rg = _regions(regions, "field_diagnostics")
        out = np.zeros((max(rg.shape[0], 1), FIELD_DIAG_WORDS), np.float64)
        self._chk(self._L.sph_field_diagnostics(self._h, int(slot), _ptr(rg), rg.shape[0], type_mask(types), _ptr(out)))
        return out

    def _trace_params(self, what, step, mode, integrator, max_steps, min_speed, dt):
        mode = _field_index(mode, TRACE_MODES, what)
        if dt is not None:
            if step is not None or mode != TRACE_TIME:
                raise SphError("%s: dt replaces step, in mode \"time\"" % what)
            step = np.float32(dt) / np.float32(self.cfg.simulationScale)
        if step is None:
            raise SphError("%s: step or dt must be given" % what)
        return SphTraceParams(float(np.float32(step)), float(np.float32(min_speed)), int(max_steps), mode,
                              _field_index(integrator, TRACE_INTEGRATORS, what))

    def streamlines(self, seeds, types=(1,), step=None, mode="arc", integrator="midpoint", max_steps=256, min_speed=0.0, region=None,
                    dt=None):
        p4 = _points4(seeds, "streamlines")
        prm = self._trace_params("streamlines", step, mode, integrator, max_steps, min_speed, dt)
        rg = _region(region, "streamlines")
        Q, M = p4.shape[0], max(int(max_steps), 0)
        verts = np.empty((Q, M + 1, 4), np.float32)
        lengths = np.empty(Q, np.int32)
        status = np.empty(Q, np.int32)
        self._chk(self._L.sph_trace_streamlines(self._h, _ptr(p4), Q, type_mask(types), C.byref(prm), _ptr(rg), _ptr(verts),
                                                _ptr(lengths), _ptr(status)))
        return verts, lengths, status

    def tracers_set(self, points):
        p4 = _points4(points, "tracers_set") if points is not None and np.size(points) else np.zeros((0, 4), np.float32)
        self._chk(self._L.sph_tracers_set(self._h, _ptr(p4) if p4.size else None, p4.shape[0]))
        self._tracers = p4.shape[0]

    def tracers_advect(self, types=(1,), step=None, mode="time", integrator="midpoint", min_speed=0.0, region=None, dt=None):
        prm = self._trace_params("tracers_advect", step, mode, integrator, 0, min_speed, dt)
        rg = _region(region, "tracers_advect")
        counts = np.zeros(2, np.int64)
        self._chk(self._L.sph_tracers_advect(self._h, type_mask(types), C.byref(prm), _ptr(rg), _ptr(counts)))
        return int(counts[0]), int(counts[1])

    def tracers(self):
        n = getattr(self, "_tracers", 0)
        pos = np.empty((n, 4), np.float32)
        status = np.empty(n, np.int32)
        steps = np.empty(n, np.int32)
        self._chk(self._L.sph_tracers_read(self._h, _ptr(pos) if n else None, _ptr(status) if n else None, _ptr(steps) if n else None))
        return pos, status, steps

    def step(self, iterationCount=0):
        return self._chk(self._L.sph_step(self._h, iterationCount))

    def synchronize(self):
        return self._chk(self._L.sph_synchronize(self._h))

    def buffer(self, name):
        need = C.c_size_t()
        self._chk(self._L.sph_read_buffer(self._h, name.encode(), None, 0, C.byref(need)))
        out = np.empty(need.value // np.dtype(_BUF_DTYPE[name]).itemsize, _BUF_DTYPE[name])
        self._chk(self._L.sph_read_buffer(self._h, name.encode(), _ptr(out), need.value, None))
        return out

    def neighbor_rows(self, first, count):
        ids = np.empty((count, 32), np.int32)
        dist = np.empty((count, 32), np.float32)
        self._chk(self._L.sph_read_neighbor_rows(self._h, first, count, _ptr(ids), _ptr(dist)))
        return ids, dist

    def slab_init(self, slab, global_ids):
        g = np.ascontiguousarray(global_ids, np.uint32)
        return self._chk(self._L.sph_slab_init(self._h, C.byref(slab), _ptr(g)))

    def slab_pack(self, msg_down_ptr, msg_up_ptr, cap_records):
        counts = (C.c_int32 * 3)()
        self._chk(self._L.sph_slab_pack(self._h, msg_down_ptr, msg_up_ptr, cap_records, counts))
        return counts[0], counts[1], counts[2]

    def slab_pack_framed(self, frame_down_ptr, frame_up_ptr, cap_records):
        counts = (C.c_int32 * 3)()
        self._chk(self._L.sph_slab_pack_framed(self._h, frame_down_ptr, frame_up_ptr, cap_records, counts))
        return counts[0], counts[1], counts[2]

    def slab_step_begin(self, iterationCount, frame_down_ptr, frame_up_ptr, cap_records):
        self._chk(self._L.sph_slab_step_begin(self._h, iterationCount, frame_down_ptr, frame_up_ptr, cap_records))

    def slab_step_messages(self):
        counts = (C.c_int32 * 2)()
        self._chk(self._L.sph_slab_step_messages(self._h, counts))
        return counts[0], counts[1]

    def slab_rebuild(self, recv_down_ptr, n_down, recv_up_ptr, n_up):
        self._chk(self._L.sph_slab_rebuild(self._h, recv_down_ptr, n_down, recv_up_ptr, n_up))
        self.N = self._L.sph_particle_count(self._h)
        return self.N

    def slab_rebuild_framed(self, frame_down_ptr, cap_down_records, frame_up_ptr, cap_up_records):
        self._chk(self._L.sph_slab_rebuild_framed(self._h, frame_down_ptr, cap_down_records, frame_up_ptr, cap_up_records))

    def slab_rebuild_finish(self):
        c = (C.c_int32 * 4)()
        self._chk(self._L.sph_slab_rebuild_finish(self._h, c))
        if not c[3]:
            self.N = self._L.sph_particle_count(self._h)
        return c[0], c[1], c[2], bool(c[3])

    def slab_liquid_signature(self):
        b = C.c_uint32()
        self._chk(self._L.sph_slab_liquid_signature(self._h, C.byref(b)))
        return b.value

    def slab_set_record_format(self, words, type_bits=0):
        return self._chk(self._L.sph_slab_set_record_format(self._h, words, type_bits))

    def stream_wait_event(self, hip_event_handle):
        return self._chk(self._L.sph_stream_wait_event(self._h, C.c_void_p(hip_event_handle)))

    def slab_read(self):
        n = self._L.sph_particle_count(self._h)
        pos, vel = np.empty((n, 4), np.float32), np.empty((n, 4), np.float32)
        gid, owned = np.empty(n, np.uint32), np.empty(n, np.uint32)
        self._chk(self._L.sph_slab_read(self._h, _ptr(pos), _ptr(vel), _ptr(gid), _ptr(owned)))
        return pos, vel, gid, owned

    def set_stage_timing(self, enable=True):
        return self._chk(self._L.sph_set_stage_timing(self._h, int(enable)))

    def set_step_chunks(self, chunks=0):
        return self._chk(self._L.sph_set_step_chunks(self._h, int(chunks)))

    def set_step_pipeline(self, depth=-1):
        if not hasattr(self._L, "sph_set_step_pipeline"):
            raise SphError("this libsphmi has no sph_set_step_pipeline")
        return self._chk(self._L.sph_set_step_pipeline(self._h, int(depth)))

    def reset_stage_times(self):
        return self._chk(self._L.sph_reset_stage_times(self._h))

    def step_sort_passes(self):
        n = self._L.sph_step_sort_passes(self._h)
        if n < 0:
            self._chk(n)
        return n

    def stage_times(self):
        n = len(STAGE_NAMES)
        ms = (C.c_double * n)()
        cnt = (C.c_int64 * n)()
        self._chk(self._L.sph_get_stage_times(self._h, ms, cnt, n))
        return {STAGE_NAMES[i]: (ms[i], cnt[i]) for i in range(n)}


class owPhysicsFluidSimulator:

    def __init__(self, cfg, position_cpp, velocity_cpp, elasticConnectionsData_cpp=None, membraneData_cpp=None,
                 particleMembranesList_cpp=None, fused=True, muscles=False):
        self.ocl_solver = owHIPSolver(cfg, position_cpp, velocity_cpp, elasticConnectionsData_cpp, membraneData_cpp,
                                      particleMembranesList_cpp)
        self.cfg = cfg
        self.iterationCount = 0
        self.fused = fused
        self.muscles = muscles
        self.position_cpp = np.array(position_cpp, np.float32).reshape(-1, 4)

    def simulationStep(self, read_back=True, async_read_back=False):
        s = self.ocl_solver
        if self.fused:
            s.step(self.iterationCount)
        else:
            s._runClearBuffers(); s._runHashParticles(); s._runSort(); s._runSortPostPass(); s._runIndexx()
            s._runIndexPostPass(); s._runFindNeighbors()
            s._run_pcisph_computeDensity(); s._run_pcisph_computeForcesAndInitPressure()
            s._run_pcisph_computeElasticForces()
            it = 0
            while True:
                s._run_pcisph_predictPositions(); s._run_pcisph_predictDensity(); s._run_pcisph_correctPressure()
                s._run_pcisph_computePressureForceAcceleration()
                it += 1
                if it >= self.cfg.maxIteration:
                    break
            s._run_pcisph_integrate(self.iterationCount)
            s._run_clearMembraneBuffers(); s._run_computeInteractionWithMembranes()
            s._run_computeInteractionWithMembranes_finalize()
        if read_back and self.position_cpp.shape[0] != s.N:
            s._chk(s._L.sph_host_unregister(s._h, _ptr(self.position_cpp)))
            self.position_cpp = np.empty((s.N, 4), np.float32)
        if read_back and async_read_back:
            s.read_position_buffer_async(self.position_cpp)
        elif read_back:
            s.read_position_buffer(self.position_cpp)
        if self.muscles:
            s.updateMuscleActivityData(muscle_signal(self.iterationCount, self.cfg.muscleCount))
        self.iterationCount += 1

    def getPosition_cpp(self):
        self.ocl_solver.wait_position_buffer()
        return self.position_cpp

    def getDensity_cpp(self): return self.ocl_solver.read_density_buffer()
    def getParticleIndex_cpp(self): return self.ocl_solver.read_particleIndex_buffer()
```

Measured before the change: 1.284 billion particle-steps/s.

## Push wave-skip flags to reader neighbourhoods instead of pulling per-neighbour flags

Replaces the pull-style check, where every particle in the predict-density and pressure-force stages gathers its 32 neighbours' wave flags, with a push-style scheme. Writers whose pressure or position changed mark all waves covering the 27 neighbouring cells into a per-stage neighbourhood byte array, and readers test a single byte per wave before loading any neighbour data. Neighbour tile loads are moved after the skip decision so skipped waves no longer fetch them. This adds cell-table scans and scattered byte stores on the writer side, a per-step clear in the hash kernel, an escape hatch that disables skipping for huge cells or out-of-grid keys, and a mode knob.

Result: faster. 1.355 billion particle-steps/s, median of 6 (+5.5%).

```diff
diff --git a/include/sphmi.h b/include/sphmi.h
--- a/include/sphmi.h
+++ b/include/sphmi.h
@@ -245,6 +245,8 @@
 int sph_set_step_chunks(sph_solver* s, int32_t chunks);
 int sph_set_step_pipeline(sph_solver* s, int32_t depth);
 
+int sph_set_wave_skip(sph_solver* s, int32_t mode);
+
 typedef struct sph_slab {
   int32_t layerLo, layerHi;
   int32_t ghostLayers;
diff --git a/smoothed-particle-hydrodynamics_amd/csrc/sph_api.hip b/smoothed-particle-hydrodynamics_amd/csrc/sph_api.hip
--- a/smoothed-particle-hydrodynamics_amd/csrc/sph_api.hip
+++ b/smoothed-particle-hydrodynamics_amd/csrc/sph_api.hip
@@ -372,7 +372,10 @@
   A(d.nbrId, mapN); A(d.nbrDist, mapN); A(d.nbr16, mapN); A(d.nbrBase, (size_t)s->capTiles * 64);
   A(d.rho, n);
   const size_t waves = (size_t)s->capTiles;
-  A(d.pBlk, waves); A(d.cBlk, waves); A(d.xBlk, waves); A(d.k12Skip, waves); A(d.k10Skip, waves); A(d.skipGate, SPH_GATE_SLOTS);
+  const size_t waves4 = (waves + 3) / 4 * 4;
+  A(d.pBlk, waves4); A(d.cBlk, waves4); A(d.xBlk, waves4); A(d.k12Skip, waves); A(d.k10Skip, waves); A(d.skipGate, SPH_GATE_SLOTS);
+  A(d.nbhd, waves4 * SPH_GATE_SLOTS);
+  d.nbStride = (int)waves4; d.nbOut = d.nbIn = d.nbhd; d.gatePolicy = 1; d.cellTable = d.cellStart;
   A(s->blockHist, (size_t)SPH_SORT_MAX_DIGITS * s->maxSortBlocks + SPH_SORT_MAX_DIGITS);
   A(d.gid, n); A(d.owned, n); A(s->slabCounts, SPH_SLAB_COUNT_WORDS);
   A(d.dbg, SPH_DBG_WORDS); A(s->chunkEdges, SPH_STEP_CHUNKS_MAX + 1); A(s->pipeTable, SPH_STEP_CHUNKS_MAX + 3);
@@ -411,6 +414,7 @@
   hipMemsetAsync(d.rho, 0, sizeof(float) * n, s->stream);
   hipMemsetAsync(d.rp, 0, sizeof(float2) * n, s->stream);
   for (uint8_t* f : {d.pBlk, d.cBlk, d.xBlk, d.k12Skip, d.k10Skip}) hipMemsetAsync(f, 0, waves, s->stream);
+  hipMemsetAsync(d.nbhd, 0, waves4 * SPH_GATE_SLOTS, s->stream);
   hipMemsetAsync(d.nbrId, 0xff, sizeof(int32_t) * mapN, s->stream);
   hipMemsetAsync(d.nbrDist, 0, sizeof(float) * mapN, s->stream);
   hipMemsetAsync(d.nbr16, 0xff, sizeof(uint16_t) * mapN, s->stream);
@@ -515,6 +519,13 @@
   return SPH_OK;
 }
 
+extern "C" int sph_set_wave_skip(sph_solver* s, int32_t mode) {
+  ENTER(s);
+  if (mode < 0 || mode > 2) { sph_set_error("sph_set_wave_skip: %d is not in [0, 2]", mode); return SPH_ERR_INVALID; }
+  s->waveSkipMode = mode;
+  return SPH_OK;
+}
+
 static int step_chunks(const sph_solver* s) {
   if (s->hasSlab || s->timing) return 1;
   if (s->stepChunks > 0) return s->stepChunks;
@@ -611,7 +622,7 @@
   auto layersFor = [&](int hops) { return slab ? min((hops * 31 + 59) / 60, s->slab.ghostLayers) : -1; };
   const int chunks = step_chunks(s);
   const int piped = chunks > 1 ? step_pipeline(s) : 0;
-  s->waveSkip = !slab && piped <= 1;
+  s->waveSkip = !slab && piped <= 1 && s->waveSkipMode != 2 && (long long)s->d.G > (long long)s->d.gx * s->d.gy + s->d.gx + 1;
   if (chunks > 1) {
     rc = enqueue_search_overlapped(s, chunks, piped);
     if (rc != SPH_OK) return rc;
diff --git a/smoothed-particle-hydrodynamics_amd/csrc/sph_api_read.hip b/smoothed-particle-hydrodynamics_amd/csrc/sph_api_read.hip
--- a/smoothed-particle-hydrodynamics_amd/csrc/sph_api_read.hip
+++ b/smoothed-particle-hydrodynamics_amd/csrc/sph_api_read.hip
@@ -140,7 +140,7 @@
   const SphDev& d = s->d;
   const size_t n = (size_t)d.N, G1 = (size_t)d.G + 1;
   size_t need = 0;
-  enum { B_POS, B_VEL, B_SPOS, B_SVEL, B_ACC, B_NMAP, B_NIDS, B_PI, B_PIB, B_GCI, B_GCIF, B_P, B_RHO, B_DBG, B_TRACE, B_K12SKIP, B_K10SKIP } which;
+  enum { B_POS, B_VEL, B_SPOS, B_SVEL, B_ACC, B_NMAP, B_NIDS, B_PI, B_PIB, B_GCI, B_GCIF, B_P, B_RHO, B_DBG, B_TRACE, B_K12SKIP, B_K10SKIP, B_NBP, B_NBX, B_PBLK, B_XBLK } which;
   if (!strcmp(name, "position")) { which = B_POS; need = sizeof(float4) * 2 * n; }
   else if (!strcmp(name, "velocity")) { which = B_VEL; need = sizeof(float4) * 2 * n; }
   else if (!strcmp(name, "sortedPosition")) { which = B_SPOS; need = sizeof(float4) * 2 * n; }
@@ -158,6 +158,10 @@
   else if (!strcmp(name, "debugCounters")) { which = B_DBG; need = sizeof(uint32_t) * SPH_DBG_WORDS; }
   else if (!strcmp(name, "pressureForceSkipped")) { which = B_K12SKIP; need = (n + SPH_TILE - 1) / SPH_TILE; }
   else if (!strcmp(name, "predictDensitySkipped")) { which = B_K10SKIP; need = (n + SPH_TILE - 1) / SPH_TILE; }
+  else if (!strcmp(name, "pressureNeighbourhood")) { which = B_NBP; need = (n + SPH_TILE - 1) / SPH_TILE; }
+  else if (!strcmp(name, "movedNeighbourhood")) { which = B_NBX; need = (n + SPH_TILE - 1) / SPH_TILE; }
+  else if (!strcmp(name, "pressureFlags")) { which = B_PBLK; need = (n + SPH_TILE - 1) / SPH_TILE; }
+  else if (!strcmp(name, "movedFlags")) { which = B_XBLK; need = (n + SPH_TILE - 1) / SPH_TILE; }
   else { sph_set_error("unknown buffer '%s'", name); return SPH_ERR_UNKNOWN_BUFFER; }
   if (needed) *needed = need;
   if (!out) return SPH_OK;
@@ -219,6 +223,10 @@
     case B_DBG: rc = sph_d2h(s, o, d.dbg, sizeof(uint32_t) * SPH_DBG_WORDS); break;
     case B_K12SKIP: rc = sph_d2h(s, o, d.k12Skip, need); break;
     case B_K10SKIP: rc = sph_d2h(s, o, d.k10Skip, need); break;
+    case B_NBP: rc = sph_d2h(s, o, d.nbhd + (size_t)((2 * s->cfg.maxIteration - 1) & (SPH_GATE_SLOTS - 1)) * d.nbStride, need); break;
+    case B_NBX: rc = sph_d2h(s, o, d.nbhd + (size_t)((s->cfg.maxIteration >= 2 ? 2 * s->cfg.maxIteration - 2 : 0) & (SPH_GATE_SLOTS - 1)) * d.nbStride, need); break;
+    case B_PBLK: rc = sph_d2h(s, o, d.pBlk, need); break;
+    case B_XBLK: rc = sph_d2h(s, o, d.xBlk, need); break;
     case B_RHO:
       rc = sph_d2h(s, o, d.rho, sizeof(float) * n);
       if (rc == SPH_OK) {
diff --git a/smoothed-particle-hydrodynamics_amd/csrc/sph_common.h b/smoothed-particle-hydrodynamics_amd/csrc/sph_common.h
--- a/smoothed-particle-hydrodynamics_amd/csrc/sph_common.h
+++ b/smoothed-particle-hydrodynamics_amd/csrc/sph_common.h
@@ -53,6 +53,11 @@
   uint8_t* xBlk;
   uint32_t* skipGate;
   int gateIn, gateOut;
+  uint8_t* nbhd;
+  uint8_t *nbOut, *nbIn;
+  int nbStride;
+  int gatePolicy;
+  const uint32_t* cellTable;
   uint8_t *k12Skip, *k10Skip;
   uint32_t *keys, *vals, *keysAlt, *valsAlt, *backIndex;
   uint32_t *cellStart, *cellStartRaw;
@@ -123,6 +128,7 @@
   int chunkEdgesN = -1, chunkEdgesC = -1;
   int stepPipeline = -1;
   bool waveSkip = false;
+  int waveSkipMode = 0;
   uint32_t* pipeTable = nullptr;
   bool copyPending = false;
   float* copyUserDst = nullptr;
diff --git a/smoothed-particle-hydrodynamics_amd/csrc/sph_pcisph.hip b/smoothed-particle-hydrodynamics_amd/csrc/sph_pcisph.hip
--- a/smoothed-particle-hydrodynamics_amd/csrc/sph_pcisph.hip
+++ b/smoothed-particle-hydrodynamics_amd/csrc/sph_pcisph.hip
@@ -83,27 +83,41 @@
 }
 __device__ __forceinline__ bool gate_open(const SphDev& d) { return d.skipGate[d.gateIn] == 0u; }
 __device__ __forceinline__ void gate_count(const SphDev& d, int id, bool waveFlagged) {
-  if (waveFlagged && ((id >> 8) & 63) == 0 && wave_leader() && *(volatile uint32_t*)&d.skipGate[d.gateOut] == 0u)
+  if (d.gatePolicy && waveFlagged && ((id >> 8) & 63) == 0 && wave_leader() && *(volatile uint32_t*)&d.skipGate[d.gateOut] == 0u)
     atomicAdd(&d.skipGate[d.gateOut], 1u);
 }
-__device__ __forceinline__ bool nbr_wave_flags(const NbrTile& t, const uint2 (&v16)[8], const bool wideRow, const uint8_t* flags) {
-  uint32_t seen = 0u;
-#pragma unroll
-  for (int g = 0; g < 8; g++) {
-    int jj[4];
-#pragma unroll
-    for (int k = 0; k < 4; k++) jj[k] = t.decode(v16[g], k);
-    if (wideRow) {
-#pragma unroll
-      for (int k = 0; k < 4; k++) jj[k] = t.id_wide(g * 4 + k);
-    }
-#pragma unroll
-    for (int k = 0; k < 4; k++) {
-      const uint32_t f = flags[NBR_INDEX(jj[k]) >> 6];
-      seen |= jj[k] != -1 ? f : 0u;
-    }
-  }
-  return seen != 0u;
+__device__ __forceinline__ void mark_readers(const SphDev& d, const int id) {
+  if (d.gatePolicy && *(volatile uint32_t*)&d.skipGate[d.gateOut] != 0u) return;
+  const uint32_t mine = d.keys[id];
+  const unsigned long long act = __ballot(1);
+  const int lane = (int)__lane_id();
+  const int rank = __popcll(act & ((1ull << lane) - 1ull)), n = __popcll(act);
+  const int layer = d.gx * d.gy;
+  bool todo = true;
+  for (;;) {
+    const unsigned long long m = __ballot(todo);
+    if (m == 0ull) break;
+    const uint32_t kj = (uint32_t)__builtin_amdgcn_readlane((int)mine, __ffsll(m) - 1);
+    todo = todo && mine != kj;
+    bool refuse = kj >= (uint32_t)d.G;
+    if (!refuse) {
+      for (int o = rank; o < 27; o += n) {
+        const int off = (o % 3 - 1) + ((o / 3) % 3 - 1) * d.gx + (o / 9 - 1) * layer;
+        int ki = (int)kj - off;
+        if (ki < 0) ki += d.G;
+        if (ki >= d.G) ki -= d.G;
+        if (ki < 0 || ki >= d.G) continue;
+        const uint32_t lo = d.cellTable[ki], hi = min(d.cellTable[ki + 1], (uint32_t)d.N);
+        if (hi <= lo) continue;
+        if (hi - lo > (1u << 20)) { refuse = true; continue; }
+        for (uint32_t w = lo >> 6; w <= (hi - 1u) >> 6; w++) d.nbOut[w] = 1;
+      }
+    }
+    if (__any(refuse) && rank == 0) atomicAdd(&d.skipGate[d.gateOut], 1u);
+  }
+}
+__device__ __forceinline__ uint32_t wave_byte(const uint8_t* a, int w) {
+  return (reinterpret_cast<const uint32_t*>(a)[w >> 2] >> ((w & 3) * 8)) & 0xffu;
 }
 
 constexpr int DENSITY_ITEMS = 1;
@@ -178,7 +192,7 @@
 
 __device__ __forceinline__ float corrected_pressure(const SphDev& d, float p, float rhoPred);
 
-template <bool FUSE_PREDICT, bool FUSE_DENSITY>
+template <bool FUSE_PREDICT, bool FUSE_DENSITY, bool MARK>
 __device__ __forceinline__ void forces_particle(const SphDev& d, const int id) {
   static_assert(FUSE_PREDICT || !FUSE_DENSITY, "the density half reads what the predict half forms");
   const float4 xi = d.sortedPos[id];
@@ -252,6 +266,7 @@
       }
     }
   }
+  bool mark = false;
   if (FUSE_DENSITY) {
     if (density < (double)d.hs6) density = (double)d.hs6;
     density *= d.massWpoly6;
@@ -260,21 +275,28 @@
     d.rp[id] = make_float2(rhoP, p);
     store_pred(d, id, xpi);
     if (d.pBlk) {
-      const bool anyP = wave_flag_store(d.pBlk, id, p != 0.f);
+      mark = wave_flag_store(d.pBlk, id, p != 0.f);
       const bool anyC = wave_flag_store(d.cBlk, id, closePair && !boundary);
-      gate_count(d, id, anyP || anyC);
-    }
-    if (boundary) { d.acc[id] = zero; return; }
-  }
-  d.bndMask[id] = bnd;
-  if (d.hasElastic) d.elasticMask[id] = ela;
-  const float scale = d.massMu * (float)(d.del2W / (double)d.rho[id]);
-  float4 a;
-  a.x = sx * scale + d.gravx + tx;
-  a.y = sy * scale + d.gravy + ty;
-  a.z = sz * scale + d.gravz + tz;
-  a.w = 0.f;
-  d.acc[id] = a;
+      gate_count(d, id, mark || anyC);
+    }
+  }
+  if (FUSE_DENSITY && boundary) {
+    d.acc[id] = zero;
+  } else {
+    d.bndMask[id] = bnd;
+    if (d.hasElastic) d.elasticMask[id] = ela;
+    const float scale = d.massMu * (float)(d.del2W / (double)d.rho[id]);
+    float4 a;
+    a.x = sx * scale + d.gravx + tx;
+    a.y = sy * scale + d.gravy + ty;
+    a.z = sz * scale + d.gravz + tz;
+    a.w = 0.f;
+    d.acc[id] = a;
+  }
+  if (mark) {
+    if (MARK) mark_readers(d, id);
+    else if (wave_leader() && *(volatile uint32_t*)&d.skipGate[d.gateOut] == 0u) atomicAdd(&d.skipGate[d.gateOut], 1u);
+  }
   if (FUSE_DENSITY) return;
   if (FUSE_PREDICT) store_pred(d, id, predict_position(d, xi, vi, zero));
   else { d.accP[id] = zero; d.rp[id].y = 0.f; }
@@ -284,14 +306,14 @@
 __global__ __launch_bounds__(SPH_BLOCK, 4) void k_forces(SphDev d, int nblocks) {
   int id;
   if (!xcd_range_id(d, id)) return;
-  forces_particle<FUSE_PREDICT, FUSE_DENSITY>(d, id);
+  forces_particle<FUSE_PREDICT, FUSE_DENSITY, true>(d, id);
 }
 template <bool FUSE_PREDICT, bool FUSE_DENSITY>
 __global__ __launch_bounds__(SPH_BLOCK, 4) void k_forces_strided(SphDev d) {
   const int active = range_blocks(d);
   for (int b = blockIdx.x; b < active; b += gridDim.x) {
     int id;
-    if (xcd_range_id(d, b, id)) forces_particle<FUSE_PREDICT, FUSE_DENSITY>(d, id);
+    if (xcd_range_id(d, b, id)) forces_particle<FUSE_PREDICT, FUSE_DENSITY, false>(d, id);
   }
 }
 
@@ -337,9 +359,15 @@
   return SPH_OK;
 }
 
+#ifndef SPH_WAVE_SKIP_GATED
+#define SPH_WAVE_SKIP_GATED 1
+#endif
 static SphDev wave_skip_view(const sph_solver* s, SphDev d, bool fused, int stage) {
   if (!(fused && s->waveSkip)) d.pBlk = d.cBlk = d.xBlk = d.k12Skip = d.k10Skip = nullptr;
   d.gateIn = (stage - 1) & (SPH_GATE_SLOTS - 1); d.gateOut = stage & (SPH_GATE_SLOTS - 1);
+  d.nbIn = s->d.nbhd + (size_t)d.gateIn * s->d.nbStride; d.nbOut = s->d.nbhd + (size_t)d.gateOut * s->d.nbStride;
+  d.cellTable = s->d.cellStart;
+  d.gatePolicy = s->waveSkipMode == 1 ? 0 : SPH_WAVE_SKIP_GATED;
   return d;
 }
 
@@ -362,29 +390,32 @@
   return p + p_corr;
 }
 
+__device__ __forceinline__ void publish_pressure(const SphDev& d, const int id, const float p) {
+  const bool anyP = wave_flag_store(d.pBlk, id, p != 0.f);
+  gate_count(d, id, anyP || d.cBlk[id >> 6] != 0);
+  if (anyP) mark_readers(d, id);
+}
+
 template <bool FUSE_CORRECT, bool FIRST>
 __device__ __forceinline__ void predict_density_particle(const SphDev& d, const int id) {
-  const float4 xi = load_pred(d, id);
-  const NbrTile t(d, id);
-  uint2 v16[8];
-#pragma unroll
-  for (int g = 0; g < 8; g++) v16[g] = t.vec16(g);
-  const bool wideRow = NbrTile::wide(v16[0]);
   if (FUSE_CORRECT && !FIRST && d.xBlk) {
-    bool skip = false;
+    const int w = __builtin_amdgcn_readfirstlane(id) >> 6;
+    const bool skip = gate_open(d) && wave_byte(d.nbIn, w) == 0u;
     const float2 old = d.rp[id];
-    if (gate_open(d)) {
-      const bool moved = d.xBlk[id >> 6] != 0 || nbr_wave_flags(t, v16, wideRow, d.xBlk);
-      skip = !__any(moved);
-    }
     if (wave_leader()) d.k10Skip[id >> 6] = skip ? 1 : 0;
     if (skip) {
       const float p = corrected_pressure(d, old.y, old.x);
       d.rp[id] = make_float2(old.x, p);
-      gate_count(d, id, wave_flag_store(d.pBlk, id, p != 0.f) || d.cBlk[id >> 6] != 0);
+      publish_pressure(d, id, p);
       return;
     }
   }
+  const float4 xi = load_pred(d, id);
+  const NbrTile t(d, id);
+  uint2 v16[8];
+#pragma unroll
+  for (int g = 0; g < 8; g++) v16[g] = t.vec16(g);
+  const bool wideRow = NbrTile::wide(v16[0]);
   double density = 0.0;
 #pragma unroll
   for (int b = 0; b < 32 / PD_BATCH; b++) {
@@ -417,7 +448,7 @@
     const float pOld = FIRST ? 0.f : d.rp[id].y;
     const float p = corrected_pressure(d, pOld, rhoP);
     d.rp[id] = make_float2(rhoP, p);
-    if (d.pBlk) gate_count(d, id, wave_flag_store(d.pBlk, id, p != 0.f) || d.cBlk[id >> 6] != 0);
+    if (d.pBlk) publish_pressure(d, id, p);
   } else {
     d.rp[id].x = rhoP;
   }
@@ -575,6 +606,12 @@
 __device__ __forceinline__ void pressure_force_particle(const SphDev& d, const int id) {
   const float4 xi = d.sortedPos[id];
   const float4 zero = make_float4(0.f, 0.f, 0.f, 0.f);
+  bool consult = false, skip = false;
+  if (FUSE != 0 && d.pBlk) {
+    const int w = __builtin_amdgcn_readfirstlane(id) >> 6;
+    consult = gate_open(d);
+    skip = consult && (wave_byte(d.nbIn, w) | wave_byte(d.cBlk, w)) == 0u;
+  }
   const bool boundary = TYPE_OF(xi) == SPH_BOUNDARY_PARTICLE;
   if (FUSE != 0 && d.pBlk && !__any(!boundary) && wave_leader()) {
     d.k12Skip[id >> 6] = 1;
@@ -586,26 +623,20 @@
     return;
   }
   const float2 rpi = d.rp[id];
-  const bool consult = FUSE != 0 && d.pBlk && gate_open(d);
   float4 vi = zero;
   if (FUSE != 0) vi = d.sortedVel[id];
   const float pi_ = rpi.y;
-  const bool ownOk = sph_exp_in(xi.x, SPH_FAST_COORD_EXP_LO, 100) && sph_exp_in(xi.y, SPH_FAST_COORD_EXP_LO, 100) &&
-                     sph_exp_in(xi.z, SPH_FAST_COORD_EXP_LO, 100);
-  const NbrTile t(d, id);
   float rx = 0.f, ry = 0.f, rz = 0.f;
-  const float hq = d.hs * 0.25f;
-  uint2 v16[8];
-#pragma unroll
-  for (int g = 0; g < 8; g++) v16[g] = t.vec16(g);
-  const bool wideRow = NbrTile::wide(v16[0]);
-  bool skip = false;
-  if (consult) {
-    const bool live = pi_ != 0.f || nbr_wave_flags(t, v16, wideRow, d.pBlk);
-    skip = d.cBlk[id >> 6] == 0 && !__any(live);
-  }
   if (FUSE != 0 && d.pBlk && wave_leader()) d.k12Skip[id >> 6] = skip ? 1 : 0;
   if (!skip) {
+    const bool ownOk = sph_exp_in(xi.x, SPH_FAST_COORD_EXP_LO, 100) && sph_exp_in(xi.y, SPH_FAST_COORD_EXP_LO, 100) &&
+                       sph_exp_in(xi.z, SPH_FAST_COORD_EXP_LO, 100);
+    const NbrTile t(d, id);
+    const float hq = d.hs * 0.25f;
+    uint2 v16[8];
+#pragma unroll
+    for (int g = 0; g < 8; g++) v16[g] = t.vec16(g);
+    const bool wideRow = NbrTile::wide(v16[0]);
 #pragma unroll
     for (int b = 0; b < 32 / PF_BATCH; b++) {
       int jj[PF_BATCH];
@@ -639,6 +670,7 @@
   if (FUSE != 1) d.accP[id] = ap;
   if (FUSE == 1) {
     const float4 xp = predict_position(d, xi, vi, ap);
+    bool moved = false;
     if (d.xBlk) {
       bool changed = true;
       if (consult) {
@@ -646,9 +678,11 @@
         changed = __float_as_uint(was.x) != __float_as_uint(xp.x) || __float_as_uint(was.y) != __float_as_uint(xp.y) ||
                   __float_as_uint(was.z) != __float_as_uint(xp.z);
       }
-      gate_count(d, id, wave_flag_store(d.xBlk, id, changed));
+      moved = wave_flag_store(d.xBlk, id, changed);
+      gate_count(d, id, moved);
     }
     store_pred(d, id, xp);
+    if (moved) mark_readers(d, id);
   }
   if (FUSE == 2) integrate_particle(d, id, xi, vi, d.acc[id], ap);
 }
diff --git a/smoothed-particle-hydrodynamics_amd/csrc/sph_sort.hip b/smoothed-particle-hydrodynamics_amd/csrc/sph_sort.hip
--- a/smoothed-particle-hydrodynamics_amd/csrc/sph_sort.hip
+++ b/smoothed-particle-hydrodynamics_amd/csrc/sph_sort.hip
@@ -1,8 +1,14 @@
 #include "sph_common.h"
+
+__device__ __forceinline__ void clear_wave_skip_state(const SphDev& d, int id) {
+  if (id < SPH_GATE_SLOTS) d.skipGate[id] = 0u;
+  const int words = (((d.N + 63) >> 6) + 3) >> 2;
+  if (id < SPH_GATE_SLOTS * words) reinterpret_cast<uint32_t*>(d.nbhd + (size_t)(id / words) * d.nbStride)[id % words] = 0u;
+}
 
 __global__ __launch_bounds__(SPH_BLOCK) void k_hash(SphDev d) {
   const int id = blockIdx.x * SPH_BLOCK + threadIdx.x;
-  if (id < SPH_GATE_SLOTS) d.skipGate[id] = 0u;
+  clear_wave_skip_state(d, id);
   if (id >= d.N) return;
   const float4 p = d.posOrig[id];
   if (!(fabsf(p.x) <= 3.0e38f && fabsf(p.y) <= 3.0e38f && fabsf(p.z) <= 3.0e38f)) atomicAdd(&d.dbg[6], 1u);
@@ -16,7 +22,7 @@
 
 __global__ __launch_bounds__(SPH_BLOCK) void k_hash_compact(SphDev d, CompactKey c) {
   const int id = blockIdx.x * SPH_BLOCK + threadIdx.x;
-  if (id < SPH_GATE_SLOTS) d.skipGate[id] = 0u;
+  clear_wave_skip_state(d, id);
   if (id >= d.N) return;
   const float4 p = d.posOrig[id];
   if (!(fabsf(p.x) <= 3.0e38f && fabsf(p.y) <= 3.0e38f && fabsf(p.z) <= 3.0e38f)) atomicAdd(&d.dbg[6], 1u);
@@ -261,6 +267,8 @@
     if (d.keys[mid] < (uint32_t)c) lo = mid + 1; else hi = mid;
   }
   d.cellStart[c] = (c == d.G) ? (uint32_t)d.N : (uint32_t)lo;
+  if (c == d.G && (lo < d.N || d.dbg[6] != 0u))
+    for (int i = 0; i < SPH_GATE_SLOTS; i++) d.skipGate[i] = 1u;
 }
 
 int sphk_sort_post(sph_solver* s) {
diff --git a/smoothed-particle-hydrodynamics_amd/sphmi/__init__.py b/smoothed-particle-hydrodynamics_amd/sphmi/__init__.py
--- a/smoothed-particle-hydrodynamics_amd/sphmi/__init__.py
+++ b/smoothed-particle-hydrodynamics_amd/sphmi/__init__.py
@@ -144,7 +144,7 @@
                     "sph_read_position", "sph_read_velocity", "sph_read_density", "sph_read_particle_index",
                     "sph_read_position_async", "sph_read_position_wait", "sph_host_unregister", "sph_build_info",
                     "sph_read_buffer", "sph_read_neighbor_rows", "sph_synchronize", "sph_set_stage_timing", "sph_get_stage_times",
-                    "sph_reset_stage_times", "sph_step_sort_passes", "sph_set_step_chunks", "sph_set_step_pipeline", "sph_last_error", "sph_abi_version", "sph_slab_init", "sph_slab_pack", "sph_slab_pack_framed", "sph_slab_step_begin", "sph_slab_step_messages",
+                    "sph_reset_stage_times", "sph_step_sort_passes", "sph_set_step_chunks", "sph_set_step_pipeline", "sph_set_wave_skip", "sph_last_error", "sph_abi_version", "sph_slab_init", "sph_slab_pack", "sph_slab_pack_framed", "sph_slab_step_begin", "sph_slab_step_messages",
                     "sph_slab_rebuild", "sph_particle_count", "sph_slab_read", "sph_slab_rebuild_framed", "sph_slab_rebuild_finish",
                     "sph_slab_liquid_signature", "sph_slab_set_record_format", "sph_stream_wait_event", "sph_sample_points",
                     "sph_sample_grid", "sph_extract_surface", "sph_read_surface", "sph_sample_gradient_points",
@@ -215,6 +215,8 @@
         L.sph_set_step_chunks.argtypes = [C.c_void_p, C.c_int32]
         if hasattr(L, "sph_set_step_pipeline"):
             L.sph_set_step_pipeline.argtypes = [C.c_void_p, C.c_int32]
+        if hasattr(L, "sph_set_wave_skip"):
+            L.sph_set_wave_skip.argtypes = [C.c_void_p, C.c_int32]
         L.sph_get_stage_times.argtypes = [C.c_void_p, C.POINTER(C.c_double), C.POINTER(C.c_int64), C.c_int]
         L.sph_last_error.restype = C.c_char_p
         L.sph_slab_init.argtypes = [C.c_void_p, C.POINTER(SphSlab), C.c_void_p]
@@ -480,7 +482,8 @@
               "neighborIds": np.int32, "particleIndex": np.uint32, "particleIndexBack": np.uint32,
               "gridCellIndex": np.uint32, "gridCellIndexFixedUp": np.uint32, "pressure": np.float32,
               "rho": np.float32, "debugCounters": np.uint32, "diagnosticTrace": np.uint32,
-              "pressureForceSkipped": np.uint8, "predictDensitySkipped": np.uint8}
+              "pressureForceSkipped": np.uint8, "predictDensitySkipped": np.uint8,
+              "pressureNeighbourhood": np.uint8, "movedNeighbourhood": np.uint8, "pressureFlags": np.uint8, "movedFlags": np.uint8}
 
 
 def type_mask(types):
@@ -1059,6 +1062,11 @@
         if not hasattr(self._L, "sph_set_step_pipeline"):
             raise SphError("this libsphmi has no sph_set_step_pipeline")
         return self._chk(self._L.sph_set_step_pipeline(self._h, int(depth)))
+
+    def set_wave_skip(self, mode=0):
+        if not hasattr(self._L, "sph_set_wave_skip"):
+            raise SphError("this libsphmi has no sph_set_wave_skip")
+        return self._chk(self._L.sph_set_wave_skip(self._h, int(mode)))
 
     def reset_stage_times(self):
         return self._chk(self._L.sph_reset_stage_times(self._h))
```
